# shangfuu/avse_challenge

Measured on AMD Instinct MI355X. Metric: utterances/sec (3s@16kHz + 75 lip frames), higher is better.
Workload: dtype fp32; 1 GPU; avse1 AV baseline train step (BASELINE configs[1]): HIP STFT front-end + AVNet (ResNet18 lip enc + TCN, dilated Conv2d audio net, LSTM fusion) fwd/bwd + Adam; global_batch=32, per_gpu_batch=32, seq_len=48000, stft_frames=376, lip_frames=75, lip_hw=96, parallelism=dp1, hip_graph=fwd+bwd+opt

## Files before the change

avse_challenge_amd/_lib.py:

```python
import ctypes
import os

import torch

_HERE = os.path.dirname(os.path.abspath(__file__))
LIB_PATH = os.environ.get("AVSE_HIP_LIB", os.path.join(_HERE, "libavse_hip.so"))

c_i64, c_i32, c_f32, c_vp = ctypes.c_int64, ctypes.c_int32, ctypes.c_float, ctypes.c_void_p

AVSE_F32, AVSE_BF16 = 0, 1


class ScanFwdArgs(ctypes.Structure):
    _fields_ = [
        ("batch", c_i64), ("dim", c_i64), ("seqlen", c_i64), ("dstate", c_i64),
        ("in_dtype", c_i32), ("delta_softplus", c_i32), ("reverse", c_i32),
        ("u", c_vp), ("u_bs", c_i64), ("u_ds", c_i64),
        ("delta", c_vp), ("delta_bs", c_i64), ("delta_ds", c_i64),
        ("A", c_vp),
        ("B", c_vp), ("B_bs", c_i64), ("B_ns", c_i64),
        ("C", c_vp), ("C_bs", c_i64), ("C_ns", c_i64),
        ("D", c_vp),
        ("z", c_vp), ("z_bs", c_i64), ("z_ds", c_i64),
        ("delta_bias", c_vp),
# ... 28 lines not shown
        ("ddelta_bias", c_vp),
        ("dz", c_vp), ("dz_bs", c_i64), ("dz_ds", c_i64),
        ("out_z", c_vp), ("out_z_bs", c_i64), ("out_z_ds", c_i64),
        ("workspace", c_vp),
        ("dz_accumulate", c_i32),
        ("dz_max", c_vp),
    ]


class GemmBf16Args(ctypes.Structure):
    _fields_ = [
        ("batch", c_i64), ("mp", c_i64), ("mq", c_i64), ("k", c_i64), ("fold", c_i64),
        ("p", c_vp), ("p_bs", c_i64), ("p_sx", c_i64), ("p_sk", c_i64), ("p_extent", c_i64),
        ("q", c_vp), ("q_bs", c_i64), ("q_sx", c_i64), ("q_sk", c_i64), ("q_extent", c_i64),
        ("c", c_vp), ("c_bs", c_i64), ("c_sq", c_i64),
        ("alpha", c_f32), ("c_dtype", c_i32),
    ]


class GemmF32sArgs(ctypes.Structure):
    _fields_ = [
        ("batch", c_i64), ("mp", c_i64), ("mq", c_i64), ("k", c_i64), ("fold", c_i64),
        ("p_hi", c_vp), ("p_lo", c_vp), ("p_bs", c_i64), ("p_sx", c_i64), ("p_sk", c_i64), ("p_extent", c_i64),
        ("p_max", c_vp),
        ("q_hi", c_vp), ("q_lo", c_vp), ("q_bs", c_i64), ("q_sx", c_i64), ("q_sk", c_i64), ("q_extent", c_i64),
        ("q_max", c_vp),
        ("c", c_vp), ("c_bs", c_i64), ("c_sq", c_i64),
        ("alpha", c_f32),
        ("nsub", c_i64), ("p_bs2", c_i64), ("q_bs2", c_i64),
    ]


SIGNATURES = {
    "avse_strerror": (ctypes.c_char_p, [c_i32]),
    "avse_abi_version": (c_i32, []),
    "avse_scan_n_chunks": (c_i64, [c_i64]),
    "avse_scan_bwd_workspace_bytes": (c_i64, [c_i64, c_i64, c_i64, c_i64]),
    "avse_scan_fwd": (c_i32, [ctypes.POINTER(ScanFwdArgs), c_vp]),
    "avse_scan_bwd": (c_i32, [ctypes.POINTER(ScanBwdArgs), c_vp]),
    "avse_dtproj": (c_i32, [c_i64, c_i64, c_i64, c_i64, c_i32, c_vp, c_i64, c_vp, c_i64, c_i64, c_vp, c_i32, c_vp, c_i64,
                            c_i64, c_vp]),
    "avse_cconv_bwd_workspace_bytes": (c_i64, [c_i64, c_i64, c_i64]),
    "avse_cconv_fwd": (c_i32, [c_i64, c_i64, c_i64, c_i64, c_vp, c_i64, c_i64, c_vp, c_vp, c_vp, c_i64, c_i64,
                               c_i32, c_i32, c_vp]),
    "avse_cconv_fwd_bf16": (c_i32, [c_i64, c_i64, c_i64, c_i64, c_vp, c_i64, c_i64, c_vp, c_vp, c_vp, c_i64, c_i64,
                                    c_i32, c_i32, c_vp]),
    "avse_cconv_bwd": (c_i32, [c_i64, c_i64, c_i64, c_i64, c_vp, c_i64, c_i64, c_vp, c_vp, c_vp, c_i64, c_i64,
                               c_vp, c_i64, c_i64, c_vp, c_vp, c_i32, c_i32, c_vp, c_i32, c_vp, c_vp]),
    "avse_cconv_bwd_bf16": (c_i32, [c_i64, c_i64, c_i64, c_i64, c_vp, c_i64, c_i64, c_vp, c_vp, c_vp, c_i64, c_i64,
                                    c_vp, c_i64, c_i64, c_vp, c_vp, c_i32, c_i32, c_vp, c_i32, c_vp, c_vp]),
    "avse_add_rmsnorm_fwd": (c_i32, [c_i64, c_i64, c_vp, c_vp, c_vp, c_f32, c_vp, c_vp, c_vp, c_vp, c_vp]),
    "avse_rmsnorm_bwd_workspace_bytes": (c_i64, [c_i64, c_i64]),
    "avse_rmsnorm_bwd": (c_i32, [c_i64, c_i64, c_vp, c_vp, c_vp, c_vp, c_vp, c_vp, c_vp, c_vp, c_vp, c_vp]),
    "avse_add_rmsnorm_fwd2": (c_i32, [c_i64, c_i64, c_vp, c_i32, c_vp, c_vp, c_f32, c_vp, c_i32, c_vp, c_vp, c_vp, c_vp]),
    "avse_rmsnorm_bwd2": (c_i32, [c_i64, c_i64, c_vp, c_i32] + [c_vp] * 9),
    "avse_stft_frames": (c_i64, [c_i64]),
    "avse_stft_fwd": (c_i32, [c_i64, c_i64, c_vp, c_vp, c_vp, c_vp]),
    "avse_istft": (c_i32, [c_i64, c_i64, c_i64, c_vp, c_vp, c_vp, c_vp, c_vp]),
    "avse_conv3d_wgrad_workspace_bytes": (c_i64, [c_i64, c_i64, c_i64, c_i64]),
    "avse_conv3d_wgrad": (c_i32, [c_i64] * 11 + [c_vp, c_vp, c_vp, c_i32, c_vp, c_vp]),
    "avse_conv3d_wgrad_u8": (c_i32, [c_i64] * 11 + [c_vp, c_vp, c_vp, c_i32, c_vp, c_vp]),
    "avse_conv3d_wgrad_u8_split": (c_i32, [c_i64] * 11 + [c_vp, c_vp, c_vp, c_vp, c_i32, c_vp, c_vp]),
    "avse_conv3d_wgrad_split": (c_i32, [c_i64] * 11 + [c_vp, c_vp, c_vp, c_vp, c_vp, c_i32, c_vp, c_vp]),
    "avse_conv3d_fwd_workspace_bytes": (c_i64, [c_i64, c_i64, c_i64]),
    "avse_conv3d_fwd": (c_i32, [c_i64] * 5 + [c_i32] + [c_vp] * 5),
    "avse_dconv_wgrad_workspace_bytes": (c_i64, [c_i64] * 4),
    "avse_dconv_wgrad": (c_i32, [c_i64] * 4 + [c_vp] * 6),
    "avse_prelu_fwd": (c_i32, [c_i64, c_i64, c_i64, c_i32, c_vp, c_vp, c_vp, c_vp]),
    "avse_prelu_bwd_workspace_bytes": (c_i64, [c_i64, c_i64]),
    "avse_prelu_bwd": (c_i32, [c_i64, c_i64, c_i64, c_i32, c_vp, c_vp, c_vp, c_vp, c_vp, c_vp, c_vp]),
    "avse_maxpool2d_out_size": (c_i64, [c_i64] * 4),
    "avse_maxpool2d_fwd": (c_i32, [c_i64] * 9 + [c_vp, c_vp, c_vp, c_vp]),
    "avse_maxpool2d_bwd": (c_i32, [c_i64] * 9 + [c_vp, c_vp, c_vp, c_vp]),
    "avse_transpose_cp": (c_i32, [c_i64] * 3 + [c_vp, c_vp, c_vp]),
    "avse_bnact_workspace_bytes": (c_i64, [c_i64, c_i64, c_i64]),
    "avse_bnact_fwd": (c_i32, [c_i64, c_i64, c_i64, c_vp, c_vp, c_vp, c_vp, c_i32, c_vp, c_i32, c_i32, c_f32, c_f32,
                               c_vp, c_vp, c_vp, c_vp, c_vp, c_vp, c_vp]),
    "avse_bnact_bwd": (c_i32, [c_i64, c_i64, c_i64, c_vp, c_vp, c_vp, c_vp, c_vp, c_vp, c_i32, c_vp, c_i32, c_i32,
                               c_vp, c_vp, c_vp, c_vp, c_vp, c_vp, c_vp, c_vp]),
    "avse_bnact_fwd_q": (c_i32, [c_i64, c_i64, c_i64, c_vp, c_vp, c_vp, c_i32, c_vp, c_i32, c_f32, c_f32, c_vp, c_vp,
                                 c_vp, c_vp, c_vp, c_vp, c_vp]),
    "avse_bnact_bwd_q": (c_i32, [c_i64, c_i64, c_i64, c_vp, c_vp, c_vp, c_vp, c_vp, c_i32, c_vp, c_i32, c_i32, c_vp,
                                 c_vp, c_vp, c_vp, c_vp, c_vp, c_vp]),
    "avse_prelu_nhwc_fwd": (c_i32, [c_i64, c_i64, c_i32, c_vp, c_vp, c_vp, c_vp]),
    "avse_prelu_nhwc_bwd_workspace_bytes": (c_i64, [c_i64, c_i64]),
    "avse_prelu_nhwc_bwd": (c_i32, [c_i64, c_i64, c_i32, c_vp, c_vp, c_vp, c_vp, c_vp, c_vp, c_vp]),
    "avse_prelu_gln_workspace_bytes": (c_i64, [c_i64, c_i64]),
    "avse_prelu_gln_fwd": (c_i32, [c_i64, c_i64, c_i64, c_vp, c_vp, c_vp, c_vp, c_f32, c_vp, c_vp, c_vp, c_vp]),
    "avse_prelu_gln_bwd": (c_i32, [c_i64, c_i64, c_i64] + [c_vp] * 11),
    "avse_prelu_gln_bwd_q": (c_i32, [c_i64, c_i64, c_i64] + [c_vp] * 7 + [c_i64] + [c_vp] * 6),
    "avse_dwconv_bwd_workspace_bytes": (c_i64, [c_i64, c_i64]),
    "avse_dwconv_fwd": (c_i32, [c_i64, c_i64, c_i64, c_i64, c_i64, c_vp, c_vp, c_vp, c_vp]),
    "avse_dwconv_bwd": (c_i32, [c_i64, c_i64, c_i64, c_i64, c_i64] + [c_vp] * 7),
    "avse_dwconv_gln_workspace_bytes": (c_i64, [c_i64, c_i64]),
    "avse_dwconv_gln_fwd": (c_i32, [c_i64] * 5 + [c_vp] * 5 + [c_f32] + [c_vp] * 5),
    "avse_dwconv_gln_fwd_q": (c_i32, [c_i64] * 5 + [c_vp] * 5 + [c_f32] + [c_vp] * 3 + [c_i64] + [c_vp] * 4),
    "avse_dwconv_gln_bwd": (c_i32, [c_i64] * 5 + [c_vp] * 14),
    "avse_lstm_padded_hidden": (c_i64, [c_i64]),
    "avse_lstm_group_size": (c_i64, [c_i64, c_i64]),
    "avse_lstm_group_workspace_bytes": (c_i64, [c_i64, c_i64]),
    "avse_lstm_group_capacity": (c_i64, [c_i64, c_i32]),
    "avse_lstm_fwd_group": (c_i32, [c_i64, c_i64, c_i64, c_i32, c_vp, c_vp, c_vp, c_i64, c_i64, c_vp, c_vp, c_vp, c_vp,
                                    c_vp]),
    "avse_lstm_bwd_group": (c_i32, [c_i64, c_i64, c_i64, c_i32, c_vp, c_i64, c_i64, c_vp, c_vp, c_vp, c_vp, c_vp, c_vp,
                                    c_vp]),
    "avse_lstm_fwd": (c_i32, [c_i64, c_i64, c_i64, c_i32, c_vp, c_vp, c_vp, c_i64, c_i64, c_vp, c_vp, c_vp]),
    "avse_lstm_bwd": (c_i32, [c_i64, c_i64, c_i64, c_i32, c_vp, c_i64, c_i64, c_vp, c_vp, c_vp, c_vp, c_vp]),
    "avse_gemm_bf16": (c_i32, [ctypes.POINTER(GemmBf16Args), c_vp]),
    "avse_gemm_f32s": (c_i32, [ctypes.POINTER(GemmF32sArgs), c_vp]),
    "avse_split16_planes": (c_i32, [c_i64, c_i64, c_i64, c_vp, c_i64, c_i64, c_vp, c_vp, c_vp, c_vp]),
    "avse_add_max": (c_i32, [c_i64, c_i64, c_i64, c_vp, c_vp, c_vp, c_vp, c_vp]),
    "avse_split16_planes_known": (c_i32, [c_i64, c_i64, c_i64, c_vp, c_i64, c_i64, c_vp, c_vp, c_vp, c_vp]),
    "avse_split16_planes_to": (c_i32, [c_i64, c_i64, c_i64, c_vp, c_i64, c_i64, c_vp, c_vp, c_i64, c_i64, c_vp, c_i32,
                                       c_vp]),
    "avse_dconv_wprep_bytes": (c_i64, []),
    "avse_split16": (c_i32, [c_i64, c_vp, c_vp, c_vp, c_vp]),
    "avse_split16_known": (c_i32, [c_i64, c_vp, c_vp, c_vp, c_vp]),
    "avse_dconv_wprep": (c_i32, [c_vp, c_i32, c_vp, c_vp, c_vp]),
    "avse_dconv_fwd": (c_i32, [c_i64, c_i64, c_i64, c_i64, c_vp, c_vp, c_vp, c_vp, c_vp, c_vp]),
    "avse_dconv_wprep2": (c_i32, [c_vp] * 6),
    "avse_dconv_wgrad16_workspace_bytes": (c_i64, [c_i64, c_i64, c_i64]),
    "avse_dconv_wgrad16": (c_i32, [c_i64, c_i64, c_i64, c_i64, c_vp, c_vp, c_vp, c_vp, c_vp, c_vp, c_vp, c_vp]),
    "avse_conv1_fwd": (c_i32, [c_i64] * 3 + [c_vp] * 5),
    "avse_conv1_dgrad": (c_i32, [c_i64] * 3 + [c_vp] * 4),
    "avse_conv1_wgrad_workspace_bytes": (c_i64, [c_i64] * 3),
    "avse_conv1_wgrad": (c_i32, [c_i64] * 3 + [c_vp] * 6),
    "avse_convf_fwd": (c_i32, [c_i64] + [c_vp] * 5),
    "avse_convf_dgrad": (c_i32, [c_i64] + [c_vp] * 4),
    "avse_convf_wgrad_workspace_bytes": (c_i64, [c_i64]),
    "avse_convf_wgrad": (c_i32, [c_i64] + [c_vp] * 6),
    "avse_sconv_wprep_bytes": (c_i64, [c_i64, c_i64]),
    "avse_sconv_wprep": (c_i32, [c_i64, c_i64, c_vp, c_i32, c_vp, c_vp, c_vp]),
    "avse_sconv_fwd": (c_i32, [c_i64] * 6 + [c_vp] * 6),
    "avse_sconv_wgrad_workspace_bytes": (c_i64, [c_i64] * 6),
    "avse_sconv_wgrad": (c_i32, [c_i64] * 6 + [c_vp] * 7),
    "avse_sconv_dgrad2_supported": (c_i32, [c_i64] * 5),
    "avse_sconv_dgrad2": (c_i32, [c_i64] * 5 + [c_vp] * 6),
}

_lib = None


class HipLibraryError(RuntimeError):
    pass


ABI_VERSION = 2


def lib():
    global _lib
    if _lib is None:
        if not os.path.exists(LIB_PATH):
            raise HipLibraryError(
                f"libavse_hip.so not found at {LIB_PATH}: build it with `python -c 'import __graft_entry__ as g; "
                f"g.build()'` (make -C avse_challenge_amd/csrc)")
        try:
            L = ctypes.CDLL(LIB_PATH, mode=ctypes.RTLD_GLOBAL)
        except OSError as e:
            raise HipLibraryError(f"failed to load {LIB_PATH}: {e}") from e
        for name, (res, args) in SIGNATURES.items():
            fn = getattr(L, name)
            fn.restype = res
            fn.argtypes = args
        if L.avse_abi_version() != ABI_VERSION:
            raise HipLibraryError(f"{LIB_PATH} has C-ABI version {L.avse_abi_version()}, the bindings expect "
# ... 17 lines not shown
```

avse_challenge_amd/csrc/bnact.hip:

```cpp
#include <algorithm>

#include "common.h"

namespace avse {
namespace bnact {

constexpr int THREADS = 256;
enum { ACT_NONE = 0, ACT_RELU = 1, ACT_PRELU = 2 };

struct Geo {
    int64_t N, CS, S;
    int C, TW, RPI, tiles, nrb;
};

template <int V> struct vld;
template <> struct vld<1> {
    __device__ static inline void ld(const float* p, float* v) { v[0] = *p; }
    __device__ static inline void st(float* p, const float* v) { *p = v[0]; }
};
template <> struct vld<4> {
    __device__ static inline void ld(const float* p, float* v) {
        const float4 q = *reinterpret_cast<const float4*>(p);
        v[0] = q.x; v[1] = q.y; v[2] = q.z; v[3] = q.w;
    }
    __device__ static inline void st(float* p, const float* v) {
        *reinterpret_cast<float4*>(p) = make_float4(v[0], v[1], v[2], v[3]);
    }
};

template <int V, int ACT>
struct ColConst {
    float a[V], b[V], al[V], mean[V], mlo[V], rstd[V], gam[V];
    __device__ inline float centred(float v, int k) const { return (v - mean[k]) - mlo[k]; }
    __device__ inline void load(const Geo& g, int64_t j0, const float* stats, const float* gamma, const float* beta,
                                const float* alpha, int alpha_n) {
#pragma unroll
        for (int k = 0; k < V; ++k) {
            const int c = (int)((j0 + k) / g.S);
            mean[k] = stats[4 * c];
            mlo[k] = stats[4 * c + 1];
            rstd[k] = stats[4 * c + 2];
            gam[k] = gamma ? gamma[c] : 1.f;
            a[k] = gam[k] * rstd[k];
            b[k] = beta ? beta[c] : 0.f;
            al[k] = ACT == ACT_PRELU ? alpha[alpha_n > 1 ? c : 0] : 0.f;
        }
    }
};

template <int ACT>
__device__ inline float act_fwd(float z, float al) {
    if constexpr (ACT == ACT_RELU) return z > 0.f ? z : 0.f;
    else if constexpr (ACT == ACT_PRELU) return z > 0.f ? z : al * z;
    else return z;
}
template <int ACT>
__device__ inline float act_bwd(float z, float g, float al) {
    if constexpr (ACT == ACT_RELU) return z > 0.f ? g : 0.f;
    else if constexpr (ACT == ACT_PRELU) return z > 0.f ? g : al * g;
    else return g;
}

template <int V, int NQ, int MAXQ = -1>
__device__ inline void block_partials(const Geo& g, float (&p)[NQ][V], bool valid, int64_t j0, float* ws) {
    __shared__ float part[NQ][THREADS * V];
    const int tx = threadIdx.x % g.TW, ty = threadIdx.x / g.TW;
#pragma unroll
    for (int q = 0; q < NQ; ++q)
#pragma unroll
        for (int k = 0; k < V; ++k) part[q][threadIdx.x * V + k] = p[q][k];
    __syncthreads();
    if (ty == 0 && valid) {
#pragma unroll
        for (int q = 0; q < NQ; ++q) {
            float s[V];
#pragma unroll
            for (int k = 0; k < V; ++k) s[k] = p[q][k];
            for (int t = 1; t < g.RPI; ++t)
#pragma unroll
                for (int k = 0; k < V; ++k)
                    s[k] = q == MAXQ ? fmaxf(s[k], part[q][(t * g.TW + tx) * V + k]) : s[k] + part[q][(t * g.TW + tx) * V + k];
            vld<V>::st(ws + ((int64_t)blockIdx.y * NQ + q) * g.CS + j0, s);
        }
    }
}

__device__ inline void block_max_out(float m, uint32_t* omax) {
    __shared__ uint32_t red[THREADS / 64];
    uint32_t b = __float_as_uint(m);
    for (int o = 32; o >= 1; o >>= 1) b = max(b, (uint32_t)__shfl_xor((int)b, o, 64));
    if ((threadIdx.x & 63) == 0) red[threadIdx.x >> 6] = b;
    __syncthreads();
    if (threadIdx.x == 0) {
        b = red[0];
#pragma unroll
        for (int w = 1; w < THREADS / 64; ++w) b = max(b, red[w]);
        if (b) atomicMax(omax, b);
    }
}

__device__ inline int q_split_exp(uint32_t mb) {
    const int ef = (int)((mb >> 23) & 0xff);
    if (mb == 0) return 0;
    const int k = ef == 0 ? -127 : ef - 127;
    return min(100, max(-100, 14 - k));
}
__device__ inline void q_store4(uint16_t* q, int64_t r, int64_t C, int64_t c, const float* v, float sc) {
    uint32_t hi[2], lo[2];
#pragma unroll
    for (int k = 0; k < 2; ++k) {
        const float s0 = v[2 * k] * sc, s1 = v[2 * k + 1] * sc;
        const _Float16 h0 = (_Float16)s0, h1 = (_Float16)s1;
        const _Float16 l0 = (_Float16)(s0 - (float)h0), l1 = (_Float16)(s1 - (float)h1);
        hi[k] = (uint32_t)__builtin_bit_cast(uint16_t, h0) | ((uint32_t)__builtin_bit_cast(uint16_t, h1) << 16);
        lo[k] = (uint32_t)__builtin_bit_cast(uint16_t, l0) | ((uint32_t)__builtin_bit_cast(uint16_t, l1) << 16);
    }
    uint16_t* base = q + r * 2 * C + 32 * (c >> 4) + (c & 15);
    *reinterpret_cast<uint2*>(base) = make_uint2(hi[0], hi[1]);
    *reinterpret_cast<uint2*>(base + 16) = make_uint2(lo[0], lo[1]);
}
__device__ inline void q_bound_out(double bnd, uint32_t* omax) {
    const float f = (float)(bnd * (1.0 + 1.0 / 1024.0));
    if (f > 0.f) atomicMax(omax, __float_as_uint(f));
}

template <int V, bool MAXD>
__global__ __launch_bounds__(THREADS) void stats_kernel(Geo g, const float* __restrict__ x, float* __restrict__ ws) {
    constexpr int NQ = MAXD ? 3 : 2;
    const int tx = threadIdx.x % g.TW, ty = threadIdx.x / g.TW;
    const int64_t j0 = ((int64_t)blockIdx.x * g.TW + tx) * V;
    const bool valid = j0 < g.CS;
    float p[NQ][V], K[V];
#pragma unroll
    for (int k = 0; k < V; ++k) {
#pragma unroll
        for (int q = 0; q < NQ; ++q) p[q][k] = 0.f;
        K[k] = valid ? x[((j0 + k) / g.S) * g.S] : 0.f;
    }
    if (valid) {
        for (int64_t r = (int64_t)blockIdx.y * g.RPI + ty; r < g.N; r += (int64_t)gridDim.y * g.RPI) {
            float v[V];
            vld<V>::ld(x + r * g.CS + j0, v);
#pragma unroll
            for (int k = 0; k < V; ++k) {
// ... 45 lines not shown
#pragma unroll
    for (int q = 0; q < NQ; ++q) acc[q] = 0.0;
    for (int i = i0 + threadIdx.x; i < i1; i += THREADS) {
        const int y = i / S, sidx = i - y * S;
        const int64_t col = (int64_t)c * g.S + sidx;
#pragma unroll
        for (int q = 0; q < NQ; ++q) {
            const double v = ws[((int64_t)y * NQ + q) * g.CS + col];
            acc[q] = q == MAXQ ? fmax(acc[q], v) : acc[q] + v;
        }
    }
#pragma unroll
    for (int q = 0; q < NQ; ++q) {
        const double v = q == MAXQ ? block_max_d(acc[q], red) : block_sum_d(acc[q], red);
        if (threadIdx.x == 0) fin[((int64_t)c * G + gi) * NQ + q] = v;
    }
}

__global__ void stats_combine(Geo g, const float* __restrict__ x, const double* __restrict__ fin, int G, float eps,
                              float momentum, float* __restrict__ running_mean, float* __restrict__ running_var,
                              float* __restrict__ stats, uint32_t* __restrict__ omax, int qb,
                              const float* __restrict__ gamma, const float* __restrict__ beta,
                              const float* __restrict__ alpha, int alpha_n, int act) {
    const int c = blockIdx.x * blockDim.x + threadIdx.x;
    if (!qb && c == 0 && omax) *omax = 0u;
    if (c >= g.C) return;
    double s1 = 0.0, s2 = 0.0, dmax = 0.0;
    for (int gi = 0; gi < G; ++gi) {
        s1 += fin[((int64_t)c * G + gi) * 3];
        s2 += fin[((int64_t)c * G + gi) * 3 + 1];
        dmax = fmax(dmax, fin[((int64_t)c * G + gi) * 3 + 2]);
    }
    const double n = (double)g.N * (double)g.S;
    const double m1 = s1 / n;
    double var = s2 / n - m1 * m1;
    if (var < 0.0) var = 0.0;
    const double mean = (double)x[(int64_t)c * g.S] + m1;
    const float hi = (float)mean;
    stats[4 * c] = hi;
    stats[4 * c + 1] = (float)(mean - (double)hi);
    const double rstd = 1.0 / sqrt(var + (double)eps);
    stats[4 * c + 2] = (float)rstd;
    const double dev = dmax + fabs(m1);
    stats[4 * c + 3] = (float)(dev * (1.0 + 1.0 / 1024.0));
    if (qb) {
        const double ga = gamma ? fabs((double)gamma[c]) : 1.0;
        double bz = ga * rstd * dev + (beta ? fabs((double)beta[c]) : 0.0);
        if (act == ACT_PRELU) bz *= fmax(1.0, fabs((double)alpha[alpha_n > 1 ? c : 0]));
        q_bound_out(bz, omax);
    }
    if (running_mean) running_mean[c] = (float)((1.0 - momentum) * running_mean[c] + momentum * mean);
    if (running_var) running_var[c] = (float)((1.0 - momentum) * running_var[c] + momentum * var * n / (n - 1.0));
}

__global__ void eval_stats_kernel(int C, const float* __restrict__ rm, const float* __restrict__ rv, float eps,
                                  float* __restrict__ stats, uint32_t* __restrict__ omax) {
    const int c = blockIdx.x * blockDim.x + threadIdx.x;
    if (c == 0 && omax) *omax = 0u;
    if (c < C) {
        stats[4 * c] = rm[c];
        stats[4 * c + 1] = 0.f;
        stats[4 * c + 2] = (float)(1.0 / sqrt((double)rv[c] + (double)eps));
        stats[4 * c + 3] = 0.f;
    }
}

template <int V, int ACT, bool RES, bool QOUT = false>
__global__ __launch_bounds__(THREADS) void apply_kernel(Geo g, const float* __restrict__ x, const float* __restrict__ res,
                                                        const float* __restrict__ stats, const float* __restrict__ gamma,
                                                        const float* __restrict__ beta, const float* __restrict__ alpha,
                                                        int alpha_n, float* __restrict__ y, uint32_t* __restrict__ ymax) {
    const int tx = threadIdx.x % g.TW, ty = threadIdx.x / g.TW;
    const int64_t j0 = ((int64_t)blockIdx.x * g.TW + tx) * V;
    float m = 0.f;
    if constexpr (QOUT) {
        const float sc = __builtin_ldexpf(1.f, q_split_exp(*ymax));
        if (j0 < g.CS) {
            ColConst<V, ACT> cc;
            cc.load(g, j0, stats, gamma, beta, alpha, alpha_n);
            for (int64_t r = (int64_t)blockIdx.y * g.RPI + ty; r < g.N; r += (int64_t)gridDim.y * g.RPI) {
                float v[V];
                vld<V>::ld(x + r * g.CS + j0, v);
#pragma unroll
                for (int k = 0; k < V; ++k) v[k] = act_fwd<ACT>(fmaf(cc.centred(v[k], k), cc.a[k], cc.b[k]), cc.al[k]);
                q_store4(reinterpret_cast<uint16_t*>(y), r, g.CS, j0, v, sc);
            }
        }
        return;
    }
    if (j0 < g.CS) {
        ColConst<V, ACT> cc;
        cc.load(g, j0, stats, gamma, beta, alpha, alpha_n);
        for (int64_t r = (int64_t)blockIdx.y * g.RPI + ty; r < g.N; r += (int64_t)gridDim.y * g.RPI) {
            const int64_t o = r * g.CS + j0;
            float v[V], rv[V];
            vld<V>::ld(x + o, v);
            if (RES) vld<V>::ld(res + o, rv);
#pragma unroll
            for (int k = 0; k < V; ++k) {
                float z = fmaf(cc.centred(v[k], k), cc.a[k], cc.b[k]);
                if (RES) z += rv[k];
                v[k] = act_fwd<ACT>(z, cc.al[k]);
                m = fmaxf(m, fabsf(v[k]));
            }
            vld<V>::st(y + o, v);
        }
    }
    if (ymax) block_max_out(m, ymax);
}

template <int V, int ACT, bool RES, bool MAXDZ = false>
__global__ __launch_bounds__(THREADS) void bwd_partial_kernel(Geo g, const float* __restrict__ x,
                                                              const float* __restrict__ res, const float* __restrict__ dy,
                                                              const float* __restrict__ stats,
                                                              const float* __restrict__ gamma, const float* __restrict__ beta,
                                                              const float* __restrict__ alpha, int alpha_n,
                                                              float* __restrict__ ws, float* __restrict__ dres) {
    constexpr int NQ = MAXDZ ? 4 : 3;
    const int tx = threadIdx.x % g.TW, ty = threadIdx.x / g.TW;
    const int64_t j0 = ((int64_t)blockIdx.x * g.TW + tx) * V;
    const bool valid = j0 < g.CS;
    float p[NQ][V];
#pragma unroll
    for (int k = 0; k < V; ++k)
#pragma unroll
        for (int q = 0; q < NQ; ++q) p[q][k] = 0.f;
    if (valid) {
        ColConst<V, ACT> cc;
        cc.load(g, j0, stats, gamma, beta, alpha, alpha_n);
        for (int64_t r = (int64_t)blockIdx.y * g.RPI + ty; r < g.N; r += (int64_t)gridDim.y * g.RPI) {
            const int64_t o = r * g.CS + j0;
            float v[V], gv[V], rv[V], dz[V];
            vld<V>::ld(x + o, v);
            vld<V>::ld(dy + o, gv);
            if (RES) vld<V>::ld(res + o, rv);
#pragma unroll
            for (int k = 0; k < V; ++k) {
                float z = fmaf(cc.centred(v[k], k), cc.a[k], cc.b[k]);
                if (RES) z += rv[k];
                dz[k] = act_bwd<ACT>(z, gv[k], cc.al[k]);
                const float xh = cc.centred(v[k], k) * cc.rstd[k];
                p[0][k] += dz[k];
                p[1][k] = fmaf(dz[k], xh, p[1][k]);
                if (ACT == ACT_PRELU && !(z > 0.f)) p[2][k] = fmaf(gv[k], z, p[2][k]);
                if constexpr (MAXDZ) p[3][k] = fmaxf(p[3][k], fabsf(dz[k]));
            }
            if (RES) vld<V>::st(dres + o, dz);
        }
    }
    block_partials<V, NQ, MAXDZ ? 3 : -1>(g, p, valid, j0, ws);
}

__global__ void bwd_combine(Geo g, const double* __restrict__ fin, int G, int training, float* __restrict__ dgamma,
                            float* __restrict__ dbeta, float* __restrict__ dalpha_c, float* __restrict__ kbuf,
                            uint32_t* __restrict__ omax, int qb, const float* __restrict__ stats,
                            const float* __restrict__ gamma) {
    const int c = blockIdx.x * blockDim.x + threadIdx.x;
    if (!qb && c == 0 && omax) *omax = 0u;
    if (c >= g.C) return;
    const int NQ = qb ? 4 : 3;
    double s0 = 0.0, s1 = 0.0, s2 = 0.0, dzmax = 0.0;
    for (int gi = 0; gi < G; ++gi) {
        s0 += fin[((int64_t)c * G + gi) * NQ];
        s1 += fin[((int64_t)c * G + gi) * NQ + 1];
        s2 += fin[((int64_t)c * G + gi) * NQ + 2];
        if (qb) dzmax = fmax(dzmax, fin[((int64_t)c * G + gi) * NQ + 3]);
    }
    const double n = (double)g.N * (double)g.S;
    if (dbeta) dbeta[c] = (float)s0;
    if (dgamma) dgamma[c] = (float)s1;
    if (dalpha_c) dalpha_c[c] = (float)s2;
    kbuf[2 * c] = training ? (float)(s0 / n) : 0.f;
    kbuf[2 * c + 1] = training ? (float)(s1 / n) : 0.f;
    if (qb) {
        const double rstd = (double)stats[4 * c + 2];
        const double ga = (gamma ? fabs((double)gamma[c]) : 1.0) * rstd;
        const double b = training ? dzmax + fabs(s0 / n) + (double)stats[4 * c + 3] * rstd * fabs(s1 / n) : dzmax;
        q_bound_out(ga * b, omax);
    }
}

template <int V, int ACT, bool RES, bool QOUT = false>
__device__ inline void bwd_apply_cols(const Geo& g, int64_t j0, int ty, const float* __restrict__ x,
                                      const float* __restrict__ dy, const float* __restrict__ dres,
                                      const float* __restrict__ stats, const float* __restrict__ gamma,
                                      const float* __restrict__ beta, const float* __restrict__ alpha, int alpha_n,
                                      const float* __restrict__ kbuf, float* __restrict__ dx, float& m, float qsc = 1.f) {
    ColConst<V, ACT> cc;
    cc.load(g, j0, stats, gamma, beta, alpha, alpha_n);
    float k1[V], k2[V];
#pragma unroll
    for (int k = 0; k < V; ++k) {
        const int c = (int)((j0 + k) / g.S);
        k1[k] = kbuf[2 * c];
        k2[k] = kbuf[2 * c + 1];
    }
    for (int64_t r = (int64_t)blockIdx.y * g.RPI + ty; r < g.N; r += (int64_t)gridDim.y * g.RPI) {
        const int64_t o = r * g.CS + j0;
        float v[V], dz[V];
        vld<V>::ld(x + o, v);
        if (RES) {
            vld<V>::ld(dres + o, dz);
        } else {
            float gv[V];
            vld<V>::ld(dy + o, gv);
#pragma unroll
            for (int k = 0; k < V; ++k) dz[k] = act_bwd<ACT>(fmaf(cc.centred(v[k], k), cc.a[k], cc.b[k]), gv[k], cc.al[k]);
        }
#pragma unroll
        for (int k = 0; k < V; ++k) {
            const float xh = cc.centred(v[k], k) * cc.rstd[k];
            v[k] = cc.a[k] * (dz[k] - k1[k] - xh * k2[k]);
            if constexpr (!QOUT) m = fmaxf(m, fabsf(v[k]));
        }
        if constexpr (QOUT) q_store4(reinterpret_cast<uint16_t*>(dx), r, g.CS, j0, v, qsc);
        else vld<V>::st(dx + o, v);
    }
}

template <int V, int ACT, bool RES, bool QOUT = false>
__global__ __launch_bounds__(THREADS) void bwd_apply_kernel(Geo g, const float* __restrict__ x,
                                                            const float* __restrict__ dy, const float* __restrict__ dres,
                                                            const float* __restrict__ stats,
                                                            const float* __restrict__ gamma, const float* __restrict__ beta,
                                                            const float* __restrict__ alpha, int alpha_n,
                                                            const float* __restrict__ kbuf, float* __restrict__ dx,
                                                            uint32_t* __restrict__ dxmax) {
    const int tx = threadIdx.x % g.TW, ty = threadIdx.x / g.TW;
    const int64_t j0 = ((int64_t)blockIdx.x * g.TW + tx) * V;
    float m = 0.f;
    if constexpr (QOUT) {
        const float sc = __builtin_ldexpf(1.f, q_split_exp(*dxmax));
        if (j0 < g.CS)
            bwd_apply_cols<V, ACT, RES, true>(g, j0, ty, x, dy, dres, stats, gamma, beta, alpha, alpha_n, kbuf, dx, m, sc);
        return;
    }
    if (j0 < g.CS) bwd_apply_cols<V, ACT, RES>(g, j0, ty, x, dy, dres, stats, gamma, beta, alpha, alpha_n, kbuf, dx, m);
    if (dxmax) block_max_out(m, dxmax);
}

inline int pow2ceil(int64_t v) {
    int p = 1;
    while (p < v) p <<= 1;
    return p;
}

inline Geo make_geo(int64_t N, int64_t C, int64_t S, int V) {
    Geo g;
    g.N = N; g.S = S; g.C = (int)C; g.CS = C * S;
    const int64_t cw = (g.CS + V - 1) / V;
    g.TW = cw >= THREADS ? THREADS : pow2ceil(cw);
    g.RPI = THREADS / g.TW;
    g.tiles = (int)((cw + g.TW - 1) / g.TW);
    const int64_t want = (N + (int64_t)g.RPI * 8 - 1) / ((int64_t)g.RPI * 8);
    const int64_t cap = std::max<int64_t>(1, 4096 / g.tiles);
    g.nrb = (int)std::max<int64_t>(1, std::min<int64_t>(std::min<int64_t>(want, cap), 65535));
    return g;
}

inline bool shape_ok(int64_t N, int64_t C, int64_t S) {
    return N > 0 && C > 0 && S > 0 && N * C * S < (1LL << 40) && C * S < (1LL << 31) && C < (1 << 20) &&
           (C * S + 3) / 4 <= (int64_t)THREADS * 0x7FFFFFFF;
}

inline bool al16(const void* p) { return ((uintptr_t)p & 15) == 0; }

inline double* fin_ptr(float* workspace, const Geo& g) {
    const Geo g1 = make_geo(g.N, g.C, g.S, 1), g4 = make_geo(g.N, g.C, g.S, 4);
    const int64_t nrb = std::max(g1.nrb, g4.nrb);
    const uintptr_t p = (uintptr_t)(workspace + 4 * nrb * g.CS + 2 * (int64_t)g.C);
    return reinterpret_cast<double*>((p + 15) & ~(uintptr_t)15);
}

template <template <int, int, bool> class K>
struct dispatch {
    template <typename... A>
    static void run(int V, int act, bool res, dim3 grid, hipStream_t st, A... a) {
#define AVSE_BNACT_CASE(VV, AA, RR) \
    if (V == VV && act == AA && res == RR) { hipLaunchKernelGGL((K<VV, AA, RR>::fn), grid, dim3(THREADS), 0, st, a...); return; }
        AVSE_BNACT_CASE(4, ACT_NONE, false) AVSE_BNACT_CASE(4, ACT_RELU, false) AVSE_BNACT_CASE(4, ACT_PRELU, false)
        AVSE_BNACT_CASE(4, ACT_NONE, true) AVSE_BNACT_CASE(4, ACT_RELU, true) AVSE_BNACT_CASE(4, ACT_PRELU, true)
        AVSE_BNACT_CASE(1, ACT_NONE, false) AVSE_BNACT_CASE(1, ACT_RELU, false) AVSE_BNACT_CASE(1, ACT_PRELU, false)
        AVSE_BNACT_CASE(1, ACT_NONE, true) AVSE_BNACT_CASE(1, ACT_RELU, true) AVSE_BNACT_CASE(1, ACT_PRELU, true)
#undef AVSE_BNACT_CASE
    }
};
template <int V, int A, bool R> struct ApplyK { static constexpr auto fn = apply_kernel<V, A, R>; };
template <int V, int A, bool R> struct ApplyQK { static constexpr auto fn = apply_kernel<V, A, R, true>; };
template <int V, int A, bool R> struct BwdPartQK { static constexpr auto fn = bwd_partial_kernel<V, A, R, true>; };
template <int V, int A, bool R> struct BwdApplyQK { static constexpr auto fn = bwd_apply_kernel<V, A, R, true>; };
template <template <int, int, bool> class K>
struct dispatch_q {
    template <typename... A>
    static void run(int act, dim3 grid, hipStream_t st, A... a) {
// ... 53 lines not shown
    if (qout)
        dispatch_q<ApplyQK>::run(act, grid, st, g, x, res, (const float*)stats, gamma, beta, alpha, (int)alpha_n, y, y_max);
    else
        dispatch<ApplyK>::run(V, act, res != nullptr, grid, st, g, x, res, (const float*)stats, gamma, beta, alpha,
                              (int)alpha_n, y, y_max);
    AVSE_CHECK_LAUNCH();
    return AVSE_OK;
}

int avse_bnact_fwd(int64_t N, int64_t C, int64_t S, const float* x, const float* res, const float* gamma,
                   const float* beta, int32_t act, const float* alpha, int32_t alpha_n, int32_t training, float eps,
                   float momentum, float* running_mean, float* running_var, float* stats, float* y, float* workspace,
                   uint32_t* y_max, avse_stream_t stream) {
    return bnact_fwd_impl(N, C, S, x, res, gamma, beta, act, alpha, alpha_n, training, eps, momentum, running_mean,
                          running_var, stats, y, workspace, y_max, false, (hipStream_t)stream);
}

int avse_bnact_fwd_q(int64_t N, int64_t C, int64_t S, const float* x, const float* gamma, const float* beta, int32_t act,
                     const float* alpha, int32_t alpha_n, float eps, float momentum, float* running_mean,
                     float* running_var, float* stats, void* yq, float* workspace, uint32_t* y_bound,
                     avse_stream_t stream) {
    return bnact_fwd_impl(N, C, S, x, nullptr, gamma, beta, act, alpha, alpha_n, 1, eps, momentum, running_mean,
                          running_var, stats, (float*)yq, workspace, y_bound, true, (hipStream_t)stream);
}

static int bnact_bwd_impl(int64_t N, int64_t C, int64_t S, const float* x, const float* res, const float* dy,
                          const float* stats, const float* gamma, const float* beta, int32_t act, const float* alpha,
                          int32_t alpha_n, int32_t training, float* dx, float* dres, float* dgamma, float* dbeta,
                          float* dalpha_c, float* workspace, uint32_t* dx_max, bool qout, hipStream_t st) {
    if (!x || !dy || !stats || !dx || !workspace || (act == ACT_PRELU && (!alpha || !dalpha_c)) || (res && !dres))
        return AVSE_EINVAL;
    if (!shape_ok(N, C, S) || act < ACT_NONE || act > ACT_PRELU) return AVSE_ESHAPE;
    if (act == ACT_PRELU && alpha_n != 1 && alpha_n != C) return AVSE_ESHAPE;
    const int V = ((C * S) % 4 == 0 && al16(x) && al16(dy) && al16(dx) && (!res || (al16(res) && al16(dres))) &&
                   al16(workspace)) ? 4 : 1;
    if (qout && (!dx_max || res || S != 1 || C % 64 || V != 4)) return AVSE_ESHAPE;
    const Geo g = make_geo(N, C, S, V);
    const dim3 grid(g.tiles, g.nrb);
    float* kbuf = workspace + 4 * (int64_t)g.nrb * g.CS;
    const int G = chan_groups(g);
    double* fin = fin_ptr(workspace, g);
    if (qout) {
        dispatch_q<BwdPartQK>::run(act, grid, st, g, x, res, dy, stats, gamma, beta, alpha, (int)alpha_n, workspace, dres);
        AVSE_CHECK_LAUNCH();
        hipLaunchKernelGGL((chan_partial_kernel<4, 3>), dim3((unsigned)C, G), dim3(THREADS), 0, st, g,
                           (const float*)workspace, fin, dx_max);
    } else {
        dispatch<BwdPartK>::run(V, act, res != nullptr, grid, st, g, x, res, dy, stats, gamma, beta, alpha, (int)alpha_n,
                                workspace, dres);
        AVSE_CHECK_LAUNCH();
        hipLaunchKernelGGL((chan_partial_kernel<3>), dim3((unsigned)C, G), dim3(THREADS), 0, st, g,
                           (const float*)workspace, fin, (uint32_t*)nullptr);
    }
    AVSE_CHECK_LAUNCH();
    hipLaunchKernelGGL(bwd_combine, dim3((unsigned)((C + 255) / 256)), dim3(256), 0, st, g, (const double*)fin, G,
                       (int)training, dgamma, dbeta, dalpha_c, kbuf, dx_max, (int)qout, stats, gamma);
    AVSE_CHECK_LAUNCH();
    if (qout)
        dispatch_q<BwdApplyQK>::run(act, grid, st, g, x, dy, (const float*)dres, stats, gamma, beta, alpha, (int)alpha_n,
                                   (const float*)kbuf, dx, dx_max);
    else
        dispatch<BwdApplyK>::run(V, act, res != nullptr, grid, st, g, x, dy, (const float*)dres, stats, gamma, beta,
                                 alpha, (int)alpha_n, (const float*)kbuf, dx, dx_max);
    AVSE_CHECK_LAUNCH();
    return AVSE_OK;
}

int avse_bnact_bwd(int64_t N, int64_t C, int64_t S, const float* x, const float* res, const float* dy, const float* stats,
                   const float* gamma, const float* beta, int32_t act, const float* alpha, int32_t alpha_n,
                   int32_t training, float* dx, float* dres, float* dgamma, float* dbeta, float* dalpha_c,
                   float* workspace, uint32_t* dx_max, avse_stream_t stream) {
    return bnact_bwd_impl(N, C, S, x, res, dy, stats, gamma, beta, act, alpha, alpha_n, training, dx, dres, dgamma,
                          dbeta, dalpha_c, workspace, dx_max, false, (hipStream_t)stream);
}

int avse_bnact_bwd_q(int64_t N, int64_t C, int64_t S, const float* x, const float* dy, const float* stats,
                     const float* gamma, const float* beta, int32_t act, const float* alpha, int32_t alpha_n,
                     int32_t training, void* dxq, float* dgamma, float* dbeta, float* dalpha_c, float* workspace,
                     uint32_t* dx_bound, avse_stream_t stream) {
    return bnact_bwd_impl(N, C, S, x, nullptr, dy, stats, gamma, beta, act, alpha, alpha_n, training, (float*)dxq,
                          nullptr, dgamma, dbeta, dalpha_c, workspace, dx_bound, true, (hipStream_t)stream);
}

}
```

avse_challenge_amd/csrc/dconv.hip:

```cpp
#include <algorithm>

#include "common.h"

namespace avse {
namespace dcf {

typedef _Float16 half8 __attribute__((ext_vector_type(8)));
typedef float floatx16 __attribute__((ext_vector_type(16)));
typedef int i4_t __attribute__((ext_vector_type(4)));
typedef __attribute__((address_space(3))) void lds_void_t;

constexpr int C = 64, KS = 5, NQ = 4, TP = 256, THREADS = 256, WAVES = THREADS / 64;
constexpr int ROWB = 64;
constexpr int WIMG = KS * C * ROWB;
constexpr int NSTG = KS * NQ;
constexpr int MAXD = 16;
constexpr int XIMG_MAX = (TP + 8 * MAXD) * ROWB;
constexpr int STAGE = XIMG_MAX + WIMG;
constexpr int NBUF = 3;
constexpr int MAXP = (XIMG_MAX + WIMG) / 1024 / WAVES + 1;
static_assert(NBUF * STAGE <= 160 * 1024, "LDS");

__device__ inline int swz(int r) { return (r >> 2) & 3; }

__device__ inline int split_exp(uint32_t mb) {
    const int ef = (int)((mb >> 23) & 0xff);
    if (mb == 0) return 0;
    const int k = ef == 0 ? -127 : ef - 127;
    return min(100, max(-100, 14 - k));
}

__device__ inline i4_t rsrc_of(const void* base, int64_t bytes) {
    if (bytes > 0x7FFFFFF0LL) bytes = 0x7FFFFFF0LL;
    const uint64_t a = (uint64_t)base;
    return i4_t{__builtin_amdgcn_readfirstlane((int)(uint32_t)a), __builtin_amdgcn_readfirstlane((int)((a >> 32) & 0xffff)),
                __builtin_amdgcn_readfirstlane((int)bytes), 0x00020000};
}

__device__ inline void dma16(i4_t r, uint32_t lds_addr, uint32_t voff) {
    asm volatile("s_mov_b32 m0, %2\n\tbuffer_load_dwordx4 %0, %1, 0 offen lds" ::"v"(voff), "s"(r), "s"(lds_addr)
                 : "memory");
}

__device__ inline uint32_t lds_u32(const void* p) {
    return __builtin_amdgcn_readfirstlane((uint32_t)(uintptr_t)(const lds_void_t*)p);
}

__device__ inline void wait_all_but(int n) {
    switch (n) {
        case 0: asm volatile("s_waitcnt vmcnt(0)" ::: "memory"); break;
        case 1: asm volatile("s_waitcnt vmcnt(1)" ::: "memory"); break;
        case 2: asm volatile("s_waitcnt vmcnt(2)" ::: "memory"); break;
        case 3: asm volatile("s_waitcnt vmcnt(3)" ::: "memory"); break;
        case 4: asm volatile("s_waitcnt vmcnt(4)" ::: "memory"); break;
        case 5: asm volatile("s_waitcnt vmcnt(5)" ::: "memory"); break;
        case 6: asm volatile("s_waitcnt vmcnt(6)" ::: "memory"); break;
        case 7: asm volatile("s_waitcnt vmcnt(7)" ::: "memory"); break;
        case 8: asm volatile("s_waitcnt vmcnt(8)" ::: "memory"); break;
        case 9: asm volatile("s_waitcnt vmcnt(9)" ::: "memory"); break;
        case 10: asm volatile("s_waitcnt vmcnt(10)" ::: "memory"); break;
        case 11: asm volatile("s_waitcnt vmcnt(11)" ::: "memory"); break;
        default: asm volatile("s_waitcnt vmcnt(12)" ::: "memory"); break;
    }
}

__device__ inline half8 frag(const uint8_t* img, int row, int c) {
    return *reinterpret_cast<const half8*>(img + row * ROWB + 16 * (c ^ swz(row)));
}

struct Args {
    const void* xq;
    const void* wq;
    const uint32_t* maxbits;
    const float* bias;
    float* y;
    int N, H, W, tiles;
};

template <int D, int NW, int WGS = 1>
__global__ __launch_bounds__(64 * NW, WGS) void fwd_kernel(Args a) {
    constexpr int TPX = 64 * NW, NSEG = NW == 4 ? 2 : 3;
    constexpr int NP = (TPX + 4 * D * NSEG + 15) / 16 * 16;
    constexpr int XIMG = NP * ROWB;
    constexpr int STG = XIMG + WIMG;
    constexpr int NB = WGS == 2 ? 2 : ((3 * STG <= 160 * 1024) ? 3 : 2);
    constexpr int PX = XIMG / 1024, PT = PX + WIMG / 1024;
    constexpr int MP = PT / NW + 1;
    __shared__ __attribute__((aligned(1024))) uint8_t lds[NB * STG];
    const int lane = threadIdx.x & 63;
    const int wave = __builtin_amdgcn_readfirstlane(threadIdx.x >> 6);
    const int bid = xcd_remap(blockIdx.x, gridDim.x);
    const int n = bid / a.tiles, t = bid % a.tiles;
    const int HW = a.H * a.W;
    const int p0 = t * TPX;
    const int r0 = p0 / a.W, w0 = p0 - r0 * a.W;
    const int n0 = min(TPX, a.W - w0), n1 = min(TPX - n0, a.W), n2 = TPX - n0 - n1;
    const int S1 = n0 + 4 * D, S2 = n0 + n1 + 8 * D;
    const i4_t rx = rsrc_of(a.xq, (int64_t)a.N * HW * 256);
    const i4_t rw = rsrc_of(a.wq, (int64_t)NSTG * WIMG);
    const uint32_t lds0 = lds_u32(lds);

    int pcol[MP], prow[MP];
    uint32_t pchunk[MP];
    const int npieces = (PT - wave + NW - 1) / NW;
#pragma unroll
    for (int m = 0; m < MP; ++m) {
        const int k = wave + NW * m;
        if (k < PX) {
            const int r = 16 * k + (lane >> 2), c = (lane & 3) ^ swz(r);
            int col, row;
            if (r < S1) {
                col = w0 - 2 * D + r;
                row = r0;
            } else if (r < S2 || NSEG == 2) {
                col = -2 * D + (r - S1);
                row = (n1 > 0 && r < S1 + n1 + 4 * D) ? r0 + 1 : -1000000;
            } else {
                col = -2 * D + (r - S2);
                row = (n2 > 0 && r < S2 + n2 + 4 * D) ? r0 + 2 : -1000000;
            }
            pcol[m] = (col >= 0 && col < a.W) ? col : -1;
            prow[m] = row;
            pchunk[m] = 16u * c;
        } else {
            const int r = 16 * (k - PX) + (lane >> 2), c = (lane & 3) ^ swz(r);
            pcol[m] = 0;
            prow[m] = 0;
            pchunk[m] = (uint32_t)(r * ROWB + 16 * c);
        }
    }
    auto issue = [&](int s) {
        const int kh = s / NQ, q = s % NQ;
        const uint32_t img = lds0 + (s % NB) * STG;
#pragma unroll
        for (int m = 0; m < MP; ++m) {
            if (m >= npieces) break;
            const int k = wave + NW * m;
            if (k < PX) {
                const int row = prow[m] + D * (kh - 2);
                const bool ok = pcol[m] >= 0 && row >= 0 && row < a.H;
                const uint32_t pix = ((uint32_t)n * (uint32_t)a.H + (uint32_t)row) * (uint32_t)a.W + (uint32_t)pcol[m];
                const uint32_t off = ok ? pix * 256u + (uint32_t)(q * 64) + pchunk[m] : 0x7FFFFFF0u;
                dma16(rx, img + k * 1024, off);
            } else {
                dma16(rw, img + XIMG + (k - PX) * 1024, (uint32_t)(s * WIMG) + pchunk[m]);
            }
        }
    };

    int posA[2];
#pragma unroll
    for (int i = 0; i < 2; ++i) {
        const int j = 64 * wave + 32 * i + (lane & 31);
        posA[i] = j + 4 * D * ((j >= n0) + (j >= n0 + n1));
    }
    const int hc = lane >> 5;

    floatx16 acc[2][2];
#pragma unroll
    for (int i = 0; i < 2; ++i)
#pragma unroll
        for (int j = 0; j < 2; ++j)
#pragma unroll
            for (int e = 0; e < 16; ++e) acc[i][j][e] = 0.f;

    issue(0);
    if (NB == 3) issue(1);
    for (int s = 0; s < NSTG; ++s) {
        if (NB == 3 && s + 1 < NSTG) wait_all_but(npieces);
        else asm volatile("s_waitcnt vmcnt(0)" ::: "memory");
        __builtin_amdgcn_s_barrier();
        asm volatile("" ::: "memory");
        if (s + NB - 1 < NSTG) issue(s + NB - 1);
        const uint8_t* ximg = lds + (s % NB) * STG;
        const uint8_t* wimg = ximg + XIMG;
#pragma unroll
        for (int kw = 0; kw < KS; ++kw) {
            half8 ah[2], al[2], bh[2], bl[2];
#pragma unroll
            for (int i = 0; i < 2; ++i) {
                const int r = posA[i] + D * kw;
                ah[i] = frag(ximg, r, hc);
                al[i] = frag(ximg, r, 2 + hc);
            }
#pragma unroll
            for (int j = 0; j < 2; ++j) {
                const int r = kw * C + 32 * j + (lane & 31);
                bh[j] = frag(wimg, r, hc);
                bl[j] = frag(wimg, r, 2 + hc);
            }
#pragma unroll
            for (int i = 0; i < 2; ++i)
#pragma unroll
                for (int j = 0; j < 2; ++j) {
                    acc[i][j] = __builtin_amdgcn_mfma_f32_32x32x16_f16(ah[i], bh[j], acc[i][j], 0, 0, 0);
                    acc[i][j] = __builtin_amdgcn_mfma_f32_32x32x16_f16(ah[i], bl[j], acc[i][j], 0, 0, 0);
                    acc[i][j] = __builtin_amdgcn_mfma_f32_32x32x16_f16(al[i], bh[j], acc[i][j], 0, 0, 0);
                }
        }
        if (NB == 2) {
            asm volatile("s_waitcnt lgkmcnt(0)" ::: "memory");
        }
    }

    const float scale = __builtin_ldexpf(1.f, -(split_exp(a.maxbits[0]) + split_exp(a.maxbits[1])));
#pragma unroll
    for (int j = 0; j < 2; ++j) {
        const int o = 32 * j + (lane & 31);
        const float bv = a.bias ? a.bias[o] : 0.f;
#pragma unroll
        for (int i = 0; i < 2; ++i)
#pragma unroll
            for (int g = 0; g < 4; ++g)
#pragma unroll
                for (int e = 0; e < 4; ++e) {
                    const int p = p0 + 64 * wave + 32 * i + 8 * g + 4 * (lane >> 5) + e;
                    if (p < HW) a.y[((int64_t)n * HW + p) * C + o] = acc[i][j][4 * g + e] * scale + bv;
                }
    }
}

constexpr int WG_CHUNK = 64;
constexpr int PIXB = 256;
constexpr int WTHREADS = 512, WWAVES = WTHREADS / 64;

typedef short s4_t __attribute__((ext_vector_type(4)));
typedef __attribute__((address_space(3))) s4_t lds_s4_t;

__device__ inline int tswz(int r, int c) { return c ^ (((r & 1) << 1) | ((r & 2) << 2)); }

__device__ inline half8 tfrag(const uint8_t* img, const int (&row)[2], int cb, int pl, int lane) {
    const int g = lane >> 4, i = lane & 15;
    const int q = 2 * cb + (g & 1);
    s4_t v[2];
#pragma unroll
    for (int u = 0; u < 2; ++u) {
        const int r = row[u];
        const int byte = q * 64 + pl * 32 + 8 * (i & 3);
        const int off = r * PIXB + 16 * tswz(r, byte >> 4) + (byte & 15);
        v[u] = __builtin_amdgcn_ds_read_tr16_b64_v4i16((lds_s4_t*)(img + off));
    }
    const s4_t w0 = v[0], w1 = v[1];
    const short __attribute__((ext_vector_type(8))) w = {w0[0], w0[1], w0[2], w0[3], w1[0], w1[1], w1[2], w1[3]};
    return __builtin_bit_cast(half8, w);
}

struct WArgs {
    const void* xq;
    const void* dyq;
    const uint32_t* xmax;
    const uint32_t* dymax;
    float* part;
    float* dbpart;
    int N, H, W, cpi, chunks, ranges;
};

struct ChunkPos {
    int n, p0, hA, wA0;
    __device__ void init(int c, int cpi, int W) {
        n = c / cpi;
        p0 = (c - n * cpi) * WG_CHUNK;
        hA = p0 / W;
        wA0 = p0 - hA * W;
    }
    __device__ void next(int HW, int W) {
        p0 += WG_CHUNK;
        if (p0 >= HW) {
            ++n;
            p0 = hA = wA0 = 0;
        } else {
            wA0 += WG_CHUNK;
            if (wA0 >= W) {
                wA0 -= W;
                ++hA;
            }
        }
    }
};

template <int D>
__global__ __launch_bounds__(WTHREADS, 1) void wgrad_kernel(WArgs a) {
    constexpr int NP = WG_CHUNK + 8 * D;
    constexpr int YIMG = WG_CHUNK * PIXB, XIMG = NP * PIXB, STG = YIMG + XIMG;
    constexpr int NB = (3 * STG <= 160 * 1024) ? 3 : 2;
    constexpr int PY = YIMG / 1024, PT = PY + XIMG / 1024;
    constexpr int MAXPW = PT / WWAVES + 1;
    __shared__ __attribute__((aligned(1024))) uint8_t lds[NB * STG];
    const int lane = threadIdx.x & 63;
    const int wave = __builtin_amdgcn_readfirstlane(threadIdx.x >> 6);
    const int bid = xcd_remap(blockIdx.x, gridDim.x);
    const int r = bid / KS, kh = bid % KS;
    const int c_lo = (int)((int64_t)r * a.chunks / a.ranges), c_hi = (int)((int64_t)(r + 1) * a.chunks / a.ranges);
    const int HW = a.H * a.W;
    const i4_t rx = rsrc_of(a.xq, (int64_t)a.N * HW * PIXB);
    const i4_t ry = rsrc_of(a.dyq, (int64_t)a.N * HW * PIXB);
    const uint32_t lds0 = lds_u32(lds);
    const int npieces = (PT - wave + WWAVES - 1) / WWAVES;
    const int pr = lane >> 4, pc = lane & 15;
    int pj[MAXPW];
    uint32_t psw[MAXPW];
#pragma unroll
// ... 258 lines not shown
    if (((uintptr_t)x & 15) || ((uintptr_t)xq & 15)) return AVSE_EALIGN;
    hipStream_t st = (hipStream_t)stream;
    if (hipMemsetAsync(maxbits, 0, 4, st) != hipSuccess) return AVSE_ELAUNCH;
    const int64_t n4 = n_pix * C / 4;
    hipLaunchKernelGGL(absmax_kernel, dim3((unsigned)std::max<int64_t>(1, std::min<int64_t>(AMAX_GRID, (n4 + AMAX_NT - 1) / AMAX_NT))),
                       dim3(AMAX_NT), 0, st, reinterpret_cast<const float4*>(x), n4, maxbits);
    AVSE_CHECK_LAUNCH();
    const int64_t nq = n_pix * NQ;
    const int blocks = (int)std::min<int64_t>((nq + 255) / 256, 8192);
    hipLaunchKernelGGL(split_kernel, dim3(blocks), dim3(256), 0, st, x, nq, maxbits, reinterpret_cast<uint4*>(xq));
    AVSE_CHECK_LAUNCH();
    return AVSE_OK;
}

int avse_split16_known(int64_t n_pix, const float* x, void* xq, const uint32_t* maxbits, avse_stream_t stream) {
    if (!x || !xq || !maxbits) return AVSE_EINVAL;
    if (n_pix <= 0) return AVSE_ESHAPE;
    if (((uintptr_t)x & 15) || ((uintptr_t)xq & 15)) return AVSE_EALIGN;
    const int64_t nq = n_pix * NQ;
    const int blocks = (int)std::min<int64_t>((nq + 255) / 256, 8192);
    hipLaunchKernelGGL(split_kernel, dim3(blocks), dim3(256), 0, (hipStream_t)stream, x, nq, maxbits,
                       reinterpret_cast<uint4*>(xq));
    AVSE_CHECK_LAUNCH();
    return AVSE_OK;
}

int avse_dconv_wprep(const float* w, int32_t transposed, void* wq, uint32_t* maxbits, avse_stream_t stream) {
    if (!w || !wq || !maxbits) return AVSE_EINVAL;
    hipLaunchKernelGGL(wprep_kernel, dim3(1), dim3(1024), 0, (hipStream_t)stream, w, transposed, maxbits,
                       reinterpret_cast<uint16_t*>(wq));
    AVSE_CHECK_LAUNCH();
    return AVSE_OK;
}

int avse_dconv_wprep2(const float* w, void* wq, void* wq_t, uint32_t* maxbits, uint32_t* maxbits_t,
                      avse_stream_t stream) {
    if (!w || !wq || !maxbits || (wq_t == nullptr) != (maxbits_t == nullptr)) return AVSE_EINVAL;
    hipLaunchKernelGGL(wprep2_kernel, dim3(wq_t ? 2 * NSTG : NSTG), dim3(1024), 0, (hipStream_t)stream, w, maxbits,
                       maxbits_t, reinterpret_cast<uint16_t*>(wq), reinterpret_cast<uint16_t*>(wq_t));
    AVSE_CHECK_LAUNCH();
    return AVSE_OK;
}

int64_t avse_dconv_wgrad16_workspace_bytes(int64_t N, int64_t H, int64_t W) {
    const int64_t chunks = N * ((H * W + WG_CHUNK - 1) / WG_CHUNK);
    return 4 * 2 * (int64_t)wgrad_ranges((int)std::min<int64_t>(chunks, 1 << 30)) * (KS * KS * C * C + C);
}

int avse_dconv_wgrad16(int64_t N, int64_t H, int64_t W, int64_t dil, const void* xq, const uint32_t* xmax,
                       const void* dyq, const uint32_t* dymax, float* dw, float* db, float* workspace,
                       avse_stream_t stream) {
    if (!xq || !xmax || !dyq || !dymax || !dw || !workspace) return AVSE_EINVAL;
    if (N <= 0 || H <= 0 || W < WG_CHUNK || (dil != 2 && dil != 4 && dil != 8 && dil != 16)) return AVSE_ESHAPE;
    if (N * H * W * 256 >= (1LL << 31) - 1024) return AVSE_ESHAPE;
    WArgs a;
    a.xq = xq;
    a.dyq = dyq;
    a.xmax = xmax;
    a.dymax = dymax;
    a.N = (int)N;
    a.H = (int)H;
    a.W = (int)W;
    a.cpi = (int)((H * W + WG_CHUNK - 1) / WG_CHUNK);
    a.chunks = (int)(N * a.cpi);
    a.ranges = wgrad_ranges(a.chunks);
    a.part = workspace;
    a.dbpart = db ? workspace + (int64_t)2 * a.ranges * KS * KS * C * C : nullptr;
    const dim3 grid((unsigned)(a.ranges * KS)), block(WTHREADS);
    hipStream_t st = (hipStream_t)stream;
    switch (dil) {
        case 2: hipLaunchKernelGGL(wgrad_kernel<2>, grid, block, 0, st, a); break;
        case 4: hipLaunchKernelGGL(wgrad_kernel<4>, grid, block, 0, st, a); break;
        case 8: hipLaunchKernelGGL(wgrad_kernel<8>, grid, block, 0, st, a); break;
        default: hipLaunchKernelGGL(wgrad_kernel<16>, grid, block, 0, st, a); break;
    }
    AVSE_CHECK_LAUNCH();
    constexpr int TOTAL = KS * KS * C * C;
    hipLaunchKernelGGL(wgrad_reduce_kernel, dim3((TOTAL + C + 255) / 256), dim3(256), 0, st, a.part, a.dbpart,
                       2 * a.ranges, dw, db);
    AVSE_CHECK_LAUNCH();
    return AVSE_OK;
}

int avse_dconv_fwd(int64_t N, int64_t H, int64_t W, int64_t dil, const void* xq, const void* wq,
                   const uint32_t* maxbits, const float* bias, float* y, avse_stream_t stream) {
    if (!xq || !wq || !maxbits || !y) return AVSE_EINVAL;
    if (N <= 0 || H <= 0 || W < 256 || (dil != 2 && dil != 4 && dil != 8 && dil != 16)) return AVSE_ESHAPE;
    if (N * H * W * 256 >= (1LL << 31) - 1024) return AVSE_ESHAPE;
    Args a;
    a.xq = xq;
    a.wq = wq;
    a.maxbits = maxbits;
    a.bias = bias;
    a.y = y;
    a.N = (int)N;
    a.H = (int)H;
    a.W = (int)W;
    const int nw = dil <= 8 ? 4 : 8;
    a.tiles = (int)((H * W + 64 * nw - 1) / (64 * nw));
    const dim3 grid((unsigned)(N * a.tiles)), block(64 * nw);
    hipStream_t st = (hipStream_t)stream;
    switch (dil) {
        case 2: hipLaunchKernelGGL((fwd_kernel<2, 4, 2>), grid, block, 0, st, a); break;
        case 4: hipLaunchKernelGGL((fwd_kernel<4, 4, 2>), grid, block, 0, st, a); break;
        case 8: hipLaunchKernelGGL((fwd_kernel<8, 4, 2>), grid, block, 0, st, a); break;
        default: hipLaunchKernelGGL((fwd_kernel<16, 8>), grid, block, 0, st, a); break;
    }
    AVSE_CHECK_LAUNCH();
    return AVSE_OK;
}

}
```

avse_challenge_amd/csrc/sconv.hip:

```cpp
#include <algorithm>

#include "common.h"

namespace avse {
namespace scv {

typedef _Float16 half8 __attribute__((ext_vector_type(8)));
typedef float floatx16 __attribute__((ext_vector_type(16)));
typedef int i4_t __attribute__((ext_vector_type(4)));
typedef short s4_t __attribute__((ext_vector_type(4)));
typedef __attribute__((address_space(3))) void lds_void_t;
typedef __attribute__((address_space(3))) s4_t lds_s4_t;

constexpr int ROWB = 64;
constexpr int NPOS_MAX = 720;
constexpr int XIMG = NPOS_MAX * ROWB;
constexpr uint32_t OOB = 0x7FFFFFF0u;

__device__ inline int swz(int r) { return (r >> 2) & 3; }

__device__ inline int split_exp(uint32_t mb) {
    const int ef = (int)((mb >> 23) & 0xff);
    if (mb == 0) return 0;
    const int k = ef == 0 ? -127 : ef - 127;
    return min(100, max(-100, 14 - k));
}

__device__ inline i4_t rsrc_of(const void* base, int64_t bytes) {
    if (bytes > 0x7FFFFFF0LL) bytes = 0x7FFFFFF0LL;
    const uint64_t a = (uint64_t)base;
    return i4_t{__builtin_amdgcn_readfirstlane((int)(uint32_t)a), __builtin_amdgcn_readfirstlane((int)((a >> 32) & 0xffff)),
                __builtin_amdgcn_readfirstlane((int)bytes), 0x00020000};
}

__device__ inline void dma16(i4_t r, uint32_t lds_addr, uint32_t voff) {
    asm volatile("s_mov_b32 m0, %2\n\tbuffer_load_dwordx4 %0, %1, 0 offen lds" ::"v"(voff), "s"(r), "s"(lds_addr)
                 : "memory");
}

__device__ inline uint32_t lds_u32(const void* p) {
    return __builtin_amdgcn_readfirstlane((uint32_t)(uintptr_t)(const lds_void_t*)p);
}

__device__ inline half8 frag(const uint8_t* img, int row, int c) {
    return *reinterpret_cast<const half8*>(img + row * ROWB + 16 * (c ^ swz(row)));
}

__device__ inline void divmod_small(int t, int d, float inv_d, int& q, int& r) {
    q = (int)((float)t * inv_d);
    r = t - q * d;
    if (r >= d) { r -= d; ++q; }
    if (r < 0) { r += d; --q; }
}

struct FArgs {
    const void* xq;
    const void* wq;
    const uint32_t* xmax;
    const uint32_t* wmax;
    float* y;
    int N, Hi, Wi, Ci, Ho, Wo, Co;
    int tiles_n;
    int RS, npos;
};

template <int S, int TN>
__global__ __launch_bounds__(512, 1) void fwd_kernel(FArgs a) {
    constexpr int WAVES = 8, WN = TN / 64, WM = WAVES / WN, TM = 64 * WM;
    constexpr int WIMG = 3 * TN * ROWB;
    constexpr int STG = XIMG + WIMG;
    constexpr int PW = WIMG / 1024;
    constexpr int MP = (NPOS_MAX / 16 + PW + WAVES - 1) / WAVES;
    __shared__ __attribute__((aligned(1024))) uint8_t lds[2 * STG];
    const int lane = threadIdx.x & 63;
    const int wave = __builtin_amdgcn_readfirstlane(threadIdx.x >> 6);
    const int bid = xcd_remap(blockIdx.x, gridDim.x);
    const int tn = bid % a.tiles_n, tm = bid / a.tiles_n;
    const int p0 = tm * TM, o0 = tn * TN;
    const int NHWo = a.N * a.Ho * a.Wo, NHo = a.N * a.Ho;
    const int g0 = p0 / a.Wo;
    const int NQ = a.Ci / 16, NSTG = 3 * NQ;
    const i4_t rx = rsrc_of(a.xq, (int64_t)a.N * a.Hi * a.Wi * a.Ci * 4);
    const i4_t rw = rsrc_of(a.wq, (int64_t)9 * a.Ci * a.Co * 4);
    const uint32_t lds0 = lds_u32(lds);
    const int PX = a.npos / 16, PT = PX + PW;
    const int npieces = (PT - wave + WAVES - 1) / WAVES;
    const uint32_t pixb = (uint32_t)a.Ci * 4u;

    uint32_t pbase[MP];
    int khlo[MP], khhi[MP];
#pragma unroll
    for (int m = 0; m < MP; ++m) {
        const int k = wave + WAVES * m;
        if (k < PX) {
            const int r = 16 * k + (lane >> 2), c = (lane & 3) ^ swz(r);
            const int rk = r / a.RS, col = r - rk * a.RS, g = g0 + rk;
            const int n = g / a.Ho, ho = g - n * a.Ho, wi = col - 1;
            const bool ok = g < NHo && wi >= 0 && wi < a.Wi;
            const int h0 = S * ho - 1;
            khlo[m] = ok ? max(0, -h0) : 3;
            khhi[m] = ok ? min(3, a.Hi - h0) : 0;
            pbase[m] = ok ? ((uint32_t)(n * a.Hi + h0) * (uint32_t)a.Wi + (uint32_t)wi) * pixb + 16u * c : 0u;
        } else {
            const int r = 16 * (k - PX) + (lane >> 2), c = (lane & 3) ^ swz(r);
            const int kw = r / TN, ol = r - kw * TN;
            khlo[m] = khhi[m] = 0;
            pbase[m] = (uint32_t)(kw * a.Co + o0 + ol) * 64u + 16u * c;
        }
    }
    const uint32_t rowb = (uint32_t)a.Wi * pixb, wstage = 3u * (uint32_t)a.Co * 64u;
    auto issue = [&](int s) {
        const int kh = s / NQ, q = s - kh * NQ;
        const uint32_t img = lds0 + (s & 1) * STG;
        const uint32_t xadd = (uint32_t)kh * rowb + (uint32_t)(q * 64), wadd = (uint32_t)s * wstage;
#pragma unroll
        for (int m = 0; m < MP; ++m) {
            if (m >= npieces) break;
            const int k = wave + WAVES * m;
            if (k < PX) {
                const bool ok = kh >= khlo[m] && kh < khhi[m];
                dma16(rx, img + k * 1024, ok ? pbase[m] + xadd : OOB);
            } else {
                dma16(rw, img + XIMG + (k - PX) * 1024, pbase[m] + wadd);
            }
        }
    };

    const int wm = wave / WN, wn = wave % WN;
    int posA[2];
#pragma unroll
    for (int i = 0; i < 2; ++i) {
        const int p = min(p0 + 64 * wm + 32 * i + (lane & 31), NHWo - 1);
        const int gr = p / a.Wo, wo = p - gr * a.Wo;
        posA[i] = (gr - g0) * a.RS + S * wo;
    }
    const int hc = lane >> 5;

    floatx16 acc[2][2];
#pragma unroll
    for (int i = 0; i < 2; ++i)
#pragma unroll
        for (int j = 0; j < 2; ++j)
#pragma unroll
            for (int e = 0; e < 16; ++e) acc[i][j][e] = 0.f;

    issue(0);
    for (int s = 0; s < NSTG; ++s) {
        asm volatile("s_waitcnt vmcnt(0)" ::: "memory");
        __builtin_amdgcn_s_barrier();
        asm volatile("" ::: "memory");
        if (s + 1 < NSTG) issue(s + 1);
        const uint8_t* ximg = lds + (s & 1) * STG;
        const uint8_t* wimg = ximg + XIMG;
#pragma unroll
        for (int kw = 0; kw < 3; ++kw) {
            half8 ah[2], al[2], bh[2], bl[2];
#pragma unroll
            for (int i = 0; i < 2; ++i) {
                const int r = posA[i] + kw;
                ah[i] = frag(ximg, r, hc);
                al[i] = frag(ximg, r, 2 + hc);
            }
#pragma unroll
            for (int j = 0; j < 2; ++j) {
                const int r = kw * TN + 64 * wn + 32 * j + (lane & 31);
                bh[j] = frag(wimg, r, hc);
                bl[j] = frag(wimg, r, 2 + hc);
            }
#pragma unroll
            for (int pr = 0; pr < 3; ++pr)
#pragma unroll
                for (int i = 0; i < 2; ++i)
#pragma unroll
                    for (int j = 0; j < 2; ++j)
                        acc[i][j] = __builtin_amdgcn_mfma_f32_32x32x16_f16(pr == 2 ? al[i] : ah[i], pr == 1 ? bl[j] : bh[j],
                                                                           acc[i][j], 0, 0, 0);
        }
        asm volatile("s_waitcnt lgkmcnt(0)" ::: "memory");
    }

    const float scale = __builtin_ldexpf(1.f, -(split_exp(*a.xmax) + split_exp(*a.wmax)));
#pragma unroll
    for (int j = 0; j < 2; ++j) {
        const int o = o0 + 64 * wn + 32 * j + (lane & 31);
#pragma unroll
        for (int i = 0; i < 2; ++i)
#pragma unroll
            for (int g = 0; g < 4; ++g)
#pragma unroll
                for (int e = 0; e < 4; ++e) {
                    const int p = p0 + 64 * wm + 32 * i + 8 * g + 4 * (lane >> 5) + e;
                    if (p < NHWo) a.y[(int64_t)p * a.Co + o] = acc[i][j][4 * g + e] * scale;
                }
    }
}

struct DArgs {
    const void* dyq;
    const void* wq;
    const uint32_t* dymax;
    const uint32_t* wmax;
    float* dx;
    int N, Hi, Wi, O, I, Ho, Wo;
    int tiles_n;
    int tile0[5];
    int py[4], px[4], Ha[4], Wb[4], RS[4], npos[4];
    uint32_t woff[4];
};

__host__ __device__ inline uint32_t dg2_tap_off(int ph) {
    return ph == 0 ? 0u : ph == 1 ? 1u : ph == 2 ? 3u : 5u;
}

template <int NTH, int NTW, int TN>
__device__ __forceinline__ void dgrad2_body(const DArgs& a, int slot, int tile, uint8_t* lds) {
    constexpr int WAVES = 8, WN = TN / 64, WM = WAVES / WN, TM = 64 * WM;
    constexpr int WIMG = NTW * TN * ROWB, WIMG_MAX = 2 * TN * ROWB;
    constexpr int STG = XIMG + WIMG_MAX;
    constexpr int PW = WIMG / 1024;
    constexpr int MP = (NPOS_MAX / 16 + PW + WAVES - 1) / WAVES;
    const int lane = threadIdx.x & 63;
    const int wave = __builtin_amdgcn_readfirstlane(threadIdx.x >> 6);
    const int py = a.py[slot], px = a.px[slot], Ha = a.Ha[slot], Wb = a.Wb[slot], RS = a.RS[slot];
    const int tn = tile % a.tiles_n, tm = tile / a.tiles_n;
    const int p0 = tm * TM, o0 = tn * TN;
    const int NP = a.N * Ha * Wb, NHa = a.N * Ha;
    const int g0 = p0 / Wb;
    const int NQ = a.I / 16, NSTG = NTH * NQ;
    const i4_t rx = rsrc_of(a.dyq, (int64_t)a.N * a.Ho * a.Wo * a.I * 4);
    const i4_t rw = rsrc_of(a.wq, (int64_t)9 * a.I * a.O * 4);
    const uint32_t lds0 = lds_u32(lds);
    const int PX = a.npos[slot] / 16, PT = PX + PW;
    const int npieces = (PT - wave + WAVES - 1) / WAVES;
    const uint32_t pixb = (uint32_t)a.I * 4u;
    const uint32_t rowb = (uint32_t)a.Wo * pixb;
    uint32_t pbase[MP];
    int thok[MP];
#pragma unroll
    for (int m = 0; m < MP; ++m) {
        const int k = wave + WAVES * m;
        if (k < PX) {
            const int r = 16 * k + (lane >> 2), c = (lane & 3) ^ swz(r);
            const int rk = r / RS, col = r - rk * RS, g = g0 + rk;
            const int n = g / Ha, ar = g - n * Ha;
            const bool ok = g < NHa && col < a.Wo;
            int bits = 0;
            if (ok) bits = (NTH == 2) ? ((ar + 1 < a.Ho ? 1 : 0) | 2) : 1;
            thok[m] = bits;
            pbase[m] = ok ? ((uint32_t)(n * a.Ho + ar) * (uint32_t)a.Wo + (uint32_t)col) * pixb + 16u * c : 0u;
        } else {
            const int r = 16 * (k - PX) + (lane >> 2), c = (lane & 3) ^ swz(r);
            const int tw = r / TN, ol = r - tw * TN;
            thok[m] = 0;
            pbase[m] = a.woff[slot] + (uint32_t)(tw * a.O + o0 + ol) * 64u + 16u * c;
        }
    }
    const uint32_t wstage = (uint32_t)NTW * (uint32_t)a.O * 64u;
    auto issue = [&](int s) {
        const int th = s / NQ, q = s - th * NQ;
        const uint32_t img = lds0 + (s & 1) * STG;
        const uint32_t xadd = (NTH == 2 && th == 0 ? rowb : 0u) + (uint32_t)(q * 64), wadd = (uint32_t)s * wstage;
#pragma unroll
        for (int m = 0; m < MP; ++m) {
            if (m >= npieces) break;
            const int k = wave + WAVES * m;
            if (k < PX) {
                const bool ok = (thok[m] >> th) & 1;
                dma16(rx, img + k * 1024, ok ? pbase[m] + xadd : OOB);
            } else {
                dma16(rw, img + XIMG + (k - PX) * 1024, pbase[m] + wadd);
            }
        }
    };

    const int wm = wave / WN, wn = wave % WN;
    int posA[2];
// ... 401 lines not shown
int64_t avse_sconv_wprep_bytes(int64_t co, int64_t ci) { return 9 * co * ci * 4; }

int avse_sconv_wprep(int64_t co, int64_t ci, const float* w, int32_t transposed, void* wq, uint32_t* wmax,
                     avse_stream_t stream) {
    if (!w || !wq || !wmax) return AVSE_EINVAL;
    if (co <= 0 || ci <= 0 || co % 64 || ci % 64 || co > 4096 || ci > 4096) return AVSE_ESHAPE;
    hipStream_t st = (hipStream_t)stream;
    if (hipMemsetAsync(wmax, 0, 4, st) != hipSuccess) return AVSE_ELAUNCH;
    const int n = (int)(9 * co * ci);
    hipLaunchKernelGGL(wmax_kernel, dim3((unsigned)std::min(256, (n + 255) / 256)), dim3(256), 0, st, w, n, wmax);
    AVSE_CHECK_LAUNCH();
    if (transposed == 2)
        hipLaunchKernelGGL(wsplit_dgrad2_kernel, dim3((unsigned)std::min(2048, (n + 255) / 256)), dim3(256), 0, st, w,
                           (int)co, (int)ci, wmax, reinterpret_cast<uint16_t*>(wq));
    else
        hipLaunchKernelGGL(wsplit_kernel, dim3((unsigned)std::min(2048, (n + 255) / 256)), dim3(256), 0, st, w, (int)co,
                           (int)ci, transposed, wmax, reinterpret_cast<uint16_t*>(wq));
    AVSE_CHECK_LAUNCH();
    return AVSE_OK;
}

static int dg2_setup(int64_t N, int64_t Hi, int64_t Wi, int64_t ci, int64_t co, DArgs& a, int& TN) {
    if (N <= 0 || Hi <= 0 || Wi <= 0 || ci <= 0 || co <= 0 || ci % 64 || co % 64 || ci > 4096 || co > 4096)
        return AVSE_ESHAPE;
    if (N * Hi * Wi * ci * 4 >= (1LL << 31) - 4096 || N * Hi * Wi * co * 4 >= (1LL << 31) - 4096) return AVSE_ESHAPE;
    a.N = (int)N;
    a.Hi = (int)Hi;
    a.Wi = (int)Wi;
    a.O = (int)ci;
    a.I = (int)co;
    a.Ho = out_dim((int)Hi, 2);
    a.Wo = out_dim((int)Wi, 2);
    TN = ci % 128 ? 64 : 128;
    const int TM = TN == 64 ? 512 : 256;
    a.tiles_n = (int)(ci / TN);
    static const int order[4] = {3, 2, 1, 0};
    int64_t t0 = 0;
    for (int s = 0; s < 4; ++s) {
        const int ph = order[s], py = ph >> 1, px = ph & 1;
        a.py[s] = py;
        a.px[s] = px;
        a.Ha[s] = ((int)Hi - py + 1) / 2;
        a.Wb[s] = ((int)Wi - px + 1) / 2;
        a.RS[s] = a.Wb[s] + 1;
        a.woff[s] = dg2_tap_off(ph) * (uint32_t)(ci * co * 4);
        a.tile0[s] = (int)t0;
        const int64_t np = N * a.Ha[s] * a.Wb[s];
        a.npos[s] = np > 0 ? fwd_npos(TM, a.Wb[s], a.RS[s]) : 0;
        if (a.npos[s] > NPOS_MAX) return AVSE_ESHAPE;
        t0 += (np + TM - 1) / TM * a.tiles_n;
        if (t0 >= (1LL << 31)) return AVSE_ESHAPE;
    }
    a.tile0[4] = (int)t0;
    return AVSE_OK;
}

int avse_sconv_dgrad2_supported(int64_t N, int64_t Hi, int64_t Wi, int64_t ci, int64_t co) {
    DArgs a;
    int TN;
    return dg2_setup(N, Hi, Wi, ci, co, a, TN) == AVSE_OK ? 1 : 0;
}

int avse_sconv_dgrad2(int64_t N, int64_t Hi, int64_t Wi, int64_t ci, int64_t co, const void* dyq,
                      const uint32_t* dymax, const void* wq, const uint32_t* wmax, float* dx, avse_stream_t stream) {
    if (!dyq || !dymax || !wq || !wmax || !dx) return AVSE_EINVAL;
    DArgs a;
    int TN;
    const int rc = dg2_setup(N, Hi, Wi, ci, co, a, TN);
    if (rc != AVSE_OK) return rc;
    a.dyq = dyq;
    a.wq = wq;
    a.dymax = dymax;
    a.wmax = wmax;
    a.dx = dx;
    if (a.tile0[4] == 0) return AVSE_OK;
    const dim3 grid((unsigned)a.tile0[4]), block(512);
    hipStream_t st = (hipStream_t)stream;
    if (TN == 64) hipLaunchKernelGGL((dgrad2_kernel<64>), grid, block, 0, st, a);
    else hipLaunchKernelGGL((dgrad2_kernel<128>), grid, block, 0, st, a);
    AVSE_CHECK_LAUNCH();
    return AVSE_OK;
}

int avse_sconv_fwd(int64_t N, int64_t Hi, int64_t Wi, int64_t ci, int64_t co, int64_t stride, const void* xq,
                   const uint32_t* xmax, const void* wq, const uint32_t* wmax, float* y, avse_stream_t stream) {
    if (!xq || !xmax || !wq || !wmax || !y) return AVSE_EINVAL;
    if (N <= 0 || Hi <= 0 || Wi <= 0 || ci <= 0 || co <= 0 || ci % 64 || co % 64 || (stride != 1 && stride != 2))
        return AVSE_ESHAPE;
    if (N * Hi * Wi * ci * 4 >= (1LL << 31) - 4096 || 9 * ci * co * 4 >= (1LL << 31)) return AVSE_ESHAPE;
    FArgs a;
    a.xq = xq;
    a.wq = wq;
    a.xmax = xmax;
    a.wmax = wmax;
    a.y = y;
    a.N = (int)N;
    a.Hi = (int)Hi;
    a.Wi = (int)Wi;
    a.Ci = (int)ci;
    a.Co = (int)co;
    a.Ho = out_dim((int)Hi, (int)stride);
    a.Wo = out_dim((int)Wi, (int)stride);
    a.RS = (int)stride * a.Wo + 2;
    const int TN = co % 128 ? 64 : 128, TM = TN == 64 ? 512 : 256;
    a.npos = fwd_npos(TM, a.Wo, a.RS);
    if (a.npos > NPOS_MAX) return AVSE_ESHAPE;
    const int64_t NHWo = N * a.Ho * a.Wo;
    if (NHWo * co >= (1LL << 31)) return AVSE_ESHAPE;
    a.tiles_n = (int)(co / TN);
    const int64_t tiles = (NHWo + TM - 1) / TM * a.tiles_n;
    if (tiles >= (1LL << 31)) return AVSE_ESHAPE;
    const dim3 grid((unsigned)tiles), block(512);
    hipStream_t st = (hipStream_t)stream;
    if (stride == 1) {
        if (TN == 64) hipLaunchKernelGGL((fwd_kernel<1, 64>), grid, block, 0, st, a);
        else hipLaunchKernelGGL((fwd_kernel<1, 128>), grid, block, 0, st, a);
    } else {
        if (TN == 64) hipLaunchKernelGGL((fwd_kernel<2, 64>), grid, block, 0, st, a);
        else hipLaunchKernelGGL((fwd_kernel<2, 128>), grid, block, 0, st, a);
    }
    AVSE_CHECK_LAUNCH();
    return AVSE_OK;
}

static int wg_setup(int64_t N, int64_t Hi, int64_t Wi, int64_t ci, int64_t co, int64_t stride, WArgs& a) {
    if (N <= 0 || Hi <= 0 || Wi <= 0 || ci <= 0 || co <= 0 || ci % 64 || co % 64 || (stride != 1 && stride != 2))
        return AVSE_ESHAPE;
    if (N * Hi * Wi * ci * 4 >= (1LL << 31) - 4096) return AVSE_ESHAPE;
    a.N = (int)N;
    a.Hi = (int)Hi;
    a.Wi = (int)Wi;
    a.Ci = (int)ci;
    a.Co = (int)co;
    a.Ho = out_dim((int)Hi, (int)stride);
    a.Wo = out_dim((int)Wi, (int)stride);
    a.RS = (int)stride * a.Wo + 2;
    a.npw = wg_npw(a.Wo, a.RS);
    if (a.npw > NPW_MAX) return AVSE_ESHAPE;
    const int64_t NHWo = N * a.Ho * a.Wo;
    if (NHWo * co * 4 >= (1LL << 31) - 4096) return AVSE_ESHAPE;
    a.chunks = (int)((NHWo + WG_CHUNK - 1) / WG_CHUNK);
    a.nob = (int)(co % 128 ? co / 64 : co / 128);
    a.nib = (int)(ci / 64);
    a.ranges = wg_ranges(a.chunks, 3 * a.nob * a.nib);
    a.inv_ho = 1.f / (float)a.Ho;
    a.inv_wo = 1.f / (float)a.Wo;
    a.q64 = WG_CHUNK / a.Wo;
    a.r64 = WG_CHUNK % a.Wo;
    return AVSE_OK;
}

static int wg_kg(int64_t co) { return co % 128 ? 4 : 2; }

int64_t avse_sconv_wgrad_workspace_bytes(int64_t N, int64_t Hi, int64_t Wi, int64_t ci, int64_t co, int64_t stride) {
    WArgs a;
    if (wg_setup(N, Hi, Wi, ci, co, stride, a) != AVSE_OK) return -1;
    return (int64_t)a.ranges * wg_kg(co) * 9 * co * ci * 4;
}

int avse_sconv_wgrad(int64_t N, int64_t Hi, int64_t Wi, int64_t ci, int64_t co, int64_t stride, const void* xq,
                     const uint32_t* xmax, const void* dyq, const uint32_t* dymax, float* dw, float* workspace,
                     avse_stream_t stream) {
    if (!xq || !xmax || !dyq || !dymax || !dw || !workspace) return AVSE_EINVAL;
    WArgs a;
    const int rc = wg_setup(N, Hi, Wi, ci, co, stride, a);
    if (rc != AVSE_OK) return rc;
    a.xq = xq;
    a.dyq = dyq;
    a.xmax = xmax;
    a.dymax = dymax;
    a.part = workspace;
    const bool ob128 = co % 128 == 0;
    const dim3 grid((unsigned)(a.ranges * 3 * a.nob * a.nib)), block(512);
    hipStream_t st = (hipStream_t)stream;
    if (ob128) {
        if (stride == 1) hipLaunchKernelGGL((wgrad_kernel<1, 128>), grid, block, 0, st, a);
        else hipLaunchKernelGGL((wgrad_kernel<2, 128>), grid, block, 0, st, a);
    } else {
        if (stride == 1) hipLaunchKernelGGL((wgrad_kernel<1, 64>), grid, block, 0, st, a);
        else hipLaunchKernelGGL((wgrad_kernel<2, 64>), grid, block, 0, st, a);
    }
    AVSE_CHECK_LAUNCH();
    const int64_t total = 9 * co * ci;
    hipLaunchKernelGGL(wgrad_reduce_kernel, dim3((unsigned)((total + 63) / 64)), dim3(256), 0, st, a.part,
                       a.ranges * wg_kg(co), (int)co, (int)ci, dw);
    AVSE_CHECK_LAUNCH();
    return AVSE_OK;
}

}
```

avse_challenge_amd/kernels.py:

```python
import functools

import torch

from . import _lib
from ._lib import AVSE_BF16, AVSE_F32, ScanBwdArgs, ScanFwdArgs, check, ptr, stream_ptr

NSTATE = 16

LAUNCH_TAPS = {}
LAUNCH_WORK = {}


def _tap_begin(name, device):
    taps = LAUNCH_TAPS.get(name)
    if taps is None or torch.cuda.is_current_stream_capturing():
        return None
    e0, e1 = torch.cuda.Event(enable_timing=True), torch.cuda.Event(enable_timing=True)
    e0.record(torch.cuda.current_stream(device))
    return taps, e0, e1, device, name


def _tap_end(tap, work=None):
    if tap is not None:
        taps, e0, e1, device, name = tap
# ... 434 lines not shown
    dy = dy.float().contiguous(memory_format=cl)
    Bn, _, H, W = x.shape
    L = _lib.lib()
    out = torch.empty((64, 64, 5, 5), device=x.device, dtype=torch.float32)
    ws = torch.empty((L.avse_dconv_wgrad_workspace_bytes(Bn, H, W, dilation) + 3) // 4, device=x.device,
                     dtype=torch.float32)
    db = torch.empty(64, device=x.device, dtype=torch.float32) if bias_grad else None
    tap = _tap_begin("avse_dconv_wgrad", x.device)
    check(L.avse_dconv_wgrad(Bn, H, W, dilation, ptr(x), ptr(dy), ptr(out), ptr(db) if bias_grad else None, ptr(ws),
                             stream_ptr(x.device)), "avse_dconv_wgrad")
    _tap_end(tap)
    return (out, db) if bias_grad else out



DCONV_DILATIONS = (2, 4, 8, 16)


def dconv_split_ok(x, dilation):
    return (x.is_cuda and x.dtype == torch.float32 and x.dim() == 4 and x.shape[1] == 64 and x.shape[3] >= 256
            and dilation in DCONV_DILATIONS and x.shape[0] * x.shape[2] * x.shape[3] * 256 < (1 << 31) - 1024)


def split16(x, maxbits):
    _need_gpu(x)
    known = _known_absmax(x)
    if is_split_q(x):
        maxbits[:1].copy_(known)
        return q_view(x)
    x = x.contiguous(memory_format=torch.channels_last)
    npix = x.shape[0] * x.shape[2] * x.shape[3]
    xq = torch.empty((npix, 256), device=x.device, dtype=torch.uint8)
    if known is not None:
        maxbits[:1].copy_(known)
        check(_lib.lib().avse_split16_known(npix, ptr(x), ptr(xq), ptr(maxbits), stream_ptr(x.device)),
              "avse_split16_known")
    else:
        check(_lib.lib().avse_split16(npix, ptr(x), ptr(xq), ptr(maxbits), stream_ptr(x.device)), "avse_split16")
    return xq


def dconv_wprep(w, transposed, maxbits):
    _need_gpu(w)
    L = _lib.lib()
    wq = torch.empty(int(L.avse_dconv_wprep_bytes()), device=w.device, dtype=torch.uint8)
    check(L.avse_dconv_wprep(ptr(w.float().contiguous()), int(bool(transposed)), ptr(wq), ptr(maxbits),
                             stream_ptr(w.device)), "avse_dconv_wprep")
    return wq


def dconv_wprep2(w, maxbits, maxbits_t=None):
    _need_gpu(w)
    L = _lib.lib()
    nb = int(L.avse_dconv_wprep_bytes())
    wq = torch.empty(nb, device=w.device, dtype=torch.uint8)
    wq_t = torch.empty(nb, device=w.device, dtype=torch.uint8) if maxbits_t is not None else None
    check(L.avse_dconv_wprep2(ptr(w.float().contiguous()), ptr(wq), ptr(wq_t) if wq_t is not None else None,
                              ptr(maxbits), ptr(maxbits_t) if maxbits_t is not None else None, stream_ptr(w.device)),
          "avse_dconv_wprep2")
    return wq, wq_t


def dconv_fwd(x, w, dilation, bias=None, transposed=False, split=None, wq=None):
    _need_gpu(x, w, bias)
    if not dconv_split_ok(x, dilation) or tuple(w.shape) != (64, 64, 5, 5):
        raise RuntimeError(f"dconv_fwd: unsupported shape {tuple(x.shape)} / {tuple(w.shape)} dilation {dilation}")
    N, _, H, W = x.shape
    if split is None:
        maxbits = torch.empty(2, device=x.device, dtype=torch.int32)
        xq = split16(x, maxbits)
    else:
        xq, maxbits = split
    if wq is None:
        wq = dconv_wprep(w, transposed, maxbits)
    y = torch.empty((N, 64, H, W), device=x.device, dtype=torch.float32, memory_format=torch.channels_last)
    tap = _tap_begin("avse_dconv_fwd", x.device)
    check(_lib.lib().avse_dconv_fwd(N, H, W, dilation, ptr(xq), ptr(wq), ptr(maxbits),
                                    ptr(None if bias is None else bias.float().contiguous()), ptr(y),
                                    stream_ptr(x.device)), "avse_dconv_fwd")
    _tap_end(tap)
    return y


def dconv_wgrad16(xs, dys, shape, dilation, bias_grad=False):
    (xq, xm), (dyq, dym) = xs, dys
    _need_gpu(xq, dyq)
    N, _, H, W = shape
    L = _lib.lib()
    dw = torch.empty((64, 64, 5, 5), device=xq.device, dtype=torch.float32)
    db = torch.empty(64, device=xq.device, dtype=torch.float32) if bias_grad else None
    ws = torch.empty((L.avse_dconv_wgrad16_workspace_bytes(N, H, W) + 3) // 4, device=xq.device, dtype=torch.float32)
    tap = _tap_begin("avse_dconv_wgrad16", xq.device)
    check(L.avse_dconv_wgrad16(N, H, W, dilation, ptr(xq), ptr(xm), ptr(dyq), ptr(dym), ptr(dw), ptr(db), ptr(ws),
                               stream_ptr(xq.device)), "avse_dconv_wgrad16")
    _tap_end(tap)
    return (dw, db) if bias_grad else dw



def conv1_fwd(x, w, b=None):
    _need_gpu(x, w, b)
    n, _, h, wd = x.shape
    y = torch.empty((n, 64, h, wd), device=x.device, dtype=torch.float32, memory_format=torch.channels_last)
    tap = _tap_begin("avse_conv1_fwd", x.device)
    check(_lib.lib().avse_conv1_fwd(n, h, wd, ptr(x.contiguous()), ptr(w.float().contiguous()),
                                    ptr(None if b is None else b.float().contiguous()), ptr(y), stream_ptr(x.device)),
          "avse_conv1_fwd")
    _tap_end(tap)
    return y


def conv1_bwd(x, w, dy, need_dx=True, need_dw=True):
    _need_gpu(x, w, dy)
    n, _, h, wd = x.shape
    dy = dy.contiguous(memory_format=torch.channels_last)
    L = _lib.lib()
    dx = dw = db = None
    if need_dx:
        dx = torch.empty((n, 1, h, wd), device=x.device, dtype=torch.float32)
        check(L.avse_conv1_dgrad(n, h, wd, ptr(dy), ptr(w.float().contiguous()), ptr(dx), stream_ptr(x.device)),
              "avse_conv1_dgrad")
    if need_dw:
        dw = torch.empty((64, 1, 5, 5), device=x.device, dtype=torch.float32)
        db = torch.empty(64, device=x.device, dtype=torch.float32)
        ws = torch.empty((L.avse_conv1_wgrad_workspace_bytes(n, h, wd) + 3) // 4, device=x.device, dtype=torch.float32)
        check(L.avse_conv1_wgrad(n, h, wd, ptr(x.contiguous()), ptr(dy), ptr(dw), ptr(db), ptr(ws),
                                 stream_ptr(x.device)), "avse_conv1_wgrad")
    return dx, dw, db



def convf_fwd(x, w, b=None):
    _need_gpu(x, w, b)
    n, c, h, wd = x.shape
    x = x.contiguous(memory_format=torch.channels_last)
    y = torch.empty((n, 4, h, wd), device=x.device, dtype=torch.float32, memory_format=torch.channels_last)
    check(_lib.lib().avse_convf_fwd(n * h * wd, ptr(x), ptr(w.float().contiguous()),
                                    ptr(None if b is None else b.float().contiguous()), ptr(y), stream_ptr(x.device)),
          "avse_convf_fwd")
    return y


def convf_bwd(x, w, dy, need_dx=True, need_dw=True):
    _need_gpu(x, w, dy)
    n, c, h, wd = x.shape
    dy = dy.contiguous(memory_format=torch.channels_last)
    L = _lib.lib()
    dx = dw = db = None
    if need_dx:
        dx = torch.empty((n, c, h, wd), device=x.device, dtype=torch.float32, memory_format=torch.channels_last)
        check(L.avse_convf_dgrad(n * h * wd, ptr(dy), ptr(w.float().contiguous()), ptr(dx), stream_ptr(x.device)),
              "avse_convf_dgrad")
    if need_dw:
        x = x.contiguous(memory_format=torch.channels_last)
        dw = torch.empty((4, c, 1, 1), device=x.device, dtype=torch.float32)
        db = torch.empty(4, device=x.device, dtype=torch.float32)
        ws = torch.empty((L.avse_convf_wgrad_workspace_bytes(n * h * wd) + 3) // 4, device=x.device, dtype=torch.float32)
        check(L.avse_convf_wgrad(n * h * wd, ptr(x), ptr(dy), ptr(dw), ptr(db), ptr(ws), stream_ptr(x.device)),
              "avse_convf_wgrad")
    return dx, dw, db



def sconv_ok(x, cout, stride):
    if not (x.is_cuda and x.dtype == torch.float32 and x.dim() == 4 and stride in (1, 2)):
        return False
    n, cin, h, w = x.shape
    if cin % 64 or cout % 64 or n * h * w * max(cin, cout) * 4 >= (1 << 31) - 4096:
        return False
    return _lib.lib().avse_sconv_wgrad_workspace_bytes(n, h, w, cin, cout, stride) > 0


def split_nhwc(x, maxbits):
    _need_gpu(x)
    x = x.contiguous(memory_format=torch.channels_last)
    n, c, h, w = x.shape
    xq = torch.empty((n * h * w, 4 * c), device=x.device, dtype=torch.uint8)
    check(_lib.lib().avse_split16(n * h * w * (c // 64), ptr(x), ptr(xq), ptr(maxbits), stream_ptr(x.device)),
          "avse_split16")
    return xq


def split_q(x):
    known = _known_absmax(x)
    if is_split_q(x):
        return q_view(x), known
    if known is None:
        xm = torch.empty(1, device=x.device, dtype=torch.int32)
        return split_nhwc(x, xm), xm
    _need_gpu(x)
    x = x.contiguous(memory_format=torch.channels_last)
    n, c, h, w = x.shape
    if c % 64:
        raise RuntimeError(f"split_q: channels must be a multiple of 64, got {c}")
    xq = torch.empty((n * h * w, 4 * c), device=x.device, dtype=torch.uint8)
    check(_lib.lib().avse_split16_known(n * h * w * (c // 64), ptr(x), ptr(xq), ptr(known), stream_ptr(x.device)),
          "avse_split16_known")
    return xq, known


def sconv_wprep(w, transposed, wmax):
    _need_gpu(w)
    co, ci = w.shape[0], w.shape[1]
    L = _lib.lib()
    wq = torch.empty(int(L.avse_sconv_wprep_bytes(co, ci)), device=w.device, dtype=torch.uint8)
    check(L.avse_sconv_wprep(co, ci, ptr(w.float().contiguous()), int(bool(transposed)), ptr(wq), ptr(wmax),
                             stream_ptr(w.device)), "avse_sconv_wprep")
    return wq


def sconv_fwd(xs, xshape, w, stride, transposed=False):
    xq, xm = xs
    _need_gpu(xq, w)
    n, ci, h, wd = xshape
    co = w.shape[1] if transposed else w.shape[0]
    if transposed and stride != 1:
        raise RuntimeError("sconv_fwd: the transposed (input gradient) form is stride 1 only")
    wm = torch.empty(1, device=w.device, dtype=torch.int32)
    wq = sconv_wprep(w, transposed, wm)
    ho, wo = (h - 1) // stride + 1, (wd - 1) // stride + 1
    y = torch.empty((n, co, ho, wo), device=xq.device, dtype=torch.float32, memory_format=torch.channels_last)
    tap = _tap_begin("avse_sconv_fwd", xq.device)
    check(_lib.lib().avse_sconv_fwd(n, h, wd, ci, co, stride, ptr(xq), ptr(xm), ptr(wq), ptr(wm), ptr(y),
                                    stream_ptr(xq.device)), "avse_sconv_fwd")
    _tap_end(tap)
    return y


def sconv_dgrad2_ok(xshape, cout):
    n, ci, h, w = xshape
    return bool(_lib.lib().avse_sconv_dgrad2_supported(n, h, w, ci, cout))


def sconv_dgrad2(dys, xshape, w):
    dyq, dym = dys
    _need_gpu(dyq, w)
    n, ci, h, wd = xshape
    co = w.shape[0]
    L = _lib.lib()
    wm = torch.empty(1, device=w.device, dtype=torch.int32)
    wq = torch.empty(int(L.avse_sconv_wprep_bytes(co, ci)), device=w.device, dtype=torch.uint8)
    check(L.avse_sconv_wprep(co, ci, ptr(w.float().contiguous()), 2, ptr(wq), ptr(wm), stream_ptr(w.device)),
          "avse_sconv_wprep")
    dx = torch.empty((n, ci, h, wd), device=dyq.device, dtype=torch.float32, memory_format=torch.channels_last)
    tap = _tap_begin("avse_sconv_dgrad2", dyq.device)
    check(L.avse_sconv_dgrad2(n, h, wd, ci, co, ptr(dyq), ptr(dym), ptr(wq), ptr(wm), ptr(dx), stream_ptr(dyq.device)),
          "avse_sconv_dgrad2")
    _tap_end(tap)
    return dx


def sconv_wgrad(xs, dys, xshape, cout, stride):
    (xq, xm), (dyq, dym) = xs, dys
    _need_gpu(xq, dyq)
    n, ci, h, wd = xshape
    L = _lib.lib()
    nb = L.avse_sconv_wgrad_workspace_bytes(n, h, wd, ci, cout, stride)
    if nb <= 0:
        raise RuntimeError(f"sconv_wgrad: unsupported shape {tuple(xshape)} -> {cout}, stride {stride}")
    dw = torch.empty((cout, ci, 3, 3), device=xq.device, dtype=torch.float32)
    ws = torch.empty((nb + 3) // 4, device=xq.device, dtype=torch.float32)
    tap = _tap_begin("avse_sconv_wgrad", xq.device)
    check(L.avse_sconv_wgrad(n, h, wd, ci, cout, stride, ptr(xq), ptr(xm), ptr(dyq), ptr(dym), ptr(dw), ptr(ws),
                             stream_ptr(xq.device)), "avse_sconv_wgrad")
    _tap_end(tap)
    return dw



def _ncs(x):
    N, C = x.shape[0], x.shape[1]
    S = x.numel() // max(1, N * C)
    return N, C, S


def _nhwc(x):
    if x.dim() != 4 or x.is_contiguous() or not x.is_contiguous(memory_format=torch.channels_last):
        return None
    C = x.shape[1]
    if C % 4 or 256 % (C // 4):
        return None
    return x.numel() // C, C


def prelu_fwd(x, a):
    _need_gpu(x, a)
    if x.dtype == torch.float32 and _nhwc(x) is not None:
        R, C = _nhwc(x)
        y = torch.empty_like(x)
        check(_lib.lib().avse_prelu_nhwc_fwd(R, C, a.numel(), ptr(x), ptr(a.contiguous()), ptr(y),
                                             stream_ptr(x.device)), "avse_prelu_nhwc_fwd")
        return y
    x = x.contiguous()
    if x.dtype != torch.float32:
        raise RuntimeError("prelu kernels are fp32")
    N, C, S = _ncs(x)
    y = torch.empty_like(x)
    check(_lib.lib().avse_prelu_fwd(N, C, S, a.numel(), ptr(x), ptr(a.contiguous()), ptr(y), stream_ptr(x.device)),
          "avse_prelu_fwd")
    return y


def prelu_bwd(x, a, dy):
    _need_gpu(x, a, dy)
    if x.dtype == torch.float32 and _nhwc(x) is not None:
        R, C = _nhwc(x)
        dy = dy.float().contiguous(memory_format=torch.channels_last)
        dx = torch.empty_like(x)
        da = torch.empty((a.numel(),), device=x.device, dtype=torch.float32)
# ... 99 lines not shown

def _q_ok(x, res):
    v = _bn_view(x)
    return (res is None and x.dim() == 4 and v is not None and v[2] == 1 and x.shape[1] % 64 == 0
            and not x.is_contiguous() and x.data_ptr() % 16 == 0)


def bnact_fwd(x, gamma, beta, running_mean, running_var, training, momentum, eps, act=ACT_NONE, alpha=None, res=None,
              q_out=False):
    _need_gpu(x)
    if x.dtype != torch.float32:
        raise RuntimeError("bnact kernels are fp32")
    if _bn_view(x) is None:
        x = x.contiguous()
    N, C, S = _bn_view(x)
    if res is not None:
        res = _same_layout(res.float(), x)
    y = torch.empty_like(x)
    stats = torch.empty((C, 4), device=x.device, dtype=torch.float32)
    L = _lib.lib()
    ws = torch.empty((L.avse_bnact_workspace_bytes(N, C, S) + 3) // 4, device=x.device, dtype=torch.float32)
    a = alpha.float().contiguous() if alpha is not None else None
    ymax = torch.empty(1, device=x.device, dtype=torch.int32)
    if q_out and training and _q_ok(x, res):
        check(L.avse_bnact_fwd_q(N, C, S, ptr(x), _opt(gamma), _opt(beta), int(act), _opt(a),
                                 a.numel() if a is not None else 0, float(eps), float(momentum), _opt(running_mean),
                                 _opt(running_var), ptr(stats), ptr(y), ptr(ws), ptr(ymax), stream_ptr(x.device)),
              "avse_bnact_fwd_q")
        _set_absmax(y, ymax)
        setattr(y, SPLITQ_ATTR, True)
        return y, stats
    check(L.avse_bnact_fwd(N, C, S, ptr(x), _opt(res), _opt(gamma), _opt(beta), int(act), _opt(a),
                           a.numel() if a is not None else 0, int(bool(training)), float(eps), float(momentum),
                           _opt(running_mean), _opt(running_var), ptr(stats), ptr(y), ptr(ws), ptr(ymax),
                           stream_ptr(x.device)), "avse_bnact_fwd")
    _set_absmax(y, ymax)
    return y, stats


ABSMAX_ATTR = "_avse_absmax"


def _set_absmax(t, mb):
    setattr(t, ABSMAX_ATTR, mb)


def _known_absmax(t):
    mb = getattr(t, ABSMAX_ATTR, None)
    return mb if isinstance(mb, torch.Tensor) and mb.device == t.device else None


def bnact_bwd(x, res, dy, stats, gamma, beta, act, alpha, training, q_out=False):
    _need_gpu(x, dy, stats)
    N, C, S = _bn_view(x)
    dy = _same_layout(dy.float(), x)
    if res is not None:
        res = _same_layout(res.float(), x)
    dx = torch.empty_like(x)
    dres = torch.empty_like(x) if res is not None else None
    dgamma = torch.empty((C,), device=x.device, dtype=torch.float32)
    dbeta = torch.empty((C,), device=x.device, dtype=torch.float32)
    a = alpha.float().contiguous() if alpha is not None else None
    dalpha_c = torch.empty((C,), device=x.device, dtype=torch.float32) if a is not None else None
    L = _lib.lib()
    ws = torch.empty((L.avse_bnact_workspace_bytes(N, C, S) + 3) // 4, device=x.device, dtype=torch.float32)
    dxmax = torch.empty(1, device=x.device, dtype=torch.int32)
    q = q_out and _q_ok(x, res) and dy.data_ptr() % 16 == 0
    if q:
        check(L.avse_bnact_bwd_q(N, C, S, ptr(x), ptr(dy), ptr(stats), _opt(gamma), _opt(beta), int(act), _opt(a),
                                 a.numel() if a is not None else 0, int(bool(training)), ptr(dx), ptr(dgamma),
                                 ptr(dbeta), _opt(dalpha_c), ptr(ws), ptr(dxmax), stream_ptr(x.device)),
              "avse_bnact_bwd_q")
        setattr(dx, SPLITQ_ATTR, True)
    else:
        check(L.avse_bnact_bwd(N, C, S, ptr(x), _opt(res), ptr(dy), ptr(stats), _opt(gamma), _opt(beta), int(act),
                               _opt(a), a.numel() if a is not None else 0, int(bool(training)), ptr(dx), _opt(dres),
                               ptr(dgamma), ptr(dbeta), _opt(dalpha_c), ptr(ws), ptr(dxmax), stream_ptr(x.device)),
              "avse_bnact_bwd")
    _set_absmax(dx, dxmax)
    dalpha = None
    if a is not None:
        dalpha = (dalpha_c if a.numel() == C else dalpha_c.sum().reshape(1)).view_as(alpha)
    return dx, dres, dgamma, dbeta, dalpha



def prelu_gln_fwd(x, alpha, gamma, beta, eps=1e-8):
    _need_gpu(x, alpha, gamma, beta)
    x = x.float().contiguous()
    Bn, C, Kn = x.shape
    y = torch.empty_like(x)
    stats = torch.empty((Bn, 2), device=x.device, dtype=torch.float32)
    L = _lib.lib()
    ws = torch.empty((L.avse_prelu_gln_workspace_bytes(Bn, C) + 3) // 4, device=x.device, dtype=torch.float32)
    tap = _tap_begin("avse_prelu_gln_fwd", x.device)
    check(L.avse_prelu_gln_fwd(Bn, C, Kn, ptr(x), ptr(alpha.float().contiguous()), ptr(gamma.float().contiguous()),
                               ptr(beta.float().contiguous()), float(eps), ptr(y), ptr(stats), ptr(ws),
                               stream_ptr(x.device)), "avse_prelu_gln_fwd")
    _tap_end(tap)
    return y, stats


def prelu_gln_bwd(x, alpha, gamma, stats, dy, planes=False):
    _need_gpu(x, alpha, gamma, stats, dy)
    x, dy = x.float().contiguous(), dy.float().contiguous()
    Bn, C, Kn = x.shape
    dalpha = torch.empty((1,), device=x.device, dtype=torch.float32)
    dgamma = torch.empty((C,), device=x.device, dtype=torch.float32)
    dbeta = torch.empty((C,), device=x.device, dtype=torch.float32)
    L = _lib.lib()
    ws = torch.empty((L.avse_prelu_gln_workspace_bytes(Bn, C) + 3) // 4, device=x.device, dtype=torch.float32)
    if planes:
        dx, sp, cp = _planes_carrier((Bn, C, Kn), x.device)
        tap = _tap_begin("avse_prelu_gln_bwd_q", x.device)
        check(L.avse_prelu_gln_bwd_q(Bn, C, Kn, ptr(x), ptr(alpha.float().contiguous()), ptr(gamma.float().contiguous()),
                                     ptr(stats), ptr(dy), ptr(sp.hi), ptr(sp.lo), cp, ptr(sp.mb), ptr(dalpha),
                                     ptr(dgamma), ptr(dbeta), ptr(ws), stream_ptr(x.device)), "avse_prelu_gln_bwd_q")
        _tap_end(tap)
        return dx, dalpha, dgamma, dbeta
    dx = torch.empty_like(x)
    tap = _tap_begin("avse_prelu_gln_bwd", x.device)
    check(L.avse_prelu_gln_bwd(Bn, C, Kn, ptr(x), ptr(alpha.float().contiguous()), ptr(gamma.float().contiguous()),
                               ptr(stats), ptr(dy), ptr(dx), ptr(dalpha), ptr(dgamma), ptr(dbeta), ptr(ws),
                               stream_ptr(x.device)), "avse_prelu_gln_bwd")
    _tap_end(tap)
    return dx, dalpha, dgamma, dbeta



def dwconv_fwd(x, w, dilation):
    _need_gpu(x, w)
    x = x.float().contiguous()
    Bn, C, Kn = x.shape
    w2 = w.reshape(C, -1).float().contiguous()
    y = torch.empty_like(x)
    check(_lib.lib().avse_dwconv_fwd(Bn, C, Kn, w2.shape[1], int(dilation), ptr(x), ptr(w2), ptr(y),
                                     stream_ptr(x.device)), "avse_dwconv_fwd")
    return y


def dwconv_bwd(x, w, dy, dilation):
    _need_gpu(x, w, dy)
    x, dy = x.float().contiguous(), dy.float().contiguous()
    Bn, C, Kn = x.shape
    w2 = w.reshape(C, -1).float().contiguous()
    P = w2.shape[1]
    dx = torch.empty_like(x)
    dw = torch.empty((C, P), device=x.device, dtype=torch.float32)
    L = _lib.lib()
    ws = torch.empty((L.avse_dwconv_bwd_workspace_bytes(Bn, C) + 3) // 4, device=x.device, dtype=torch.float32)
    check(L.avse_dwconv_bwd(Bn, C, Kn, P, int(dilation), ptr(x), ptr(w2), ptr(dy), ptr(dx), ptr(dw), ptr(ws),
                            stream_ptr(x.device)), "avse_dwconv_bwd")
    return dx, dw.view_as(w)



PLANES_ATTR = "_avse_planes"


def planes_of(t):
    return getattr(t, PLANES_ATTR, None)


def _planes_carrier(shape, device):
    b, r, c = shape
    cp = (c + 7) // 8 * 8
# ... 461 lines not shown
```

avse_challenge_amd/layers.py:

```python

import torch
import torch.nn as nn
import torch.nn.functional as F

from . import kernels as K


class _PReLUFn(torch.autograd.Function):
    @staticmethod
    def forward(ctx, x, a):
        ctx.save_for_backward(x, a)
        return K.prelu_fwd(x, a)

    @staticmethod
    def backward(ctx, dy):
        x, a = ctx.saved_tensors
        dx, da = K.prelu_bwd(x, a, dy)
        return dx, da


class PReLU(nn.Module):
    def __init__(self, num_parameters=1, init=0.25):
        super().__init__()
        self.num_parameters = num_parameters
        self.weight = nn.Parameter(torch.full((num_parameters,), init))

    def forward(self, x):
        if not x.is_cuda:
            raise RuntimeError("PReLU runs on the GPU kernels only")
        return _PReLUFn.apply(x, self.weight)


class _BNActFn(torch.autograd.Function):

    @staticmethod
    def forward(ctx, x, gamma, beta, alpha, res, running_mean, running_var, training, momentum, eps, act, q_fwd, q_bwd):
        if K._bn_view(x) is None:
            x = x.contiguous()
        y, stats = K.bnact_fwd(x, gamma, beta, running_mean, running_var, training, momentum, eps, act, alpha, res,
                               q_out=q_fwd)
        ctx.save_for_backward(x, res, stats, gamma, beta, alpha)
        ctx.act, ctx.training, ctx.q_bwd = act, training, q_bwd
        return y

    @staticmethod
    def backward(ctx, dy):
        x, res, stats, gamma, beta, alpha = ctx.saved_tensors
        dx, dres, dgamma, dbeta, dalpha = K.bnact_bwd(x, res, dy, stats, gamma, beta, ctx.act, alpha, ctx.training,
                                                      q_out=ctx.q_bwd)
        return (dx, dgamma if ctx.needs_input_grad[1] else None, dbeta if ctx.needs_input_grad[2] else None,
                dalpha if ctx.needs_input_grad[3] else None, dres, None, None, None, None, None, None, None, None)


def bn_act(x, bn, act=None, res=None, folded_bias=None, q_fwd=False, q_bwd=False):
    if folded_bias is not None:
        if not (bn.training and bn.track_running_stats) or res is not None or bn.momentum is None:
            raise RuntimeError("bn_act: folded_bias needs a training-mode BatchNorm with running stats and a momentum "
                               "(not the cumulative average), no residual")
        y = bn_act(x, bn, act, q_fwd=q_fwd, q_bwd=q_bwd)
        bn.running_mean.data.add_(folded_bias.detach(), alpha=bn.momentum)
        return y
    if not x.is_cuda:
        raise RuntimeError("bn_act runs on the GPU kernels only")
    training = bn.training or not bn.track_running_stats
    if bn.training and bn.track_running_stats:
        if bn.momentum is None:
            raise NotImplementedError("bn_act: cumulative-average BatchNorm (momentum=None)")
        bn.num_batches_tracked.add_(1)
    if act is None:
        code, alpha = K.ACT_NONE, None
    elif act == "relu":
        code, alpha = K.ACT_RELU, None
    else:
        code, alpha = K.ACT_PRELU, act.weight
    rm = bn.running_mean if bn.track_running_stats else None
    rv = bn.running_var if bn.track_running_stats else None
    return _BNActFn.apply(x.float(), bn.weight, bn.bias, alpha, res, rm, rv, training,
                          bn.momentum if bn.momentum is not None else 0.0, bn.eps, code, bool(q_fwd), bool(q_bwd))


class _MaxPoolPlanesFn(torch.autograd.Function):
    @staticmethod
    def forward(ctx, x, k, s, p):
        y, idx = K.maxpool_planes_fwd(x, k, s, p)
        ctx.save_for_backward(idx)
        ctx.cfg, ctx.in_shape = (k, s, p), x.shape
        return y

    @staticmethod
    def backward(ctx, dy):
        (idx,) = ctx.saved_tensors
        k, s, p = ctx.cfg
        return K.maxpool_planes_bwd(dy, idx, ctx.in_shape, k, s, p), None, None, None


def maxpool3d(x, pool):
    k, s, p = (tuple(v) if isinstance(v, (tuple, list)) else (v,) * 3 for v in (pool.kernel_size, pool.stride,
                                                                                 pool.padding))
    d = pool.dilation if isinstance(pool.dilation, (tuple, list)) else (pool.dilation,) * 3
    if k[0] != 1 or s[0] != 1 or p[0] != 0 or tuple(d) != (1, 1, 1) or pool.ceil_mode or pool.return_indices:
        raise NotImplementedError(f"maxpool3d: only (1, KH, KW) windows, got {pool}")
    if not x.is_cuda:
        raise RuntimeError("maxpool3d runs on the GPU kernels only")
    return _MaxPoolPlanesFn.apply(x, k[1:], s[1:], p[1:])


def _conv3d_fwd_folded(x, w, padding):
    B, Cin, T, H, W = x.shape
    Co, _, KT, KH, KW = w.shape
    PT, PH, PW = padding
    xp = F.pad(x, (0, 0, 0, 0, PT, PT))
    Tn = T + 2 * PT - KT + 1
    xu = xp.unfold(2, KT, 1)
    xu = xu.permute(0, 2, 1, 5, 3, 4).reshape(B * Tn, Cin * KT, H, W)
    y = F.conv2d(xu, w.reshape(Co, Cin * KT, KH, KW), None, (2, 2), (PH, PW))
    return y.view(B, Tn, Co, y.shape[-2], y.shape[-1]).transpose(1, 2).contiguous()


class _LipConv3dFn(torch.autograd.Function):

    @staticmethod
    def forward(ctx, x, w, stride, padding):
        hip = x.is_cuda and K.conv3d_fwd_supported(x, w, stride, padding)
        if not hip and x.dtype != torch.float32:
            x = x.float()
        ctx.stride, ctx.padding = stride, padding
        ctx.xmax = None
        if hip:
            y, xmax = K.conv3d_fwd(x, w, return_xmax=True)
            ctx.save_for_backward(x, w, xmax if xmax is not None else x.new_zeros(0, dtype=torch.int32))
            ctx.xmax = xmax is not None
            return y
        ctx.save_for_backward(x, w, x.new_zeros(0, dtype=torch.int32))
        if tuple(stride) == (1, 2, 2) and x.shape[1] == 3:
            return _conv3d_fwd_folded(x, w, padding)
        return F.conv3d(x, w, None, stride, padding)

    @staticmethod
    def backward(ctx, dy):
        x, w, xmax = ctx.saved_tensors
        dx = None
        if ctx.needs_input_grad[0]:
            dx = torch.nn.grad.conv3d_input(x.shape, w, dy, ctx.stride, ctx.padding)
        dw = None
        if ctx.needs_input_grad[1]:
            if dy.shape[-1] <= K.CONV3D_WGRAD_MAX_WO:
                dw = K.conv3d_wgrad(x, dy, tuple(w.shape[2:]), ctx.padding, xmax=xmax if ctx.xmax else None)
            else:
                dw = torch.nn.grad.conv3d_weight(x.float(), w.shape, dy, ctx.stride, ctx.padding)
        return dx, dw, None, None


class LipConv3d(nn.Conv3d):
    def __init__(self, cin, cout, kernel_size, stride=(1, 2, 2), padding=(2, 3, 3), bias=False):
        super().__init__(cin, cout, kernel_size, stride=stride, padding=padding, bias=bias)
        assert tuple(self.stride) == (1, 2, 2) and cout == 64 and not bias

    def forward(self, x):
        return _LipConv3dFn.apply(x, self.weight, tuple(self.stride), tuple(self.padding))


def _conv2d_dgrad(x, w, dy, stride, padding, dilation):
    pair = lambda v: [v, v] if isinstance(v, int) else list(v)
    return torch.ops.aten.convolution_backward(dy, x, w, None, pair(stride), pair(padding), pair(dilation), False,
                                               [0, 0], 1, [True, False, False])[0]




class _DilatedConvFn(torch.autograd.Function):

    @staticmethod
    def forward(ctx, x, w, b, dilation, add_bias):
        ctx.dilation = dilation
        ctx.split = K.dconv_split_ok(x, dilation)
        if K.is_split_q(x) and not ctx.split:
            raise RuntimeError("_DilatedConvFn: a split-output input needs the split path (DilatedConv2d.q_ok)")
        if ctx.split:
            mb = torch.empty(2, device=x.device, dtype=torch.int32)
            xq = K.split16(x, mb)
            mbd = torch.empty(2, device=x.device, dtype=torch.int32) if ctx.needs_input_grad[0] else None
            wq, wq_t = K.dconv_wprep2(w, mb, mbd)
            y = K.dconv_fwd(x, w, dilation, b if add_bias else None, split=(xq, mb), wq=wq)
            ctx.has_wt = wq_t is not None
            if ctx.has_wt:
                ctx.save_for_backward(xq, mb, w, wq_t, mbd)
            else:
                ctx.save_for_backward(xq, mb, w)
            ctx.shape = tuple(x.shape)
            return y
        ctx.save_for_backward(x, w)
        pad = 2 * dilation
        return F.conv2d(x, w, b if add_bias else None, 1, pad, dilation)

    @staticmethod
    def backward(ctx, dy):
        d = ctx.dilation
        dx = dw = db = None
        if ctx.split:
            if ctx.has_wt:
                xq, mb, w, wq_t, mbd = ctx.saved_tensors
            else:
                xq, mb, w = ctx.saved_tensors
                wq_t, mbd = None, torch.empty(2, device=dy.device, dtype=torch.int32)
            dyq = K.split16(dy, mbd)
            if ctx.needs_input_grad[0]:
                dx = K.dconv_fwd(dy, w, d, transposed=True, split=(dyq, mbd), wq=wq_t)
            if ctx.needs_input_grad[1] or ctx.needs_input_grad[2]:
                dw, db = K.dconv_wgrad16((xq, mb[:1]), (dyq, mbd[:1]), ctx.shape, d, bias_grad=True)
                dw = dw if ctx.needs_input_grad[1] else None
                db = db if ctx.needs_input_grad[2] else None
            return dx, dw, db, None, None
        x, w = ctx.saved_tensors
        if ctx.needs_input_grad[0]:
            dx = _conv2d_dgrad(x, w, dy, 1, 2 * d, d)
        if ctx.needs_input_grad[1] and ctx.needs_input_grad[2]:
            dw, db = K.dconv_wgrad(x, dy, d, bias_grad=True)
        elif ctx.needs_input_grad[1]:
            dw = K.dconv_wgrad(x, dy, d)
        elif ctx.needs_input_grad[2]:
            db = dy.sum((0, 2, 3))
        return dx, dw, db, None, None


class _FramesNHWC(torch.autograd.Function):

    @staticmethod
    def forward(ctx, x):
        B, C, T, H, W = x.shape
        ctx.shape = x.shape
        y = K.transpose_cp(x.contiguous().view(B, C, T * H * W))
        return y.view(B * T, H, W, C).permute(0, 3, 1, 2)

    @staticmethod
    def backward(ctx, dy):
        B, C, T, H, W = ctx.shape
        d = dy.permute(0, 2, 3, 1).contiguous().view(B, T * H * W, C)
        return K.transpose_cp(d).view(B, C, T, H, W)


def frames_nhwc(x):
    B, C, T, H, W = x.shape
    if x.is_cuda and x.dtype == torch.float32:
        return _FramesNHWC.apply(x)
    return x.permute(0, 2, 3, 4, 1).reshape(B * T, H, W, C).permute(0, 3, 1, 2)




class _Conv1Fn(torch.autograd.Function):

    @staticmethod
    def _rows(x):
        n, _, h, w = x.shape
        xp = F.pad(x.reshape(n, h, w), (2, 2, 2, 2))
        hp, wp = h + 4, w + 4
        a = x.new_empty((n, h, w, 26))
        a[..., :25].view(n, h, w, 5, 5).copy_(xp.as_strided((n, h, w, 5, 5), (hp * wp, wp, 1, wp, 1)))
        a[..., 25] = 1.0
        return a.view(n * h * w, 26)

    @staticmethod
    def forward(ctx, x, w, b, add_bias):
        n, _, h, ww = x.shape
        ctx.hip = ww >= 128
        if ctx.hip:
            ctx.save_for_backward(x, w)
            return K.conv1_fwd(x, w, b if add_bias else None)
        a = _Conv1Fn._rows(x)
        wb = torch.cat([w.reshape(w.shape[0], 25), (b if add_bias else torch.zeros_like(b)).reshape(-1, 1)], 1)
        y = a @ wb.t()
        ctx.save_for_backward(a, w)
        ctx.shape = (n, h, ww)
        return y.view(n, h, ww, -1).permute(0, 3, 1, 2)

    @staticmethod
    def backward(ctx, dy):
        if ctx.hip:
            x, w = ctx.saved_tensors
            dx, dw, db = K.conv1_bwd(x, w, dy, ctx.needs_input_grad[0],
                                     ctx.needs_input_grad[1] or ctx.needs_input_grad[2])
            return (dx, dw if ctx.needs_input_grad[1] else None, db if ctx.needs_input_grad[2] else None, None)
        a, w = ctx.saved_tensors
        n, h, ww = ctx.shape
        cout = w.shape[0]
        dy2 = dy.permute(0, 2, 3, 1).reshape(-1, cout)
        dx = dw = db = None
        if ctx.needs_input_grad[1] or ctx.needs_input_grad[2]:
            g = dy2.t() @ a
# ... 126 lines not shown
    @staticmethod
    def backward(ctx, dy):
        cols, wm = ctx.saved_tensors
        B, T, C, k, dil, has_b = ctx.shape
        pad = (k - 1) * dil
        To = T + pad
        Co = wm.shape[0]
        dy2 = dy.reshape(B * To, Co)
        if _f32s_rows_ok(cols, dy2):
            sd = K.split_planes(dy2[None])
            dw = K.gemm_f32s_rows_tn(K.split_planes(cols[None]), sd, B).view(Co, k, C).permute(0, 2, 1)
            dcols = K.gemm_f32s_split(K.split_planes(wm[None]).t(), sd,
                                      torch.empty((1, B * To, k * C), device=dy.device, dtype=torch.float32))
            dcols = dcols.view(B, To, k, C)
        else:
            dw = (dy2.t() @ cols).view(Co, k, C).permute(0, 2, 1)
            dcols = (dy2 @ wm).view(B, To, k, C)
        db = dy2.sum(0) if has_b else None
        dxp = torch.zeros((B, T + 2 * pad, C), device=dy.device, dtype=dy.dtype)
        for j in range(k):
            dxp[:, j * dil:j * dil + To] += dcols[:, :, j]
        return dxp[:, pad:pad + T], dw, db, None


class _ConvFFn(torch.autograd.Function):

    @staticmethod
    def forward(ctx, x, w, b):
        ctx.save_for_backward(x, w)
        ctx.has_b = b is not None
        return K.convf_fwd(x, w, b)

    @staticmethod
    def backward(ctx, dy):
        x, w = ctx.saved_tensors
        need_w = ctx.needs_input_grad[1] or (ctx.has_b and ctx.needs_input_grad[2])
        dx, dw, db = K.convf_bwd(x, w, dy, need_dx=ctx.needs_input_grad[0], need_dw=need_w)
        return dx, dw if ctx.needs_input_grad[1] else None, db if ctx.has_b and ctx.needs_input_grad[2] else None


def conv1x1_to4(x, conv):
    if (x.is_cuda and x.dtype == torch.float32 and conv.weight.dtype == torch.float32 and x.dim() == 4
            and x.shape[1] == 64 and tuple(conv.weight.shape) == (4, 64, 1, 1) and conv.stride == (1, 1)
            and conv.padding == (0, 0) and conv.groups == 1 and x.is_contiguous(memory_format=torch.channels_last)
            and x.data_ptr() % 16 == 0):
        return _ConvFFn.apply(x, conv.weight, conv.bias)
    return conv(x)


def _f32s_rows_ok(a, b):
    return (a.is_cuda and a.dtype == b.dtype == torch.float32 and a.dim() == b.dim() == 2 and a.shape[0] == b.shape[0]
            and a.stride(1) == 1 and b.stride(1) == 1 and a.stride(0) % 8 == 0 and b.stride(0) % 8 == 0)


def time_conv1d(x, conv):
    assert conv.stride == (1,) and conv.groups == 1 and conv.padding == ((conv.kernel_size[0] - 1) * conv.dilation[0],)
    return _TimeConv1dFn.apply(x, conv.weight, conv.bias, conv.dilation[0])


def time_major_4d(x):
    B, T, C = x.shape
    return x.as_strided((B, C, T, 1), (T * C, 1, C, C))


class PointwiseConv2d(nn.Conv2d):

    def __init__(self, cin, cout, stride=1):
        super().__init__(cin, cout, 1, stride=stride, bias=False)

    def forward(self, x):
        if gemm_conv_ok(x, 1, self.stride[0]):
            return _GemmConvFn.apply(x, self.weight, self.stride[0])
        return super().forward(x)




class _SConvFn(torch.autograd.Function):

    @staticmethod
    def forward(ctx, x, w, stride):
        xq, xm = K.split_q(x)
        ctx.shape, ctx.stride = tuple(x.shape), stride
        ctx.save_for_backward(xq, xm, w)
        return K.sconv_fwd((xq, xm), ctx.shape, w, stride)

    @staticmethod
    def backward(ctx, dy):
        xq, xm, w = ctx.saved_tensors
        s, shape = ctx.stride, ctx.shape
        dyq, dym = K.split_q(dy)
        dx = dw = None
        if ctx.needs_input_grad[0]:
            if s == 1:
                dx = K.sconv_fwd((dyq, dym), tuple(dy.shape), w, 1, transposed=True)
            else:
                dx = K.sconv_dgrad2((dyq, dym), shape, w)
        if ctx.needs_input_grad[1]:
            dw = K.sconv_wgrad((xq, xm), (dyq, dym), shape, w.shape[0], s)
        return dx, dw, None


class TrunkConv2d(nn.Conv2d):

    def __init__(self, cin, cout, stride=1):
        super().__init__(cin, cout, 3, stride=stride, padding=1, bias=False)

    def _sconv(self, x):
        return (x.is_contiguous(memory_format=torch.channels_last) and x.dtype == self.weight.dtype
                and K.sconv_ok(x, self.out_channels, self.stride[0])
                and (self.stride[0] == 1 or K.sconv_dgrad2_ok(tuple(x.shape), self.out_channels)))

    def q_ok(self, x, grad=False):
        return self._sconv(x)

    def forward(self, x):
        if self._sconv(x):
            return _SConvFn.apply(x, self.weight, self.stride[0])
        return super().forward(x)


class _PReluGLNFn(torch.autograd.Function):
    @staticmethod
    def forward(ctx, x, alpha, gamma, beta, eps, planes_bwd=False):
        y, stats = K.prelu_gln_fwd(x, alpha, gamma.reshape(-1), beta.reshape(-1), eps)
        ctx.save_for_backward(x, alpha, gamma, stats)
        ctx.planes_bwd = planes_bwd
        return y

    @staticmethod
    def backward(ctx, dy):
        x, alpha, gamma, stats = ctx.saved_tensors
        dx, da, dg, db = K.prelu_gln_bwd(x, alpha, gamma.reshape(-1), stats, dy, planes=ctx.planes_bwd)
        return dx, da.view_as(alpha), dg.view_as(gamma), db.view_as(gamma), None, None


def prelu_gln(x, alpha, gamma, beta, eps=1e-8, planes_bwd=False):
    if not x.is_cuda:
        raise RuntimeError("prelu_gln runs on the GPU kernels only")
    return _PReluGLNFn.apply(x, alpha, gamma, beta, eps, planes_bwd)


class _DWConvGLNFn(torch.autograd.Function):

    @staticmethod
    def forward(ctx, x, w, alpha, gamma, beta, dilation, eps, planes=False):
        y, y1, stats = K.dwconv_gln_fwd(x, w, dilation, alpha, gamma.reshape(-1), beta.reshape(-1), eps, planes)
        ctx.save_for_backward(x, w, y1, alpha, gamma, stats)
        ctx.dilation = dilation
        return y

    @staticmethod
    def backward(ctx, dy):
        x, w, y1, alpha, gamma, stats = ctx.saved_tensors
        dx, dw, da, dg, db = K.dwconv_gln_bwd(x, w, ctx.dilation, y1, alpha, gamma.reshape(-1), stats, dy)
        return dx, dw, da.view_as(alpha), dg.view_as(gamma), db.view_as(gamma), None, None, None


def dwconv_prelu_gln(x, w, alpha, gamma, beta, dilation, eps=1e-8, planes=False):
    if not x.is_cuda:
        raise RuntimeError("dwconv_prelu_gln runs on the GPU kernels only")
    return _DWConvGLNFn.apply(x, w, alpha, gamma, beta, dilation, eps, planes)


class _DWConvFn(torch.autograd.Function):
    @staticmethod
    def forward(ctx, x, w, dilation):
        ctx.save_for_backward(x, w)
        ctx.dilation = dilation
        return K.dwconv_fwd(x, w, dilation)

    @staticmethod
    def backward(ctx, dy):
        x, w = ctx.saved_tensors
        dx, dw = K.dwconv_bwd(x, w, dy, ctx.dilation)
        return dx, dw, None

# ... 64 lines not shown
```

include/avse_hip.h:

```cpp
#ifndef AVSE_HIP_H
#define AVSE_HIP_H

#include <stdint.h>

#ifdef __cplusplus
extern "C" {
#endif

typedef void* avse_stream_t;

enum { AVSE_OK = 0, AVSE_EINVAL = -1, AVSE_ESHAPE = -2, AVSE_EDTYPE = -3, AVSE_ELAUNCH = -4, AVSE_EALIGN = -5,
       AVSE_ENORESIDENT = -6 };
enum { AVSE_F32 = 0, AVSE_BF16 = 1, AVSE_U8 = 2 };

const char* avse_strerror(int code);
int avse_abi_version(void);

typedef struct {
    int64_t batch, dim, seqlen, dstate;
    int32_t in_dtype;
    int32_t delta_softplus;
    int32_t reverse;
    const void* u;      int64_t u_bs, u_ds;
    const void* delta;  int64_t delta_bs, delta_ds;
// ... 71 lines not shown
                        uint16_t* out, int64_t out_bs, int64_t out_ds, int32_t silu, int32_t reverse,
                        avse_stream_t stream);
int avse_cconv_bwd_bf16(int64_t batch, int64_t dim, int64_t seqlen, int64_t width,
                        const uint16_t* x, int64_t x_bs, int64_t x_ds,
                        const float* weight, const float* bias,
                        const uint16_t* dout, int64_t dout_bs, int64_t dout_ds,
                        uint16_t* dx, int64_t dx_bs, int64_t dx_ds,
                        float* dweight, float* dbias,
                        int32_t silu, int32_t reverse, float* workspace, int32_t dx_accumulate, uint32_t* dx_max,
                        avse_stream_t stream);

int avse_add_rmsnorm_fwd(int64_t rows, int64_t n, const float* h, const float* res_in ,
                         const float* weight, float eps, float* y, float* res_out, float* rstd, uint32_t* y_max,
                         avse_stream_t stream);
int64_t avse_rmsnorm_bwd_workspace_bytes(int64_t rows, int64_t n);
int avse_rmsnorm_bwd(int64_t rows, int64_t n, const float* dy, const float* dres_out ,
                     const float* res_out, const float* weight, const float* rstd,
                     float* dx, float* dweight, float* workspace, uint32_t* dx_max, avse_stream_t stream);
int avse_add_rmsnorm_fwd2(int64_t rows, int64_t n, const void* h, int32_t h_dtype, const float* res_in ,
                          const float* weight, float eps, void* y, int32_t y_dtype, float* res_out, float* rstd,
                          uint32_t* y_max, avse_stream_t stream);
int avse_rmsnorm_bwd2(int64_t rows, int64_t n, const void* dy, int32_t dy_dtype, const float* dres_out ,
                      const float* res_out, const float* weight, const float* rstd, float* dx, float* dweight,
                      float* workspace, uint32_t* dx_max, avse_stream_t stream);

int64_t avse_stft_frames(int64_t T);
int avse_stft_fwd(int64_t batch, int64_t T, const float* wave, float* mag, float* spec_or_null,
                  avse_stream_t stream);
int avse_istft(int64_t batch, int64_t frames, int64_t length, const float* mag, const float* phase_spec,
               float* frames_buf, float* wave_out, avse_stream_t stream);

int64_t avse_conv3d_fwd_workspace_bytes(int64_t CIN, int64_t H, int64_t W);
int avse_conv3d_fwd(int64_t B, int64_t CIN, int64_t T, int64_t H, int64_t W, int32_t x_dtype, const void* x,
                    const float* w, float* y, float* workspace, avse_stream_t stream);

int64_t avse_conv3d_wgrad_workspace_bytes(int64_t B, int64_t TO, int64_t HO, int64_t N);
int avse_conv3d_wgrad(int64_t B, int64_t CIN, int64_t T, int64_t H, int64_t W, int64_t KT, int64_t KH, int64_t KW,
                      int64_t PT, int64_t PH, int64_t PW, const float* x, const float* dy, float* dw,
                      int32_t accumulate, float* workspace, avse_stream_t stream);
int avse_conv3d_wgrad_u8_split(int64_t B, int64_t CIN, int64_t T, int64_t H, int64_t W, int64_t KT, int64_t KH,
                               int64_t KW, int64_t PT, int64_t PH, int64_t PW, const uint8_t* x, const float* dy,
                               const uint32_t* dymax, float* dw, int32_t accumulate, float* workspace,
                               avse_stream_t stream);
int avse_conv3d_wgrad_split(int64_t B, int64_t CIN, int64_t T, int64_t H, int64_t W, int64_t KT, int64_t KH,
                            int64_t KW, int64_t PT, int64_t PH, int64_t PW, const float* x, const uint32_t* xmax,
                            const float* dy, const uint32_t* dymax, float* dw, int32_t accumulate, float* workspace,
                            avse_stream_t stream);
int avse_conv3d_wgrad_u8(int64_t B, int64_t CIN, int64_t T, int64_t H, int64_t W, int64_t KT, int64_t KH, int64_t KW,
                         int64_t PT, int64_t PH, int64_t PW, const uint8_t* x, const float* dy, float* dw,
                         int32_t accumulate, float* workspace, avse_stream_t stream);

int64_t avse_dconv_wgrad_workspace_bytes(int64_t N, int64_t H, int64_t W, int64_t dil);
int avse_dconv_wgrad(int64_t N, int64_t H, int64_t W, int64_t dil, const float* x, const float* dy, float* dw,
                     float* db, float* workspace, avse_stream_t stream);

int avse_prelu_fwd(int64_t N, int64_t C, int64_t S, int32_t num_params, const float* x, const float* a, float* y,
                   avse_stream_t stream);
int64_t avse_prelu_bwd_workspace_bytes(int64_t N, int64_t C);
int avse_prelu_bwd(int64_t N, int64_t C, int64_t S, int32_t num_params, const float* x, const float* a,
                   const float* dy, float* dx, float* da, float* workspace, avse_stream_t stream);
int avse_prelu_nhwc_fwd(int64_t R, int64_t C, int32_t num_params, const float* x, const float* a, float* y,
                        avse_stream_t stream);
int64_t avse_prelu_nhwc_bwd_workspace_bytes(int64_t R, int64_t C);
int avse_prelu_nhwc_bwd(int64_t R, int64_t C, int32_t num_params, const float* x, const float* a, const float* dy,
                        float* dx, float* da, float* workspace, avse_stream_t stream);

int64_t avse_bnact_workspace_bytes(int64_t N, int64_t C, int64_t S);
int avse_bnact_fwd(int64_t N, int64_t C, int64_t S, const float* x, const float* res, const float* gamma,
                   const float* beta, int32_t act, const float* alpha, int32_t alpha_n, int32_t training, float eps,
                   float momentum, float* running_mean, float* running_var, float* stats, float* y, float* workspace,
                   uint32_t* y_max, avse_stream_t stream);
int avse_bnact_bwd(int64_t N, int64_t C, int64_t S, const float* x, const float* res, const float* dy, const float* stats,
                   const float* gamma, const float* beta, int32_t act, const float* alpha, int32_t alpha_n,
                   int32_t training, float* dx, float* dres, float* dgamma, float* dbeta, float* dalpha_c,
                   float* workspace, uint32_t* dx_max, avse_stream_t stream);
int avse_bnact_fwd_q(int64_t N, int64_t C, int64_t S, const float* x, const float* gamma, const float* beta, int32_t act,
                     const float* alpha, int32_t alpha_n, float eps, float momentum, float* running_mean,
                     float* running_var, float* stats, void* yq, float* workspace, uint32_t* y_bound,
                     avse_stream_t stream);
int avse_bnact_bwd_q(int64_t N, int64_t C, int64_t S, const float* x, const float* dy, const float* stats,
                     const float* gamma, const float* beta, int32_t act, const float* alpha, int32_t alpha_n,
                     int32_t training, void* dxq, float* dgamma, float* dbeta, float* dalpha_c, float* workspace,
                     uint32_t* dx_bound, avse_stream_t stream);

int64_t avse_maxpool2d_out_size(int64_t H, int64_t K, int64_t S, int64_t P);
int avse_maxpool2d_fwd(int64_t planes, int64_t H, int64_t W, int64_t KH, int64_t KW, int64_t SH, int64_t SW, int64_t PH,
                       int64_t PW, const float* x, float* y, uint8_t* idx, avse_stream_t stream);
int avse_maxpool2d_bwd(int64_t planes, int64_t H, int64_t W, int64_t KH, int64_t KW, int64_t SH, int64_t SW, int64_t PH,
                       int64_t PW, const float* dy, const uint8_t* idx, float* dx, avse_stream_t stream);

int avse_transpose_cp(int64_t N, int64_t C, int64_t P, const float* x, float* y, avse_stream_t stream);

int64_t avse_prelu_gln_workspace_bytes(int64_t B, int64_t C);
int avse_prelu_gln_fwd(int64_t B, int64_t C, int64_t K, const float* x, const float* alpha, const float* gamma,
                       const float* beta, float eps, float* y, float* stats, float* workspace, avse_stream_t stream);
int avse_prelu_gln_bwd(int64_t B, int64_t C, int64_t K, const float* x, const float* alpha, const float* gamma,
                       const float* stats, const float* dy, float* dx, float* dalpha, float* dgamma, float* dbeta,
                       float* workspace, avse_stream_t stream);
int avse_prelu_gln_bwd_q(int64_t B, int64_t C, int64_t K, const float* x, const float* alpha, const float* gamma,
                         const float* stats, const float* dy, void* dx_hi, void* dx_lo, int64_t kp, uint32_t* dx_maxbits,
                         float* dalpha, float* dgamma, float* dbeta, float* workspace, avse_stream_t stream);

int64_t avse_dwconv_bwd_workspace_bytes(int64_t B, int64_t C);
int avse_dwconv_fwd(int64_t B, int64_t C, int64_t K, int64_t P, int64_t dil, const float* x, const float* w, float* y,
                    avse_stream_t stream);
int avse_dwconv_bwd(int64_t B, int64_t C, int64_t K, int64_t P, int64_t dil, const float* x, const float* w,
                    const float* dy, float* dx, float* dw, float* workspace, avse_stream_t stream);

int64_t avse_dwconv_gln_workspace_bytes(int64_t B, int64_t C);
int avse_dwconv_gln_fwd(int64_t B, int64_t C, int64_t K, int64_t P, int64_t dil, const float* x, const float* w,
                        const float* alpha, const float* gamma, const float* beta, float eps, float* y1, float* y,
                        float* stats, float* workspace, avse_stream_t stream);
int avse_dwconv_gln_fwd_q(int64_t B, int64_t C, int64_t K, int64_t P, int64_t dil, const float* x, const float* w,
                          const float* alpha, const float* gamma, const float* beta, float eps, float* y1, void* y_hi,
                          void* y_lo, int64_t kp, uint32_t* y_maxbits, float* stats, float* workspace,
                          avse_stream_t stream);
int avse_dwconv_gln_bwd(int64_t B, int64_t C, int64_t K, int64_t P, int64_t dil, const float* x, const float* w,
                        const float* y1, const float* alpha, const float* gamma, const float* stats, const float* dy,
                        float* dx, float* dw, float* dalpha, float* dgamma, float* dbeta, float* workspace,
                        avse_stream_t stream);

int64_t avse_lstm_padded_hidden(int64_t H);
int avse_lstm_fwd(int64_t B, int64_t T, int64_t H, int32_t reverse, const float* gx, const float* whhT, float* hout,
                  int64_t hout_bs, int64_t hout_ts, float* c_all, float* gates, avse_stream_t stream);
int avse_lstm_bwd(int64_t B, int64_t T, int64_t H, int32_t reverse, const float* dh_out, int64_t dh_bs, int64_t dh_ts,
                  const float* gates, const float* c_all, const float* whh_pad, float* dgates, avse_stream_t stream);
int64_t avse_lstm_group_size(int64_t B, int64_t H);
int64_t avse_lstm_group_workspace_bytes(int64_t B, int64_t H);
int64_t avse_lstm_group_capacity(int64_t H, int32_t backward);
int avse_lstm_fwd_group(int64_t B, int64_t T, int64_t H, int32_t reverse, const float* gx, const float* whh,
                        float* hout, int64_t hout_bs, int64_t hout_ts, float* c_all, float* gates, void* workspace,
                        uint32_t* error_flag, avse_stream_t stream);
int avse_lstm_bwd_group(int64_t B, int64_t T, int64_t H, int32_t reverse, const float* dh_out, int64_t dh_bs,
                        int64_t dh_ts, const float* gates, const float* c_all, const float* whh, float* dgates,
                        void* workspace, uint32_t* error_flag, avse_stream_t stream);

typedef struct {
    int64_t batch, mp, mq, k, fold;
    const void* p;  int64_t p_bs, p_sx, p_sk, p_extent;
    const void* q;  int64_t q_bs, q_sx, q_sk, q_extent;
    void* c;        int64_t c_bs, c_sq;
    float alpha;
    int32_t c_dtype;
} avse_gemm_bf16_args;
int avse_gemm_bf16(const avse_gemm_bf16_args* a, avse_stream_t stream);

typedef struct {
    int64_t batch, mp, mq, k, fold;
    const void* p_hi; const void* p_lo;  int64_t p_bs, p_sx, p_sk, p_extent;  const uint32_t* p_max;
    const void* q_hi; const void* q_lo;  int64_t q_bs, q_sx, q_sk, q_extent;  const uint32_t* q_max;
    float* c;       int64_t c_bs, c_sq;
    float alpha;
    int64_t nsub, p_bs2, q_bs2;
} avse_gemm_f32s_args;
int avse_gemm_f32s(const avse_gemm_f32s_args* a, avse_stream_t stream);
int avse_split16_planes(int64_t b, int64_t r, int64_t c, const float* x, int64_t x_bs, int64_t x_rs, void* hi, void* lo,
                        uint32_t* maxbits, avse_stream_t stream);
int avse_add_max(int64_t rows, int64_t lp, int64_t l, const float* a, const float* b, float* y, uint32_t* maxbits,
                 avse_stream_t stream);
int avse_split16_planes_known(int64_t b, int64_t r, int64_t c, const float* x, int64_t x_bs, int64_t x_rs, void* hi,
                              void* lo, const uint32_t* maxbits, avse_stream_t stream);
int avse_split16_planes_to(int64_t b, int64_t r, int64_t c, const float* x, int64_t x_bs, int64_t x_rs, void* hi,
                           void* lo, int64_t h_bs, int64_t h_rs, uint32_t* maxbits, int32_t known, avse_stream_t stream);

int64_t avse_dconv_wprep_bytes(void);
int avse_split16(int64_t n_pix, const float* x, void* xq, uint32_t* maxbits, avse_stream_t stream);
int avse_split16_known(int64_t n_pix, const float* x, void* xq, const uint32_t* maxbits, avse_stream_t stream);
int avse_dconv_wprep(const float* w, int32_t transposed, void* wq, uint32_t* maxbits, avse_stream_t stream);
int avse_dconv_wprep2(const float* w, void* wq, void* wq_t, uint32_t* maxbits, uint32_t* maxbits_t,
                      avse_stream_t stream);

int avse_conv1_fwd(int64_t N, int64_t H, int64_t W, const float* x, const float* w, const float* b, float* y,
                   avse_stream_t stream);
int avse_conv1_dgrad(int64_t N, int64_t H, int64_t W, const float* dy, const float* w, float* dx, avse_stream_t stream);
int64_t avse_conv1_wgrad_workspace_bytes(int64_t N, int64_t H, int64_t W);
int avse_conv1_wgrad(int64_t N, int64_t H, int64_t W, const float* x, const float* dy, float* dw, float* db,
                     float* workspace, avse_stream_t stream);
int avse_convf_fwd(int64_t npix, const float* x, const float* w, const float* b, float* y, avse_stream_t stream);
int avse_convf_dgrad(int64_t npix, const float* dy, const float* w, float* dx, avse_stream_t stream);
int64_t avse_convf_wgrad_workspace_bytes(int64_t npix);
int avse_convf_wgrad(int64_t npix, const float* x, const float* dy, float* dw, float* db, float* workspace,
                     avse_stream_t stream);

int64_t avse_sconv_wprep_bytes(int64_t co, int64_t ci);
int avse_sconv_wprep(int64_t co, int64_t ci, const float* w, int32_t transposed, void* wq, uint32_t* wmax,
                     avse_stream_t stream);
int avse_sconv_fwd(int64_t N, int64_t Hi, int64_t Wi, int64_t ci, int64_t co, int64_t stride, const void* xq,
                   const uint32_t* xmax, const void* wq, const uint32_t* wmax, float* y, avse_stream_t stream);
int64_t avse_sconv_wgrad_workspace_bytes(int64_t N, int64_t Hi, int64_t Wi, int64_t ci, int64_t co, int64_t stride);
int avse_sconv_dgrad2_supported(int64_t N, int64_t Hi, int64_t Wi, int64_t ci, int64_t co);
int avse_sconv_dgrad2(int64_t N, int64_t Hi, int64_t Wi, int64_t ci, int64_t co, const void* dyq,
                      const uint32_t* dymax, const void* wq, const uint32_t* wmax, float* dx, avse_stream_t stream);
int avse_sconv_wgrad(int64_t N, int64_t Hi, int64_t Wi, int64_t ci, int64_t co, int64_t stride, const void* xq,
                     const uint32_t* xmax, const void* dyq, const uint32_t* dymax, float* dw, float* workspace,
                     avse_stream_t stream);
int avse_dconv_fwd(int64_t N, int64_t H, int64_t W, int64_t dil, const void* xq, const void* wq,
                   const uint32_t* maxbits, const float* bias, float* y, avse_stream_t stream);
int64_t avse_dconv_wgrad16_workspace_bytes(int64_t N, int64_t H, int64_t W);
int avse_dconv_wgrad16(int64_t N, int64_t H, int64_t W, int64_t dil, const void* xq, const uint32_t* xmax,
                       const void* dyq, const uint32_t* dymax, float* dw, float* db, float* workspace,
                       avse_stream_t stream);

#ifdef __cplusplus
}
#endif
#endif
```

Measured before the change: 439.0 utt/s.

## Fuse BN+activation backward partial reductions into conv dgrad epilogues

Adds an epilogue to the dilated-conv and strided-conv data-gradient kernels. While the gradient is still in registers, the epilogue reloads the BN input and computes per-block partial sums for the following BN+ReLU/PReLU backward (sum dz, sum dz*xhat, the PReLU term, optional max). The BN backward then skips its own full reduction pass over x and dy, and only combines the per-row partials and applies. This removes one read of two activation-sized tensors per paired layer. In exchange it adds autograd pairing state (matched by pointer and version), extra workspace, and more register and LDS pressure in the conv kernels.

```diff
diff --git a/avse_challenge_amd/_lib.py b/avse_challenge_amd/_lib.py
--- a/avse_challenge_amd/_lib.py
+++ b/avse_challenge_amd/_lib.py
@@ -134,6 +134,13 @@
                                  c_vp, c_vp, c_vp, c_vp, c_vp]),
     "avse_bnact_bwd_q": (c_i32, [c_i64, c_i64, c_i64, c_vp, c_vp, c_vp, c_vp, c_vp, c_i32, c_vp, c_i32, c_i32, c_vp,
                                  c_vp, c_vp, c_vp, c_vp, c_vp, c_vp]),
+    "avse_bnact_rows_workspace_bytes": (c_i64, [c_i64, c_i64, c_i64]),
+    "avse_bnact_bwd_rows": (c_i32, [c_i64, c_i64, c_i64, c_vp, c_vp, c_vp, c_vp, c_vp, c_i32, c_vp, c_i32, c_i32, c_vp,
+                                    c_vp, c_vp, c_vp, c_vp, c_vp, c_i32, c_vp]),
+    "avse_dconv_bn_rows": (c_i64, [c_i64] * 4),
+    "avse_dconv_dgrad_bn": (c_i32, [c_i64] * 4 + [c_vp] * 8 + [c_i32, c_i32, c_vp, c_vp]),
+    "avse_sconv_bn_rows": (c_i64, [c_i64] * 4),
+    "avse_sconv_dgrad1_bn": (c_i32, [c_i64] * 5 + [c_vp] * 9 + [c_i32, c_vp, c_i32, c_i32, c_vp, c_vp]),
     "avse_prelu_nhwc_fwd": (c_i32, [c_i64, c_i64, c_i32, c_vp, c_vp, c_vp, c_vp]),
     "avse_prelu_nhwc_bwd_workspace_bytes": (c_i64, [c_i64, c_i64]),
     "avse_prelu_nhwc_bwd": (c_i32, [c_i64, c_i64, c_i32, c_vp, c_vp, c_vp, c_vp, c_vp, c_vp, c_vp]),
diff --git a/avse_challenge_amd/csrc/bnact.hip b/avse_challenge_amd/csrc/bnact.hip
--- a/avse_challenge_amd/csrc/bnact.hip
+++ b/avse_challenge_amd/csrc/bnact.hip
@@ -1,12 +1,12 @@
 #include <algorithm>
 
+#include "bnact_cols.h"
 #include "common.h"
 
 namespace avse {
 namespace bnact {
 
 constexpr int THREADS = 256;
-enum { ACT_NONE = 0, ACT_RELU = 1, ACT_PRELU = 2 };
 
 struct Geo {
     int64_t N, CS, S;
@@ -27,39 +27,6 @@
         *reinterpret_cast<float4*>(p) = make_float4(v[0], v[1], v[2], v[3]);
     }
 };
-
-template <int V, int ACT>
-struct ColConst {
-    float a[V], b[V], al[V], mean[V], mlo[V], rstd[V], gam[V];
-    __device__ inline float centred(float v, int k) const { return (v - mean[k]) - mlo[k]; }
-    __device__ inline void load(const Geo& g, int64_t j0, const float* stats, const float* gamma, const float* beta,
-                                const float* alpha, int alpha_n) {
-#pragma unroll
-        for (int k = 0; k < V; ++k) {
-            const int c = (int)((j0 + k) / g.S);
-            mean[k] = stats[4 * c];
-            mlo[k] = stats[4 * c + 1];
-            rstd[k] = stats[4 * c + 2];
-            gam[k] = gamma ? gamma[c] : 1.f;
-            a[k] = gam[k] * rstd[k];
-            b[k] = beta ? beta[c] : 0.f;
-            al[k] = ACT == ACT_PRELU ? alpha[alpha_n > 1 ? c : 0] : 0.f;
-        }
-    }
-};
-
-template <int ACT>
-__device__ inline float act_fwd(float z, float al) {
-    if constexpr (ACT == ACT_RELU) return z > 0.f ? z : 0.f;
-    else if constexpr (ACT == ACT_PRELU) return z > 0.f ? z : al * z;
-    else return z;
-}
-template <int ACT>
-__device__ inline float act_bwd(float z, float g, float al) {
-    if constexpr (ACT == ACT_RELU) return z > 0.f ? g : 0.f;
-    else if constexpr (ACT == ACT_PRELU) return z > 0.f ? g : al * g;
-    else return g;
-}
 
 template <int V, int NQ, int MAXQ = -1>
 __device__ inline void block_partials(const Geo& g, float (&p)[NQ][V], bool valid, int64_t j0, float* ws) {
@@ -271,7 +238,7 @@
                 float v[V];
                 vld<V>::ld(x + r * g.CS + j0, v);
 #pragma unroll
-                for (int k = 0; k < V; ++k) v[k] = act_fwd<ACT>(fmaf(cc.centred(v[k], k), cc.a[k], cc.b[k]), cc.al[k]);
+                for (int k = 0; k < V; ++k) v[k] = act_fwd<ACT>(cc.preact(v[k], k), cc.al[k]);
                 q_store4(reinterpret_cast<uint16_t*>(y), r, g.CS, j0, v, sc);
             }
         }
@@ -287,7 +254,7 @@
             if (RES) vld<V>::ld(res + o, rv);
 #pragma unroll
             for (int k = 0; k < V; ++k) {
-                float z = fmaf(cc.centred(v[k], k), cc.a[k], cc.b[k]);
+                float z = cc.preact(v[k], k);
                 if (RES) z += rv[k];
                 v[k] = act_fwd<ACT>(z, cc.al[k]);
                 m = fmaxf(m, fabsf(v[k]));
@@ -325,10 +292,10 @@
             if (RES) vld<V>::ld(res + o, rv);
 #pragma unroll
             for (int k = 0; k < V; ++k) {
-                float z = fmaf(cc.centred(v[k], k), cc.a[k], cc.b[k]);
+                float z = cc.preact(v[k], k);
                 if (RES) z += rv[k];
                 dz[k] = act_bwd<ACT>(z, gv[k], cc.al[k]);
-                const float xh = cc.centred(v[k], k) * cc.rstd[k];
+                const float xh = cc.xhat(v[k], k);
                 p[0][k] += dz[k];
                 p[1][k] = fmaf(dz[k], xh, p[1][k]);
                 if (ACT == ACT_PRELU && !(z > 0.f)) p[2][k] = fmaf(gv[k], z, p[2][k]);
@@ -394,11 +361,11 @@
             float gv[V];
             vld<V>::ld(dy + o, gv);
 #pragma unroll
-            for (int k = 0; k < V; ++k) dz[k] = act_bwd<ACT>(fmaf(cc.centred(v[k], k), cc.a[k], cc.b[k]), gv[k], cc.al[k]);
+            for (int k = 0; k < V; ++k) dz[k] = act_bwd<ACT>(cc.preact(v[k], k), gv[k], cc.al[k]);
         }
 #pragma unroll
         for (int k = 0; k < V; ++k) {
-            const float xh = cc.centred(v[k], k) * cc.rstd[k];
+            const float xh = cc.xhat(v[k], k);
             v[k] = cc.a[k] * (dz[k] - k1[k] - xh * k2[k]);
             if constexpr (!QOUT) m = fmaxf(m, fabsf(v[k]));
         }
@@ -618,4 +585,51 @@
                           nullptr, dgamma, dbeta, dalpha_c, workspace, dx_bound, true, (hipStream_t)stream);
 }
 
-}
+static inline int64_t rows_floats(int64_t rows, int64_t C, int64_t nq) { return rows * nq * C; }
+
+int64_t avse_bnact_rows_workspace_bytes(int64_t rows, int64_t C, int64_t nq) {
+    if (rows <= 0 || rows >= (1 << 23) || C <= 0 || C >= (1 << 20) || (nq != 3 && nq != 4)) return 0;
+    return 4 * (rows_floats(rows, C, nq) + 2 * C) + 16 + 8 * C * MAXG * 4;
+}
+
+int avse_bnact_bwd_rows(int64_t N, int64_t C, int64_t rows, const float* x, const float* dy, const float* stats,
+                        const float* gamma, const float* beta, int32_t act, const float* alpha, int32_t alpha_n,
+                        int32_t training, float* dx, float* dgamma, float* dbeta, float* dalpha_c, float* workspace,
+                        uint32_t* dx_max, int32_t q_out, avse_stream_t stream) {
+    hipStream_t st = (hipStream_t)stream;
+    if (!x || !dy || !stats || !dx || !workspace || !dx_max || (act == ACT_PRELU && (!alpha || !dalpha_c)))
+        return AVSE_EINVAL;
+    if (!shape_ok(N, C, 1) || act < ACT_NONE || act > ACT_PRELU) return AVSE_ESHAPE;
+    if (act == ACT_PRELU && alpha_n != 1 && alpha_n != C) return AVSE_ESHAPE;
+    if (rows <= 0 || rows >= (1 << 23)) return AVSE_ESHAPE;
+    if (C % 4 || !al16(x) || !al16(dy) || !al16(dx) || !al16(workspace)) return AVSE_EALIGN;
+    if (q_out && C % 64) return AVSE_ESHAPE;
+    const int nq = q_out ? 4 : 3;
+    const Geo g = make_geo(N, C, 1, 4);
+    Geo gr = g;
+    gr.nrb = (int)rows;
+    float* kbuf = workspace + rows_floats(rows, C, nq);
+    double* fin = reinterpret_cast<double*>(((uintptr_t)(kbuf + 2 * C) + 15) & ~(uintptr_t)15);
+    const int G = chan_groups(gr);
+    if (q_out)
+        hipLaunchKernelGGL((chan_partial_kernel<4, 3>), dim3((unsigned)C, G), dim3(THREADS), 0, st, gr,
+                           (const float*)workspace, fin, dx_max);
+    else
+        hipLaunchKernelGGL((chan_partial_kernel<3>), dim3((unsigned)C, G), dim3(THREADS), 0, st, gr,
+                           (const float*)workspace, fin, (uint32_t*)nullptr);
+    AVSE_CHECK_LAUNCH();
+    hipLaunchKernelGGL(bwd_combine, dim3((unsigned)((C + 255) / 256)), dim3(256), 0, st, g, (const double*)fin, G,
+                       (int)training, dgamma, dbeta, dalpha_c, kbuf, dx_max, (int)(q_out != 0), stats, gamma);
+    AVSE_CHECK_LAUNCH();
+    const dim3 grid(g.tiles, g.nrb);
+    if (q_out)
+        dispatch_q<BwdApplyQK>::run(act, grid, st, g, x, dy, (const float*)nullptr, stats, gamma, beta, alpha,
+                                   (int)alpha_n, (const float*)kbuf, dx, dx_max);
+    else
+        dispatch<BwdApplyK>::run(4, act, false, grid, st, g, x, dy, (const float*)nullptr, stats, gamma, beta, alpha,
+                                 (int)alpha_n, (const float*)kbuf, dx, dx_max);
+    AVSE_CHECK_LAUNCH();
+    return AVSE_OK;
+}
+
+}
diff --git a/avse_challenge_amd/csrc/bnact_cols.h b/avse_challenge_amd/csrc/bnact_cols.h
--- /dev/null
+++ b/avse_challenge_amd/csrc/bnact_cols.h
@@ -0,0 +1,123 @@
+#pragma once
+
+#include "common.h"
+
+namespace avse {
+namespace bnact {
+
+enum { ACT_NONE = 0, ACT_RELU = 1, ACT_PRELU = 2 };
+
+template <int V, int ACT>
+struct ColConst {
+    float a[V], b[V], al[V], mean[V], mlo[V], rstd[V], gam[V];
+    __device__ inline float centred(float v, int k) const { return (v - mean[k]) - mlo[k]; }
+    __device__ inline float preact(float v, int k) const { return fmaf(centred(v, k), a[k], b[k]); }
+    __device__ inline float xhat(float v, int k) const { return centred(v, k) * rstd[k]; }
+    __device__ inline void load_channel(int k, int c, const float* stats, const float* gamma, const float* beta,
+                                        const float* alpha, int alpha_n) {
+        mean[k] = stats[4 * c];
+        mlo[k] = stats[4 * c + 1];
+        rstd[k] = stats[4 * c + 2];
+        gam[k] = gamma ? gamma[c] : 1.f;
+        a[k] = gam[k] * rstd[k];
+        b[k] = beta ? beta[c] : 0.f;
+        al[k] = ACT == ACT_PRELU ? alpha[alpha_n > 1 ? c : 0] : 0.f;
+    }
+    template <class G>
+    __device__ inline void load(const G& g, int64_t j0, const float* stats, const float* gamma, const float* beta,
+                                const float* alpha, int alpha_n) {
+#pragma unroll
+        for (int k = 0; k < V; ++k) load_channel(k, (int)((j0 + k) / g.S), stats, gamma, beta, alpha, alpha_n);
+    }
+};
+
+template <int ACT>
+__device__ inline float act_fwd(float z, float al) {
+    if constexpr (ACT == ACT_RELU) return z > 0.f ? z : 0.f;
+    else if constexpr (ACT == ACT_PRELU) return z > 0.f ? z : al * z;
+    else return z;
+}
+template <int ACT>
+__device__ inline float act_bwd(float z, float g, float al) {
+    if constexpr (ACT == ACT_RELU) return z > 0.f ? g : 0.f;
+    else if constexpr (ACT == ACT_PRELU) return z > 0.f ? g : al * g;
+    else return g;
+}
+
+struct BnEpi {
+    const float* x;
+    const float* stats;
+    const float* gamma;
+    const float* beta;
+    const float* alpha;
+    int alpha_n;
+    float* rows;
+};
+
+template <int ACT, bool MAXDZ, class F, class ST>
+__device__ inline void bn_epi_wave(const BnEpi& b, F dyv, ST store, int64_t pix0, int64_t npix, int ch0, int C,
+                                   int lane, float* part) {
+    constexpr int NQ = MAXDZ ? 4 : 3;
+    const uint64_t xa = (uint64_t)(b.x + pix0 * C + ch0);
+    const int64_t left = ((npix - pix0) * C - ch0) * 4;
+    const __amdgpu_buffer_rsrc_t rx = __builtin_amdgcn_make_buffer_rsrc(
+        (void*)(((uint64_t)(uint32_t)__builtin_amdgcn_readfirstlane((int)(xa >> 32)) << 32) |
+                (uint32_t)__builtin_amdgcn_readfirstlane((int)(uint32_t)xa)),
+        0, __builtin_amdgcn_readfirstlane((int)(left < 0 ? 0 : (left > 0x7FFFFFF0LL ? 0x7FFFFFF0LL : left))), 0x00020000);
+#pragma unroll
+    for (int j = 0; j < 2; ++j) {
+        const int o = ch0 + 32 * j + (lane & 31);
+        ColConst<1, ACT> cc;
+        cc.load_channel(0, o, b.stats, b.gamma, b.beta, b.alpha, b.alpha_n);
+        float s[4] = {0.f, 0.f, 0.f, 0.f};
+        float xv[2][4][4];
+        const int voff = (4 * (lane >> 5) * C + 32 * j + (lane & 31)) * 4;
+#pragma unroll
+        for (int i = 0; i < 2; ++i)
+#pragma unroll
+            for (int g = 0; g < 4; ++g)
+#pragma unroll
+                for (int e = 0; e < 4; ++e)
+                    xv[i][g][e] = __builtin_bit_cast(
+                        float, __builtin_amdgcn_raw_buffer_load_b32(rx, voff + (32 * i + 8 * g + e) * C * 4, 0, 0));
+        store(j);
+#pragma unroll
+        for (int i = 0; i < 2; ++i)
+#pragma unroll
+            for (int g = 0; g < 4; ++g)
+#pragma unroll
+                for (int e = 0; e < 4; ++e) {
+                    const bool in = pix0 + 32 * i + 8 * g + 4 * (lane >> 5) + e < npix;
+                    const float gv = in ? dyv(i, j, 4 * g + e) : 0.f;
+                    const float z = cc.preact(xv[i][g][e], 0);
+                    const float dz = act_bwd<ACT>(z, gv, cc.al[0]);
+                    s[0] += dz;
+                    s[1] = fmaf(dz, cc.xhat(xv[i][g][e], 0), s[1]);
+                    if constexpr (ACT == ACT_PRELU) s[2] = fmaf(z > 0.f ? 0.f : gv, z, s[2]);
+                    if constexpr (MAXDZ) s[3] = fmaxf(s[3], fabsf(dz));
+                }
+#pragma unroll
+        for (int q = 0; q < NQ; ++q) {
+            const float t = __shfl_xor(s[q], 32, 64);
+            const float v = (MAXDZ && q == 3) ? fmaxf(s[q], t) : s[q] + t;
+            if (lane < 32) part[q * 64 + 32 * j + lane] = v;
+        }
+    }
+}
+
+template <bool MAXDZ>
+__device__ inline void bn_epi_row(const BnEpi& b, const float* part, int nwm, int nwn, int64_t row, int ch0, int C) {
+    constexpr int NQ = MAXDZ ? 4 : 3;
+    for (int t = threadIdx.x; t < NQ * 64 * nwn; t += blockDim.x) {
+        const int c = t % (64 * nwn), q = t / (64 * nwn), wn = c >> 6, cl = c & 63;
+        float v = part[(wn * NQ + q) * 64 + cl];
+        for (int wm = 1; wm < nwm; ++wm) {
+            const float u = part[((wm * nwn + wn) * NQ + q) * 64 + cl];
+            v = (MAXDZ && q == 3) ? fmaxf(v, u) : v + u;
+        }
+        b.rows[(row * NQ + q) * C + ch0 + c] = v;
+    }
+}
+
+}
+}
diff --git a/avse_challenge_amd/csrc/dconv.hip b/avse_challenge_amd/csrc/dconv.hip
--- a/avse_challenge_amd/csrc/dconv.hip
+++ b/avse_challenge_amd/csrc/dconv.hip
@@ -1,5 +1,6 @@
 #include <algorithm>
 
+#include "bnact_cols.h"
 #include "common.h"
 
 namespace avse {
@@ -75,9 +76,10 @@
     const float* bias;
     float* y;
     int N, H, W, tiles;
+    bnact::BnEpi bn;
 };
 
-template <int D, int NW, int WGS = 1>
+template <int D, int NW, int WGS = 1, int EPI = 0>
 __global__ __launch_bounds__(64 * NW, WGS) void fwd_kernel(Args a) {
     constexpr int TPX = 64 * NW, NSEG = NW == 4 ? 2 : 3;
     constexpr int NP = (TPX + 4 * D * NSEG + 15) / 16 * 16;
@@ -204,8 +206,7 @@
     }
 
     const float scale = __builtin_ldexpf(1.f, -(split_exp(a.maxbits[0]) + split_exp(a.maxbits[1])));
-#pragma unroll
-    for (int j = 0; j < 2; ++j) {
+    auto store = [&](int j) {
         const int o = 32 * j + (lane & 31);
         const float bv = a.bias ? a.bias[o] : 0.f;
 #pragma unroll
@@ -215,8 +216,23 @@
 #pragma unroll
                 for (int e = 0; e < 4; ++e) {
                     const int p = p0 + 64 * wave + 32 * i + 8 * g + 4 * (lane >> 5) + e;
-                    if (p < HW) a.y[((int64_t)n * HW + p) * C + o] = acc[i][j][4 * g + e] * scale + bv;
+                    const float v = acc[i][j][4 * g + e] * scale + bv;
+                    if constexpr (EPI != 0) acc[i][j][4 * g + e] = v;
+                    if (p < HW) a.y[((int64_t)n * HW + p) * C + o] = v;
                 }
+    };
+    if constexpr (EPI == 0) {
+#pragma unroll
+        for (int j = 0; j < 2; ++j) store(j);
+    } else {
+        constexpr int ENQ = EPI == 2 ? 4 : 3;
+        float* part = reinterpret_cast<float*>(lds);
+        __syncthreads();
+        bnact::bn_epi_wave<bnact::ACT_RELU, EPI == 2>(
+            a.bn, [&](int i, int j, int r) { return acc[i][j][r]; }, store, (int64_t)n * HW + p0 + 64 * wave,
+            (int64_t)(n + 1) * HW, 0, C, lane, part + wave * ENQ * 64);
+        __syncthreads();
+        bnact::bn_epi_row<EPI == 2>(a.bn, part, NW, 1, (int64_t)bid, 0, C);
     }
 }
 
@@ -641,8 +657,42 @@
     return AVSE_OK;
 }
 
+static inline int dcf_nw(int64_t dil) { return dil <= 8 ? 4 : 8; }
+
+int64_t avse_dconv_bn_rows(int64_t N, int64_t H, int64_t W, int64_t dil) {
+    if (N <= 0 || H <= 0 || W < 256) return 0;
+    return N * ((H * W + 64 * dcf_nw(dil) - 1) / (64 * dcf_nw(dil)));
+}
+
+static int dconv_launch(int64_t N, int64_t H, int64_t W, int64_t dil, const void* xq, const void* wq,
+                        const uint32_t* maxbits, const float* bias, float* y, const avse::bnact::BnEpi* bn, int epi,
+                        avse_stream_t stream);
+
 int avse_dconv_fwd(int64_t N, int64_t H, int64_t W, int64_t dil, const void* xq, const void* wq,
                    const uint32_t* maxbits, const float* bias, float* y, avse_stream_t stream) {
+    return dconv_launch(N, H, W, dil, xq, wq, maxbits, bias, y, nullptr, 0, stream);
+}
+
+int avse_dconv_dgrad_bn(int64_t N, int64_t H, int64_t W, int64_t dil, const void* dyq, const void* wq_t,
+                        const uint32_t* maxbits, float* dx, const float* bn_x, const float* bn_stats,
+                        const float* gamma, const float* beta, int32_t act, int32_t want_max, float* rows,
+                        avse_stream_t stream) {
+    if (!bn_x || !bn_stats || !rows) return AVSE_EINVAL;
+    if (act != avse::bnact::ACT_RELU) return AVSE_ESHAPE;
+    avse::bnact::BnEpi bn;
+    bn.x = bn_x;
+    bn.stats = bn_stats;
+    bn.gamma = gamma;
+    bn.beta = beta;
+    bn.alpha = nullptr;
+    bn.alpha_n = 0;
+    bn.rows = rows;
+    return dconv_launch(N, H, W, dil, dyq, wq_t, maxbits, nullptr, dx, &bn, want_max ? 2 : 1, stream);
+}
+
+static int dconv_launch(int64_t N, int64_t H, int64_t W, int64_t dil, const void* xq, const void* wq,
+                        const uint32_t* maxbits, const float* bias, float* y, const avse::bnact::BnEpi* bn, int epi,
+                        avse_stream_t stream) {
     if (!xq || !wq || !maxbits || !y) return AVSE_EINVAL;
     if (N <= 0 || H <= 0 || W < 256 || (dil != 2 && dil != 4 && dil != 8 && dil != 16)) return AVSE_ESHAPE;
     if (N * H * W * 256 >= (1LL << 31) - 1024) return AVSE_ESHAPE;
@@ -655,16 +705,23 @@
     a.N = (int)N;
     a.H = (int)H;
     a.W = (int)W;
-    const int nw = dil <= 8 ? 4 : 8;
+    const int nw = dcf_nw(dil);
+    if (bn) a.bn = *bn;
+    else a.bn = avse::bnact::BnEpi{nullptr, nullptr, nullptr, nullptr, nullptr, 0, nullptr};
     a.tiles = (int)((H * W + 64 * nw - 1) / (64 * nw));
     const dim3 grid((unsigned)(N * a.tiles)), block(64 * nw);
     hipStream_t st = (hipStream_t)stream;
-    switch (dil) {
-        case 2: hipLaunchKernelGGL((fwd_kernel<2, 4, 2>), grid, block, 0, st, a); break;
-        case 4: hipLaunchKernelGGL((fwd_kernel<4, 4, 2>), grid, block, 0, st, a); break;
-        case 8: hipLaunchKernelGGL((fwd_kernel<8, 4, 2>), grid, block, 0, st, a); break;
-        default: hipLaunchKernelGGL((fwd_kernel<16, 8>), grid, block, 0, st, a); break;
-    }
+#define AVSE_DCF_CASES(E)                                                                           \
+    switch (dil) {                                                                                  \
+        case 2: hipLaunchKernelGGL((fwd_kernel<2, 4, 2, E>), grid, block, 0, st, a); break;         \
+        case 4: hipLaunchKernelGGL((fwd_kernel<4, 4, 2, E>), grid, block, 0, st, a); break;         \
+        case 8: hipLaunchKernelGGL((fwd_kernel<8, 4, 2, E>), grid, block, 0, st, a); break;         \
+        default: hipLaunchKernelGGL((fwd_kernel<16, 8, 1, E>), grid, block, 0, st, a); break;       \
+    }
+    if (epi == 0) { AVSE_DCF_CASES(0) }
+    else if (epi == 1) { AVSE_DCF_CASES(1) }
+    else { AVSE_DCF_CASES(2) }
+#undef AVSE_DCF_CASES
     AVSE_CHECK_LAUNCH();
     return AVSE_OK;
 }
diff --git a/avse_challenge_amd/csrc/sconv.hip b/avse_challenge_amd/csrc/sconv.hip
--- a/avse_challenge_amd/csrc/sconv.hip
+++ b/avse_challenge_amd/csrc/sconv.hip
@@ -1,5 +1,6 @@
 #include <algorithm>
 
+#include "bnact_cols.h"
 #include "common.h"
 
 namespace avse {
@@ -62,9 +63,10 @@
     int N, Hi, Wi, Ci, Ho, Wo, Co;
     int tiles_n;
     int RS, npos;
+    bnact::BnEpi bn;
 };
 
-template <int S, int TN>
+template <int S, int TN, int EPI = 0>
 __global__ __launch_bounds__(512, 1) void fwd_kernel(FArgs a) {
     constexpr int WAVES = 8, WN = TN / 64, WM = WAVES / WN, TM = 64 * WM;
     constexpr int WIMG = 3 * TN * ROWB;
@@ -180,8 +182,7 @@
     }
 
     const float scale = __builtin_ldexpf(1.f, -(split_exp(*a.xmax) + split_exp(*a.wmax)));
-#pragma unroll
-    for (int j = 0; j < 2; ++j) {
+    auto store = [&](int j) {
         const int o = o0 + 64 * wn + 32 * j + (lane & 31);
 #pragma unroll
         for (int i = 0; i < 2; ++i)
@@ -190,8 +191,23 @@
 #pragma unroll
                 for (int e = 0; e < 4; ++e) {
                     const int p = p0 + 64 * wm + 32 * i + 8 * g + 4 * (lane >> 5) + e;
-                    if (p < NHWo) a.y[(int64_t)p * a.Co + o] = acc[i][j][4 * g + e] * scale;
+                    const float v = acc[i][j][4 * g + e] * scale;
+                    if constexpr (EPI != 0) acc[i][j][4 * g + e] = v;
+                    if (p < NHWo) a.y[(int64_t)p * a.Co + o] = v;
                 }
+    };
+    if constexpr (EPI == 0) {
+#pragma unroll
+        for (int j = 0; j < 2; ++j) store(j);
+    } else {
+        constexpr int ENQ = EPI == 2 ? 4 : 3;
+        float* part = reinterpret_cast<float*>(lds);
+        __syncthreads();
+        bnact::bn_epi_wave<bnact::ACT_PRELU, EPI == 2>(
+            a.bn, [&](int i, int j, int r) { return acc[i][j][r]; }, store, (int64_t)p0 + 64 * wm, (int64_t)NHWo,
+            o0 + 64 * wn, a.Co, lane, part + wave * ENQ * 64);
+        __syncthreads();
+        bnact::bn_epi_row<EPI == 2>(a.bn, part, WM, WN, (int64_t)tm, o0, a.Co);
     }
 }
 
@@ -759,8 +775,41 @@
     return AVSE_OK;
 }
 
+static int sconv_launch(int64_t N, int64_t Hi, int64_t Wi, int64_t ci, int64_t co, int64_t stride, const void* xq,
+                        const uint32_t* xmax, const void* wq, const uint32_t* wmax, float* y,
+                        const avse::bnact::BnEpi* bn, int epi, avse_stream_t stream);
+
 int avse_sconv_fwd(int64_t N, int64_t Hi, int64_t Wi, int64_t ci, int64_t co, int64_t stride, const void* xq,
                    const uint32_t* xmax, const void* wq, const uint32_t* wmax, float* y, avse_stream_t stream) {
+    return sconv_launch(N, Hi, Wi, ci, co, stride, xq, xmax, wq, wmax, y, nullptr, 0, stream);
+}
+
+int64_t avse_sconv_bn_rows(int64_t N, int64_t H, int64_t W, int64_t co) {
+    if (N <= 0 || H <= 0 || W <= 0 || co <= 0 || co % 64) return 0;
+    const int64_t TM = co % 128 ? 512 : 256;
+    return (N * H * W + TM - 1) / TM;
+}
+
+int avse_sconv_dgrad1_bn(int64_t N, int64_t H, int64_t W, int64_t ci, int64_t co, const void* dyq,
+                         const uint32_t* dymax, const void* wq_t, const uint32_t* wmax, float* dx, const float* bn_x,
+                         const float* bn_stats, const float* gamma, const float* beta, int32_t act, const float* alpha,
+                         int32_t alpha_n, int32_t want_max, float* rows, avse_stream_t stream) {
+    if (!bn_x || !bn_stats || !rows || !alpha) return AVSE_EINVAL;
+    if (act != avse::bnact::ACT_PRELU || (alpha_n != 1 && alpha_n != co)) return AVSE_ESHAPE;
+    avse::bnact::BnEpi bn;
+    bn.x = bn_x;
+    bn.stats = bn_stats;
+    bn.gamma = gamma;
+    bn.beta = beta;
+    bn.alpha = alpha;
+    bn.alpha_n = alpha_n;
+    bn.rows = rows;
+    return sconv_launch(N, H, W, ci, co, 1, dyq, dymax, wq_t, wmax, dx, &bn, want_max ? 2 : 1, stream);
+}
+
+static int sconv_launch(int64_t N, int64_t Hi, int64_t Wi, int64_t ci, int64_t co, int64_t stride, const void* xq,
+                        const uint32_t* xmax, const void* wq, const uint32_t* wmax, float* y,
+                        const avse::bnact::BnEpi* bn, int epi, avse_stream_t stream) {
     if (!xq || !xmax || !wq || !wmax || !y) return AVSE_EINVAL;
     if (N <= 0 || Hi <= 0 || Wi <= 0 || ci <= 0 || co <= 0 || ci % 64 || co % 64 || (stride != 1 && stride != 2))
         return AVSE_ESHAPE;
@@ -771,6 +820,8 @@
     a.xmax = xmax;
     a.wmax = wmax;
     a.y = y;
+    if (bn) a.bn = *bn;
+    else a.bn = avse::bnact::BnEpi{nullptr, nullptr, nullptr, nullptr, nullptr, 0, nullptr};
     a.N = (int)N;
     a.Hi = (int)Hi;
     a.Wi = (int)Wi;
@@ -789,7 +840,12 @@
     if (tiles >= (1LL << 31)) return AVSE_ESHAPE;
     const dim3 grid((unsigned)tiles), block(512);
     hipStream_t st = (hipStream_t)stream;
-    if (stride == 1) {
+    if (epi != 0) {
+        if (TN == 64 && epi == 1) hipLaunchKernelGGL((fwd_kernel<1, 64, 1>), grid, block, 0, st, a);
+        else if (TN == 64) hipLaunchKernelGGL((fwd_kernel<1, 64, 2>), grid, block, 0, st, a);
+        else if (epi == 1) hipLaunchKernelGGL((fwd_kernel<1, 128, 1>), grid, block, 0, st, a);
+        else hipLaunchKernelGGL((fwd_kernel<1, 128, 2>), grid, block, 0, st, a);
+    } else if (stride == 1) {
         if (TN == 64) hipLaunchKernelGGL((fwd_kernel<1, 64>), grid, block, 0, st, a);
         else hipLaunchKernelGGL((fwd_kernel<1, 128>), grid, block, 0, st, a);
     } else {
diff --git a/avse_challenge_amd/kernels.py b/avse_challenge_amd/kernels.py
--- a/avse_challenge_amd/kernels.py
+++ b/avse_challenge_amd/kernels.py
@@ -540,6 +540,39 @@
     return y
 
 
+def _bn_rows_ws(rows, C, q_out, device):
+    nq = 4 if q_out else 3
+    nb = int(_lib.lib().avse_bnact_rows_workspace_bytes(rows, C, nq))
+    if rows <= 0 or nb <= 0:
+        raise RuntimeError(f"bnact rows workspace: unsupported rows {rows} x {C} channels")
+    return torch.empty((nb + 3) // 4, device=device, dtype=torch.float32)
+
+
+def bn_rows_ok(bn_x, gamma, beta, alpha):
+    return (bn_x.is_cuda and bn_x.dtype == torch.float32 and bn_x.dim() == 4 and bn_x.shape[1] % 64 == 0
+            and not bn_x.is_contiguous() and bn_x.is_contiguous(memory_format=torch.channels_last)
+            and bn_x.data_ptr() % 16 == 0
+            and all(t is None or (t.dtype == torch.float32 and t.is_contiguous()) for t in (gamma, beta, alpha)))
+
+
+def dconv_dgrad_bn(shape, dilation, split, wq_t, bn_x, stats, gamma, beta, act, q_out):
+    dyq, maxbits = split
+    _need_gpu(dyq, wq_t, bn_x, stats)
+    N, _, H, W = shape
+    if tuple(bn_x.shape) != tuple(shape) or act != ACT_RELU or not bn_rows_ok(bn_x, gamma, beta, None):
+        raise RuntimeError(f"dconv_dgrad_bn: unsupported BatchNorm input {tuple(bn_x.shape)} act {act}")
+    L = _lib.lib()
+    rows = int(L.avse_dconv_bn_rows(N, H, W, dilation))
+    ws = _bn_rows_ws(rows, 64, q_out, bn_x.device)
+    dx = torch.empty((N, 64, H, W), device=bn_x.device, dtype=torch.float32, memory_format=torch.channels_last)
+    tap = _tap_begin("avse_dconv_fwd", bn_x.device)
+    check(L.avse_dconv_dgrad_bn(N, H, W, dilation, ptr(dyq), ptr(wq_t), ptr(maxbits), ptr(dx), ptr(bn_x), ptr(stats),
+                                _opt(gamma), _opt(beta), int(act), int(bool(q_out)), ptr(ws), stream_ptr(bn_x.device)),
+          "avse_dconv_dgrad_bn")
+    _tap_end(tap)
+    return dx, rows, ws
+
+
 def dconv_wgrad16(xs, dys, shape, dilation, bias_grad=False):
     (xq, xm), (dyq, dym) = xs, dys
     _need_gpu(xq, dyq)
@@ -683,6 +716,29 @@
                                     stream_ptr(xq.device)), "avse_sconv_fwd")
     _tap_end(tap)
     return y
+
+
+def sconv_dgrad1_bn(dys, dyshape, w, bn_x, stats, gamma, beta, act, alpha, q_out):
+    dyq, dym = dys
+    _need_gpu(dyq, w, bn_x, stats)
+    n, ci, h, wd = dyshape
+    co = w.shape[1]
+    a = alpha
+    if (tuple(bn_x.shape) != (n, co, h, wd) or act != ACT_PRELU or a is None or a.numel() not in (1, co)
+            or not bn_rows_ok(bn_x, gamma, beta, a)):
+        raise RuntimeError(f"sconv_dgrad1_bn: unsupported BatchNorm input {tuple(bn_x.shape)} act {act}")
+    L = _lib.lib()
+    rows = int(L.avse_sconv_bn_rows(n, h, wd, co))
+    ws = _bn_rows_ws(rows, co, q_out, bn_x.device)
+    wm = torch.empty(1, device=w.device, dtype=torch.int32)
+    wq = sconv_wprep(w, True, wm)
+    dx = torch.empty((n, co, h, wd), device=dyq.device, dtype=torch.float32, memory_format=torch.channels_last)
+    tap = _tap_begin("avse_sconv_fwd", dyq.device)
+    check(L.avse_sconv_dgrad1_bn(n, h, wd, ci, co, ptr(dyq), ptr(dym), ptr(wq), ptr(wm), ptr(dx), ptr(bn_x),
+                                 ptr(stats), _opt(gamma), _opt(beta), int(act), ptr(a), a.numel(), int(bool(q_out)),
+                                 ptr(ws), stream_ptr(dyq.device)), "avse_sconv_dgrad1_bn")
+    _tap_end(tap)
+    return dx, rows, ws
 
 
 def sconv_dgrad2_ok(xshape, cout):
@@ -948,6 +1004,30 @@
     if a is not None:
         dalpha = (dalpha_c if a.numel() == C else dalpha_c.sum().reshape(1)).view_as(alpha)
     return dx, dres, dgamma, dbeta, dalpha
+
+
+def bnact_bwd_rows(x, dy, stats, gamma, beta, act, alpha, training, rows, ws, q_out=False):
+    _need_gpu(x, dy, stats, ws)
+    N, C, S = _bn_view(x)
+    if S != 1 or dy.stride() != x.stride() or dy.dtype != torch.float32:
+        raise RuntimeError("bnact_bwd_rows: channels-last fp32 x and dy of one layout")
+    dx = torch.empty_like(x)
+    dgamma = torch.empty((C,), device=x.device, dtype=torch.float32)
+    dbeta = torch.empty((C,), device=x.device, dtype=torch.float32)
+    a = alpha.float().contiguous() if alpha is not None else None
+    dalpha_c = torch.empty((C,), device=x.device, dtype=torch.float32) if a is not None else None
+    dxmax = torch.empty(1, device=x.device, dtype=torch.int32)
+    check(_lib.lib().avse_bnact_bwd_rows(N, C, int(rows), ptr(x), ptr(dy), ptr(stats), _opt(gamma), _opt(beta),
+                                         int(act), _opt(a), a.numel() if a is not None else 0, int(bool(training)),
+                                         ptr(dx), ptr(dgamma), ptr(dbeta), _opt(dalpha_c), ptr(ws), ptr(dxmax),
+                                         int(bool(q_out)), stream_ptr(x.device)), "avse_bnact_bwd_rows")
+    if q_out:
+        setattr(dx, SPLITQ_ATTR, True)
+    _set_absmax(dx, dxmax)
+    dalpha = None
+    if a is not None:
+        dalpha = (dalpha_c if a.numel() == C else dalpha_c.sum().reshape(1)).view_as(alpha)
+    return dx, None, dgamma, dbeta, dalpha
 
 
 
diff --git a/avse_challenge_amd/layers.py b/avse_challenge_amd/layers.py
--- a/avse_challenge_amd/layers.py
+++ b/avse_challenge_amd/layers.py
@@ -29,6 +29,32 @@
         if not x.is_cuda:
             raise RuntimeError("PReLU runs on the GPU kernels only")
         return _PReLUFn.apply(x, self.weight)
+
+
+class _BNPair:
+
+    ATTR = "_avse_bnpair"
+
+    def __init__(self, x, stats, gamma, beta, alpha, act, q_bwd):
+        self.x, self.stats, self.gamma, self.beta, self.alpha, self.act = x, stats, gamma, beta, alpha, act
+        self.q_out = bool(q_bwd) and K._q_ok(x, None)
+        self.clear()
+
+    def clear(self):
+        self.dy = self.dy_version = self.rows = self.ws = None
+
+    def offer(self, dy, rows, ws):
+        self.dy, self.dy_version, self.rows, self.ws = dy, dy._version, rows, ws
+        return dy
+
+    def takes(self, dy):
+        return (self.dy is not None and dy.data_ptr() == self.dy.data_ptr() and dy._version == self.dy_version
+                and dy.shape == self.x.shape and dy.stride() == self.x.stride() and dy.dtype == torch.float32)
+
+    @staticmethod
+    def of(t, act):
+        pair = getattr(t, _BNPair.ATTR, None)
+        return pair if pair is not None and pair.act == act else None
 
 
 class _BNActFn(torch.autograd.Function):
@@ -41,13 +67,25 @@
                                q_out=q_fwd)
         ctx.save_for_backward(x, res, stats, gamma, beta, alpha)
         ctx.act, ctx.training, ctx.q_bwd = act, training, q_bwd
+        ctx.pair = None
+        if (K.is_split_q(y) and training and res is None and act in (K.ACT_RELU, K.ACT_PRELU)
+                and K.bn_rows_ok(x, gamma, beta, alpha)):
+            ctx.pair = _BNPair(x, stats, gamma, beta, alpha, act, q_bwd)
+            setattr(y, _BNPair.ATTR, ctx.pair)
         return y
 
     @staticmethod
     def backward(ctx, dy):
         x, res, stats, gamma, beta, alpha = ctx.saved_tensors
-        dx, dres, dgamma, dbeta, dalpha = K.bnact_bwd(x, res, dy, stats, gamma, beta, ctx.act, alpha, ctx.training,
-                                                      q_out=ctx.q_bwd)
+        pair = ctx.pair
+        if pair is not None and pair.takes(dy):
+            dx, dres, dgamma, dbeta, dalpha = K.bnact_bwd_rows(x, dy, stats, gamma, beta, ctx.act, alpha, ctx.training,
+                                                               pair.rows, pair.ws, q_out=pair.q_out)
+        else:
+            dx, dres, dgamma, dbeta, dalpha = K.bnact_bwd(x, res, dy, stats, gamma, beta, ctx.act, alpha, ctx.training,
+                                                          q_out=ctx.q_bwd)
+        if pair is not None:
+            pair.clear()
         return (dx, dgamma if ctx.needs_input_grad[1] else None, dbeta if ctx.needs_input_grad[2] else None,
                 dalpha if ctx.needs_input_grad[3] else None, dres, None, None, None, None, None, None, None, None)
 
@@ -176,6 +214,7 @@
         ctx.split = K.dconv_split_ok(x, dilation)
         if K.is_split_q(x) and not ctx.split:
             raise RuntimeError("_DilatedConvFn: a split-output input needs the split path (DilatedConv2d.q_ok)")
+        ctx.bnpair = _BNPair.of(x, K.ACT_RELU) if ctx.split else None
         if ctx.split:
             mb = torch.empty(2, device=x.device, dtype=torch.int32)
             xq = K.split16(x, mb)
@@ -204,7 +243,11 @@
                 xq, mb, w = ctx.saved_tensors
                 wq_t, mbd = None, torch.empty(2, device=dy.device, dtype=torch.int32)
             dyq = K.split16(dy, mbd)
-            if ctx.needs_input_grad[0]:
+            pair = ctx.bnpair
+            if ctx.needs_input_grad[0] and pair is not None and wq_t is not None:
+                dx = pair.offer(*K.dconv_dgrad_bn(ctx.shape, d, (dyq, mbd), wq_t, pair.x, pair.stats, pair.gamma,
+                                                  pair.beta, pair.act, pair.q_out))
+            elif ctx.needs_input_grad[0]:
                 dx = K.dconv_fwd(dy, w, d, transposed=True, split=(dyq, mbd), wq=wq_t)
             if ctx.needs_input_grad[1] or ctx.needs_input_grad[2]:
                 dw, db = K.dconv_wgrad16((xq, mb[:1]), (dyq, mbd[:1]), ctx.shape, d, bias_grad=True)
@@ -497,6 +540,7 @@
     def forward(ctx, x, w, stride):
         xq, xm = K.split_q(x)
         ctx.shape, ctx.stride = tuple(x.shape), stride
+        ctx.bnpair = _BNPair.of(x, K.ACT_PRELU) if stride == 1 else None
         ctx.save_for_backward(xq, xm, w)
         return K.sconv_fwd((xq, xm), ctx.shape, w, stride)
 
@@ -507,7 +551,11 @@
         dyq, dym = K.split_q(dy)
         dx = dw = None
         if ctx.needs_input_grad[0]:
-            if s == 1:
+            pair = ctx.bnpair
+            if s == 1 and pair is not None:
+                dx = pair.offer(*K.sconv_dgrad1_bn((dyq, dym), tuple(dy.shape), w, pair.x, pair.stats, pair.gamma,
+                                                   pair.beta, pair.act, pair.alpha, pair.q_out))
+            elif s == 1:
                 dx = K.sconv_fwd((dyq, dym), tuple(dy.shape), w, 1, transposed=True)
             else:
                 dx = K.sconv_dgrad2((dyq, dym), shape, w)
diff --git a/include/avse_hip.h b/include/avse_hip.h
--- a/include/avse_hip.h
+++ b/include/avse_hip.h
@@ -177,6 +177,11 @@
                      const float* gamma, const float* beta, int32_t act, const float* alpha, int32_t alpha_n,
                      int32_t training, void* dxq, float* dgamma, float* dbeta, float* dalpha_c, float* workspace,
                      uint32_t* dx_bound, avse_stream_t stream);
+int64_t avse_bnact_rows_workspace_bytes(int64_t rows, int64_t C, int64_t nq);
+int avse_bnact_bwd_rows(int64_t N, int64_t C, int64_t rows, const float* x, const float* dy, const float* stats,
+                        const float* gamma, const float* beta, int32_t act, const float* alpha, int32_t alpha_n,
+                        int32_t training, float* dx, float* dgamma, float* dbeta, float* dalpha_c, float* workspace,
+                        uint32_t* dx_max, int32_t q_out, avse_stream_t stream);
 
 int64_t avse_maxpool2d_out_size(int64_t H, int64_t K, int64_t S, int64_t P);
 int avse_maxpool2d_fwd(int64_t planes, int64_t H, int64_t W, int64_t KH, int64_t KW, int64_t SH, int64_t SW, int64_t PH,
@@ -291,6 +296,16 @@
                      avse_stream_t stream);
 int avse_dconv_fwd(int64_t N, int64_t H, int64_t W, int64_t dil, const void* xq, const void* wq,
                    const uint32_t* maxbits, const float* bias, float* y, avse_stream_t stream);
+int64_t avse_dconv_bn_rows(int64_t N, int64_t H, int64_t W, int64_t dil);
+int avse_dconv_dgrad_bn(int64_t N, int64_t H, int64_t W, int64_t dil, const void* dyq, const void* wq_t,
+                        const uint32_t* maxbits, float* dx, const float* bn_x, const float* bn_stats,
+                        const float* gamma, const float* beta, int32_t act, int32_t want_max, float* rows,
+                        avse_stream_t stream);
+int64_t avse_sconv_bn_rows(int64_t N, int64_t H, int64_t W, int64_t co);
+int avse_sconv_dgrad1_bn(int64_t N, int64_t H, int64_t W, int64_t ci, int64_t co, const void* dyq,
+                         const uint32_t* dymax, const void* wq_t, const uint32_t* wmax, float* dx, const float* bn_x,
+                         const float* bn_stats, const float* gamma, const float* beta, int32_t act, const float* alpha,
+                         int32_t alpha_n, int32_t want_max, float* rows, avse_stream_t stream);
 int64_t avse_dconv_wgrad16_workspace_bytes(int64_t N, int64_t H, int64_t W);
 int avse_dconv_wgrad16(int64_t N, int64_t H, int64_t W, int64_t dil, const void* xq, const uint32_t* xmax,
                        const void* dyq, const uint32_t* dymax, float* dw, float* db, float* workspace,
```

Measured after the change: 445.9 utt/s (median of 6 runs). 1.6% higher.
